# swacisko/ALGA

Hardware: AMD Instinct MI355X
Metric: overlap_edges_per_sec (higher is better)
Workload: dtype u32; 1 GPU; cfg4_50M_150bp: 50000000 x 150 bp reads, genome 250000000, seed 11, err 0.00 -> 90621096 nodes (both strands, duplicates removed), min_overlap 82, rsoemo 116; generated on the device (alga_amd.workload.device_build) in 0.9 s; nodes=90621096, edges=92350115

## Files before the change

alga_amd/csrc/engine.hip:

```cpp
#include <hip/hip_runtime.h>

#include <algorithm>
#include <chrono>
#include <cstdio>
#include <cstdlib>
#include <cstring>
#include <new>
#include <string>
#include <thread>
#include <vector>

#include "engine_internal.h"
#include "prefsuf_shard.h"

using namespace alga;

namespace {

using Prepared = AlgaPrepared;

int prepare(alga_engine *e, const alga_nodes *nodes, const alga_prefsuf_params *p, hipStream_t s, Prepared &out) {
    if (!nodes || !p) return alga_fail(e, ALGA_ERR_INVALID_ARGUMENT, "nodes/params must not be NULL");
    if (nodes->n < 0) return alga_fail(e, ALGA_ERR_INVALID_ARGUMENT, "negative node count");
    if (nodes->n > 0 && (!nodes->words || !nodes->len)) return alga_fail(e, ALGA_ERR_INVALID_ARGUMENT, "words/len must not be NULL");
// ... 88 lines not shown
    const void *before = e->cl_pile_tab.p;
    const size_t cap_before = e->cl_pile_tab.cap;
    if ((rc = alga_ensure(e, e->cl_pile_tab, pile_table_bytes(n_buckets)))) return rc;
    if (e->cl_pile_tab.p != before || e->cl_pile_tab.cap != cap_before) {
        HIP_TRY(e, hipMemsetAsync(e->cl_pile_tab.p, 0, e->cl_pile_tab.cap, s));
        HIP_TRY(e, hipStreamSynchronize(s));
        e->pile_epoch = 0;
    }
    return ALGA_OK;
}

int discover_impl(alga_engine *e, const Prepared &pp, int32_t src_begin, int32_t src_end, hipStream_t s, uint64_t *n_rec, bool local = false,
                  bool *overflow = nullptr) {
    int rc;
    const NodesDev &nd = pp.nd;
    const PrefSufCfg &cfg = pp.cfg;
    unsigned long long *cnt = (unsigned long long *) e->counters.p;
    *n_rec = 0;
    HIP_TRY(e, hipEventRecord(e->ev[EV_START], s));
    if (pp.live >= (1ull << 31)) return alga_fail(e, ALGA_ERR_CAPACITY, "too many nodes for one seed table; shard the input");
    const bool clustered = local && pp.cluster_eq != 0;
    e->pairs_timed = false;
    e->store_timed = false;
    e->pile_timed = false;
    e->pile_deg_pending = false;
    const bool all_sources = src_begin == 0 && src_end == pp.nd.n;
    const bool pile_index_left = e->opt_pile_range != 0 && e->pile_n == pp.nd.n && e->pile_words == (const void *) pp.nd.words;
    bool pile = clustered && e->opt_pile != 0 && e->opt_cluster_pairs != 0 && e->opt_cluster_order != 0 && pp.local_sw == 1 &&
                      (pp.keys_shared == 0 || (pp.keys_shared == 2 && pile_index_left)) &&
                      (all_sources || (e->opt_pile_range != 0 && src_begin >= 0 && src_end <= pp.nd.n && src_begin < src_end)) && pile_plan(cfg, pp.cluster, pp.cluster_eq, pp.uniform_len, pp.nd.from != nullptr || pp.nd.to != nullptr);
    e->loc_second_used = false;
    bool keys_only = false;
    const bool need_vals = !e->opt_own_sort || e->opt_test_unsorted_index;
    uint32_t n_buckets = 0, filter_bits = 0;
    bool have_table = false;
    auto build_table = [&]() -> int {
        n_buckets = seed_buckets_for(pp.live, e->seed_fill_x10);
        const size_t table_bytes = (size_t) n_buckets * SEED_BUCKET * sizeof(unsigned long long);
        int r;
        if ((r = alga_ensure(e, e->table, table_bytes))) return r;
        HIP_TRY(e, hipMemsetAsync(e->table.p, 0xFF, table_bytes, s));
        filter_bits = seed_filter_bits_for(pp.live);
        if (filter_bits) {
            if ((r = alga_ensure(e, e->filter, filter_bits / 8))) return r;
            HIP_TRY(e, hipMemsetAsync(e->filter.p, 0, filter_bits / 8, s));
        }
        launch_seed_build(nd, cfg, (unsigned long long *) e->table.p, n_buckets, (uint32_t *) e->filter.p, filter_bits, s);
        if ((r = alga_check_launch(e, "k_seed_build"))) return r;
        e->stats.table_slots = (uint64_t) n_buckets * SEED_BUCKET;
        have_table = true;
        return ALGA_OK;
    };
    ClusterCfg cc{};
    if (clustered) {
        cc = pp.cluster;
        if ((rc = cluster_alloc(e, pp))) return rc;
        if (pp.keys_shared == 2) {
            const bool store_left = e->store_n == nd.n && e->store_words == (const void *) nd.words && e->store_eq == pp.cluster_eq && e->store_buckets == cc.n_buckets;
            const bool piles_serve = pile && e->pile_kept_pure && e->store_buckets == cc.n_buckets && e->store_eq == pp.cluster_eq;
            if (!(store_left || piles_serve) || src_begin < e->store_run_begin || src_end > e->store_run_end)
                return alga_fail(e, ALGA_ERR_INVALID_ARGUMENT, "keys_shared = 2: no entry array of this node set that covers the sources is left from the previous build");
            keys_only = pile && e->pile_keys_only;
        } else {
            int32_t run_begin = 0, run_end = nd.n;
            if (pp.keys_shared == 1) {
                if (e->keyed_n != nd.n || e->keyed_words != (const void *) nd.words || src_begin < e->keyed_begin || src_end > e->keyed_end)
                    return alga_fail(e, ALGA_ERR_INVALID_ARGUMENT, "keys_shared: alga_prefsuf_keys_device has not been called on this node set for a range that covers the sources");
                run_begin = e->keyed_begin; run_end = e->keyed_end;
            } else {
                keys_only = pile && e->opt_pile_runs != 0 && !e->expect_pairwise && !e->opt_pile_check;
                launch_cluster_keys(nd, cfg, cc, 0, nd.n, (uint32_t *) e->cl_keys[0].p, need_vals ? (uint32_t *) e->cl_vals[0].p : nullptr, (uint32_t *) e->cl_meta.p, e->cl_runs.p,
                                    (uint8_t *) e->cl_nruns.p, s, !keys_only);
                if ((rc = alga_check_launch(e, "k_node_runs"))) return rc;
            }
            HIP_TRY(e, hipEventRecord(e->ev[EV_KEYS], s));
            e->keyed_n = -1;
            e->store_n = -1;
            HIP_TRY(e, launch_cluster_sort(nd, cc, (uint32_t *) e->cl_keys[0].p, (uint32_t *) e->cl_vals[0].p, (uint32_t *) e->cl_keys[1].p,
                                           (uint32_t *) e->cl_vals[1].p, e->sort_temp.p, cluster_sort_temp_bytes((uint64_t) nd.n), pp.keys_shared == 1 || !need_vals,
                                           e->ev[EV_SORT], e->opt_test_unsorted_index != 0, s, e->opt_own_sort != 0));
            const bool dir_late = pile && e->opt_pile_dir >= 1;
            e->dir_late = dir_late;
            if (!dir_late) {
                HIP_TRY(e, launch_cluster_dir(nd, cc, (const uint32_t *) e->cl_keys[1].p, e->cl_dir.p, cnt + CNT_TOTAL + 1, nullptr, s));
                HIP_TRY(e, hipEventRecord(e->ev[EV_DIR], s));
            }
            e->pile_n = -1;
            if (pile) {
                rc = e->opt_test_pile_oom ? alga_fail(e, ALGA_ERR_OUT_OF_MEMORY, "pile_alloc (option test_pile_oom)") : pile_alloc(e, (uint64_t) nd.n, cc.n_buckets, s);
                if (rc == ALGA_ERR_OUT_OF_MEMORY) {
                    (void) hipGetLastError();
                    alga_release(e->cl_pile_tab); alga_release(e->cl_pile_rec); alga_release(e->cl_pile_rec2); alga_release(e->cl_pile_succ); alga_release(e->cl_pile_own);
                    alga_release(e->cl_pile_list);
                    e->pile_epoch = 0; e->pile_n = -1;
                    e->err.clear();
                    pile = false;
                    rc = ALGA_OK;
                    if (keys_only) {
                        launch_cluster_keys(nd, cfg, cc, 0, nd.n, (uint32_t *) e->cl_keys[0].p, (uint32_t *) e->cl_vals[0].p, (uint32_t *) e->cl_meta.p, e->cl_runs.p,
                                            (uint8_t *) e->cl_nruns.p, s, true);
                        if ((rc = alga_check_launch(e, "k_node_runs"))) return rc;
                        keys_only = false;
                    }
                } else if (rc) return rc;
            }
            if (pile) {
                launch_pile_sample(nd, cc, pp.uniform_len, (const uint32_t *) e->cl_keys[1].p, (const uint32_t *) e->cl_vals[1].p, e->cl_dir.p,
                                   (unsigned long long *) e->cl_pile_cnt.p, e->opt_pile >= 2 ? e->opt_pile - 1 : 0, s, e->opt_pile_dir >= 1);
                if ((rc = alga_check_launch(e, "k_pile_build<sample>"))) return rc;
            }
            e->pile_tab_index = pile && e->opt_pile_dir >= 2 && e->opt_pile_skip_gather && !cfg.stats;
            if (dir_late) {
                HIP_TRY(e, hipEventRecord(e->ev[EV_SAMPLE], s));
                HIP_TRY(e, launch_cluster_dir(nd, cc, (const uint32_t *) e->cl_keys[1].p, e->cl_dir.p, cnt + CNT_TOTAL + 1,
                                              e->pile_tab_index ? (const unsigned long long *) e->cl_pile_cnt.p : nullptr, s));
                HIP_TRY(e, hipEventRecord(e->ev[EV_DIR], s));
            }
            HIP_TRY(e, launch_cluster_gather(nd, cc, pp.cluster_eq, (const uint32_t *) e->cl_keys[1].p, (const uint32_t *) e->cl_vals[1].p, (const uint32_t *) e->cl_meta.p,
                                             pp.uniform_len, e->cl_store.p, (pile && e->opt_pile_skip_gather) ? (const unsigned long long *) e->cl_pile_cnt.p : nullptr, s));
            HIP_TRY(e, hipEventRecord(e->ev[EV_GATHER], s));
            if (pile) {
                if (e->pile_epoch >= 511u) {
                    HIP_TRY(e, hipMemsetAsync(e->cl_pile_tab.p, 0, e->cl_pile_tab.cap, s));
                    e->pile_epoch = 0;
                }
                e->pile_epoch++;
                const bool from_consensus = e->opt_pile_runs != 0;
                launch_pile_build(nd, cfg, cc, pp.uniform_len, (const uint32_t *) e->cl_keys[1].p, (const uint32_t *) e->cl_vals[1].p, e->cl_dir.p, e->cl_pile_rec.p, e->cl_pile_rec2.p, e->cl_pile_tab.p,
                                  e->pile_epoch, e->cl_pile_succ.p, e->cl_runs.p, pp.uniform_len - cfg.Lmin + 1, (const unsigned long long *) e->cl_pile_cnt.p,
                                  from_consensus ? (uint32_t *) e->cl_pile_own.p : nullptr, (from_consensus && e->opt_pile_runs_list) ? e->cl_pile_list.p : nullptr, s,
                                  e->opt_pile_dir >= 1, cnt + CNT_TOTAL + 1, e->pile_tab_index, e->opt_pile_runs_ahead != 0);
                if ((rc = alga_check_launch(e, "k_pile_build"))) return rc;
                if (keys_only) {
                    launch_pile_own_ids((const uint32_t *) e->cl_pile_own.p, (const uint32_t *) e->cl_vals[1].p, (uint64_t) nd.n, (int32_t *) e->cl_defer.p, (uint32_t) nd.n,
                                        (unsigned long long *) e->cl_pile_cnt.p, s);
                    launch_cluster_runs_list(nd, cfg, cc, (const int32_t *) e->cl_defer.p, (const unsigned long long *) e->cl_pile_cnt.p + 3, (uint32_t) nd.n, (uint32_t) e->n_cu * 16u,
                                             e->cl_runs.p, (uint8_t *) e->cl_nruns.p, s);
                    launch_cluster_keys(nd, cfg, cc, 0, nd.n, (uint32_t *) e->cl_keys[0].p, (uint32_t *) e->cl_vals[0].p, (uint32_t *) e->cl_meta.p, e->cl_runs.p,
                                        (uint8_t *) e->cl_nruns.p, s, true, (const unsigned long long *) e->cl_pile_cnt.p);
                    if ((rc = alga_check_launch(e, "k_node_runs (own lists)"))) return rc;
                }
                if (e->opt_pile_check && from_consensus)
                    launch_pile_check(e->cl_pile_succ.p, (uint64_t) nd.n, cc.n_buckets, e->cl_pile_tab.p, e->cl_pile_rec2.p, e->pile_epoch, e->cl_runs.p, nd.n, pp.uniform_len - cfg.Lmin + 1,
                                      (unsigned long long *) e->cl_pile_cnt.p, s);
                e->pile_n = nd.n; e->pile_words = (const void *) nd.words;
                e->pile_keys_only = keys_only; e->pile_kept_pure = false;
                e->pile_timed = nd.n > 0;
            }
            e->store_timed = nd.n > 0;
            e->store_n = pile ? -1 : nd.n;
            e->store_words = (const void *) nd.words; e->store_eq = pp.cluster_eq; e->store_buckets = cc.n_buckets;
            e->store_run_begin = run_begin; e->store_run_end = run_end;
        }
        e->stats.table_slots = cc.n_buckets;
    } else if ((rc = build_table())) return rc;
    HIP_TRY(e, hipEventRecord(e->ev[EV_SEED], s));

    const uint64_t n_src = (uint64_t) std::max<int64_t>(0, (int64_t) src_end - src_begin);
    const uint64_t slack = std::max(probe_record_slack(e->n_cu, n_src, local), clustered ? cluster_record_slack(e->n_cu, n_src) : 0);
    uint64_t &hint = local ? e->rec_cap_hint_local : e->rec_cap_hint;
    uint64_t cap = std::max<uint64_t>(hint, (local ? 2 : 16) * n_src + 4096) + slack;
    if (local) {
        if ((rc = alga_ensure(e, e->outdeg, (size_t) (n_src + 1) * sizeof(uint32_t)))) return rc;
        if ((rc = alga_ensure(e, e->loc_first, (size_t) (n_src + 1) * sizeof(unsigned long long)))) return rc;
    }
    const uint32_t big_list_cap = 1u << 20;
    if (local && (rc = alga_ensure(e, e->loc_big_list, big_list_cap * sizeof(int32_t)))) return rc;
    bool pure_streamed = false;
    for (int attempt = 0; attempt < 4; attempt++) {
        if (cap >= (1ull << 32) - 16) return alga_fail(e, ALGA_ERR_CAPACITY, "more than 2^32 overlap records; shard the input");
        if (local) HIP_TRY(e, hipMemsetAsync(e->outdeg.p, 0, (size_t) (n_src + 1) * sizeof(uint32_t), s));
        if ((rc = alga_ensure(e, e->rec_dst, cap * sizeof(uint32_t)))) return rc;
        if ((rc = alga_ensure(e, e->rec_val, cap * sizeof(unsigned long long)))) return rc;
        HIP_TRY(e, hipMemsetAsync(cnt, 0, CNT_TOTAL * sizeof(unsigned long long), s));
        ProbeBig big{(int32_t *) e->loc_big_list.p, big_list_cap, 0u, nullptr, 0u};
        e->defer_list_valid = clustered && e->opt_cluster_pairs && pp.local_sw == 1 && pp.cluster_eq <= 4;
        if (clustered) {
            if (e->opt_cluster_pairs && pp.local_sw == 1 && pp.cluster_eq <= 4) {
                if ((rc = alga_ensure(e, e->cl_defer, (size_t) (n_src + 64) * sizeof(int32_t)))) return rc;
                const uint32_t slot_stride = e->opt_stream_slots >= 4 ? (uint32_t) (n_src + 1) : 0u;
                if ((rc = alga_ensure(e, e->loc_second, (size_t) (slot_stride ? LOCAL_SLOTS_MAX - 1 : 1) * (n_src + 1) * sizeof(unsigned long long)))) return rc;
                e->loc_second_used = true;
                e->loc_slot_stride = slot_stride;
                const bool by_key = e->opt_cluster_order != 0 && src_begin == 0 && src_end == nd.n;
                const bool piled = pile && e->pile_n == nd.n && e->pile_words == (const void *) nd.words;
                if (piled) {
                    if (!all_sources) {
                        if ((rc = alga_ensure(e, e->cl_pile_side_r, (size_t) (n_src + 64) * 16))) return rc;
                        if ((rc = alga_ensure(e, e->cl_pile_cursor, 64))) return rc;
                    }
                    launch_pile_probe(nd, cfg, cc, pp.uniform_len, e->cl_pile_tab.p, e->pile_epoch, e->cl_pile_rec.p, e->cl_pile_rec2.p, e->cl_pile_succ.p,
                                      e->cl_runs.p, cnt, (uint32_t *) e->outdeg.p, (unsigned long long *) e->loc_first.p, (unsigned long long *) e->loc_second.p,
                                      (int32_t *) e->cl_defer.p, (uint32_t) n_src, (const unsigned long long *) e->cl_pile_cnt.p, e->n_cu, s, src_begin, src_end,
                                      e->cl_pile_side_r.p, (unsigned long long *) e->cl_pile_cursor.p, e->opt_pile_probe_lean != 0, e->opt_pile_probe_tail != 0);
                    if ((rc = alga_check_launch(e, "k_pile_probe"))) return rc;
                    if (keys_only)
                        launch_cluster_runs_list(nd, cfg, cc, (const int32_t *) e->cl_defer.p, cnt + CNT_DEFERRED, (uint32_t) std::min<uint64_t>(n_src + 64, 0xFFFFFFFFull),
                                                 (uint32_t) e->n_cu * 16u, e->cl_runs.p, (uint8_t *) e->cl_nruns.p, s);
                }
                launch_probe_stream(nd, cfg, cc, pp.cluster_eq, e->cl_store.p, e->cl_dir.p, e->cl_runs.p, (const uint8_t *) e->cl_nruns.p,
                                    src_begin, src_end, by_key, cnt, e->n_cu, (uint32_t *) e->outdeg.p, (unsigned long long *) e->loc_first.p,
                                    (unsigned long long *) e->loc_second.p, (int32_t *) e->cl_defer.p, (uint32_t) n_src,
                                    piled ? (const unsigned long long *) e->cl_pile_cnt.p : nullptr, s, slot_stride);
                if ((rc = alga_check_launch(e, "k_probe_stream"))) return rc;
                if (piled) {
                    if ((rc = alga_ensure(e, e->cl_defer2, (size_t) (n_src + 64) * sizeof(int32_t)))) return rc;
                    pure_streamed = launch_probe_stream_list(nd, cfg, cc, pp.cluster_eq, e->cl_store.p, e->cl_dir.p, e->cl_runs.p, (const uint8_t *) e->cl_nruns.p, (int32_t *) e->cl_defer.p,
                                             (uint32_t) n_src, cnt, e->n_cu, (uint32_t *) e->outdeg.p, (unsigned long long *) e->loc_first.p,
                                             (unsigned long long *) e->loc_second.p, (int32_t *) e->cl_defer2.p, (const unsigned long long *) e->cl_pile_cnt.p, s, slot_stride, src_begin,
                                             (const uint32_t *) e->cl_keys[1].p, (const uint32_t *) e->cl_vals[1].p, pp.uniform_len, e->opt_pile_stream_by_id != 0,
                                             e->pile_tab_index ? e->cl_pile_tab.p : nullptr, e->pile_epoch);
                    if ((rc = alga_check_launch(e, "k_probe_stream (list)"))) return rc;
                }
                HIP_TRY(e, hipEventRecord(e->ev[EV_PAIRS], s));
// ... 256 lines not shown
    hipError_t err = hipGetDeviceCount(&ndev);
    if (err != hipSuccess || ndev <= 0) return ALGA_ERR_NO_DEVICE;
    if (hip_device < 0 || hip_device >= ndev) return ALGA_ERR_INVALID_ARGUMENT;
    DeviceGuard guard;
    if (hipSetDevice(hip_device) != hipSuccess) return ALGA_ERR_NO_DEVICE;
    alga_engine *e = new (std::nothrow) alga_engine();
    if (!e) return ALGA_ERR_OUT_OF_MEMORY;
    e->device = hip_device;
    memset(&e->stats, 0, sizeof(e->stats));
    hipDeviceProp_t prop;
    if (hipGetDeviceProperties(&prop, hip_device) == hipSuccess) {
        snprintf(e->dev_name, sizeof(e->dev_name), "%s (%s, %d CUs)", prop.name, prop.gcnArchName, prop.multiProcessorCount);
        if (prop.multiProcessorCount > 0) e->n_cu = prop.multiProcessorCount;
    }
    int rc = ALGA_OK;
    if (hipStreamCreateWithFlags(&e->own_stream, hipStreamNonBlocking) != hipSuccess) { e->own_stream = nullptr; rc = ALGA_ERR_HIP; }
    if (rc == ALGA_OK && hipStreamCreateWithFlags(&e->side_stream, hipStreamNonBlocking) != hipSuccess) { e->side_stream = nullptr; rc = ALGA_ERR_HIP; }
    if (rc == ALGA_OK && hipEventCreateWithFlags(&e->ev_side, hipEventDisableTiming) != hipSuccess) { e->ev_side = nullptr; rc = ALGA_ERR_HIP; }
    for (int i = 0; i < EV_COUNT && rc == ALGA_OK; i++)
        if (hipEventCreate(&e->ev[i]) != hipSuccess) { e->ev[i] = nullptr; rc = ALGA_ERR_HIP; }
    if (rc == ALGA_OK && hipHostMalloc((void **) &e->h_counters, (CNT_TOTAL + 2 + alga_engine::H_EXTRA) * sizeof(unsigned long long)) != hipSuccess) { e->h_counters = nullptr; rc = ALGA_ERR_OUT_OF_MEMORY; }
    if (rc == ALGA_OK && hipHostGetDevicePointer((void **) &e->h_counters_dev, e->h_counters, 0) != hipSuccess) rc = ALGA_ERR_HIP;
    if (rc != ALGA_OK) { engine_free_handles(e); delete e; return rc; }
    *out = e;
    return ALGA_OK;
}

void alga_engine_destroy(alga_engine *e) {
    if (!e) return;
    DeviceGuard guard;
    (void) hipSetDevice(e->device);
    if (e->own_stream) (void) hipStreamSynchronize(e->own_stream);
    if (e->side_stream) (void) hipStreamSynchronize(e->side_stream);
    for (DevBuf *b : e->owned) alga_release(*b);
    alga_release(e->up_raw);
    for (DevBuf *b : {&e->in_bytes[0], &e->in_bytes[1], &e->in_nl[0], &e->in_nl[1], &e->in_tiles, &e->in_tile_off}) alga_release(*b);
    for (DevBuf *b : {&e->sp_rowptr, &e->sp_sorted, &e->sp_list, &e->sp_cnt, &e->sp_orow, &e->sp_out, &e->sp_in}) alga_release(*b);
    alga_staging_release(e);
    for (void *&p : e->gfa_pin) { if (p) (void) hipHostFree(p); p = nullptr; }
    for (auto &kv : e->host_lists) free(kv.first);
    e->host_lists.clear();
    engine_free_handles(e);
    delete e;
}

const char *alga_last_error(const alga_engine *e) { return e ? e->err.c_str() : "no engine"; }

int alga_engine_device_name(const alga_engine *e, char *buf, size_t buflen) {
    if (!e || !buf || buflen == 0) return ALGA_ERR_INVALID_ARGUMENT;
    snprintf(buf, buflen, "%s", e->dev_name);
    return ALGA_OK;
}

int alga_engine_set_option(alga_engine *e, const char *name, int64_t value) {
    if (!e || !name) return ALGA_ERR_INVALID_ARGUMENT;
    e->err.clear();
    if (!strcmp(name, "probe")) {
        if (value < ALGA_PROBE_AUTO || value > ALGA_PROBE_CLUSTER) return alga_fail(e, ALGA_ERR_INVALID_ARGUMENT, "option probe: 0 auto, 1 table, 2 cluster");
        e->opt_probe = (int) value;
    } else if (!strcmp(name, "cluster_bucket_bias")) {
        if (value < -8 || value > 8) return alga_fail(e, ALGA_ERR_INVALID_ARGUMENT, "option cluster_bucket_bias: -8 .. 8");
        e->opt_cluster_bucket_bias = (int) value;
    } else if (!strcmp(name, "cluster_pairs")) {
        e->opt_cluster_pairs = value != 0;
    } else if (!strcmp(name, "pile")) {
        e->opt_pile = (value == 2 || value == 3) ? (int) value : (value != 0);
    } else if (!strcmp(name, "pile_runs")) {
        e->opt_pile_runs = value != 0;
    } else if (!strcmp(name, "pile_runs_list")) {
        e->opt_pile_runs_list = value != 0;
    } else if (!strcmp(name, "pile_dir")) {
        if (value < 0 || value > 2) return alga_fail(e, ALGA_ERR_INVALID_ARGUMENT, "option pile_dir: 0 directory records, 1 k_pile_build from the keys, 2 ... and no directory for a pure pile build");
        e->opt_pile_dir = (int) value;
    } else if (!strcmp(name, "pile_deg_fold")) {
        e->opt_pile_deg_fold = value != 0;
    } else if (!strcmp(name, "emit_fused")) {
        e->opt_emit_fused = value != 0;
    } else if (!strcmp(name, "pile_probe_lean")) {
        e->opt_pile_probe_lean = value != 0;
    } else if (!strcmp(name, "pile_probe_tail")) {
        e->opt_pile_probe_tail = value != 0;
    } else if (!strcmp(name, "pile_runs_ahead")) {
        e->opt_pile_runs_ahead = value != 0;
    } else if (!strcmp(name, "pile_stream_by_id")) {
        e->opt_pile_stream_by_id = value != 0;
    } else if (!strcmp(name, "pile_check")) {
        e->opt_pile_check = value != 0;
    } else if (!strcmp(name, "pile_skip_gather")) {
        e->opt_pile_skip_gather = value != 0;
    } else if (!strcmp(name, "cluster_order")) {
        e->opt_cluster_order = value != 0;
    } else if (!strcmp(name, "local_big_max")) {
        e->big_limit = value < 0 ? -1 : (int) std::min<int64_t>(value, 1 << 20);
    } else if (!strcmp(name, "shard_bucket_max")) {
        e->opt_shard_dmax = (int) std::max<int64_t>(1, std::min<int64_t>(value, 4096));
    } else if (!strcmp(name, "rsort_variant")) {
        if (value < 0 || value > 1) return alga_fail(e, ALGA_ERR_INVALID_ARGUMENT, "option rsort_variant: 0 tiles of 8192 pairs, 1 tiles of 16384 pairs");
        rsort_set_variant((int) value);
    } else if (!strcmp(name, "stream_slots")) {
        e->opt_stream_slots = value >= 4 ? 4 : 2;
    } else if (!strcmp(name, "pile_range")) {
        e->opt_pile_range = value != 0;
    } else if (!strcmp(name, "pkb_legacy")) {
        e->opt_pkb_legacy = (int) value;
    } else if (!strcmp(name, "own_sort")) {
        e->opt_own_sort = value != 0;
    } else if (!strcmp(name, "test_presort_oom")) {
        e->opt_test_presort_oom = value != 0;
    } else if (!strcmp(name, "test_pile_oom")) {
        e->opt_test_pile_oom = value != 0;
    } else if (!strcmp(name, "test_unsorted_index")) {
        e->opt_test_unsorted_index = value != 0;
    } else if (!strcmp(name, "gfa_chunk_mb")) {
        if (value < 1 || value > 4096) return alga_fail(e, ALGA_ERR_INVALID_ARGUMENT, "option gfa_chunk_mb: 1 .. 4096");
        e->opt_gfa_chunk_mb = (int) value;
    } else if (!strcmp(name, "mst_mid_nodes")) {
        if (value < 8 || value > (1 << 20)) return alga_fail(e, ALGA_ERR_INVALID_ARGUMENT, "option mst_mid_nodes: 8 .. 2^20");
        e->opt_mst_mid_nodes = (int) value;
    } else if (!strcmp(name, "consensus_max_blocks")) {
        if (value < 0 || value > (1 << 20)) return alga_fail(e, ALGA_ERR_INVALID_ARGUMENT, "option consensus_max_blocks: 0 .. 2^20");
        e->opt_consensus_max_blocks = (int) value;
    } else if (!strcmp(name, "unitig_ruling")) {
        if (value < -1 || value > 1) return alga_fail(e, ALGA_ERR_INVALID_ARGUMENT, "option unitig_ruling: -1, 0 or 1");
        e->opt_unitig_ruling = (int) value;
    } else if (!strcmp(name, "correct_slice_keys")) {
        if (value < 1 || value > (1ll << 31)) return alga_fail(e, ALGA_ERR_INVALID_ARGUMENT, "option correct_slice_keys: 1 .. 2^31");
        e->opt_correct_slice_keys = value;
    } else if (!strcmp(name, "correct_dir_bits")) {
        if (value < 0 || value > 28) return alga_fail(e, ALGA_ERR_INVALID_ARGUMENT, "option correct_dir_bits: 0 (auto) or 1 .. 28");
        e->opt_correct_dir_bits = (int) value;
    } else if (!strcmp(name, "place_dir_bits")) {
        if (value < 0 || value > 26) return alga_fail(e, ALGA_ERR_INVALID_ARGUMENT, "option place_dir_bits: 0 (auto) or 1 .. 26");
        e->opt_place_dir_bits = (int) value;
    } else if (!strcmp(name, "auto_reduction_per_target")) {
        e->opt_force_per_target = value != 0;
    } else return alga_fail(e, ALGA_ERR_INVALID_ARGUMENT, "unknown option");
    return ALGA_OK;
}

int alga_engine_reserve(alga_engine *e, int32_t n_nodes, int32_t max_len, int32_t min_overlap, uint64_t n_edges_hint) {
    if (!e) return ALGA_ERR_INVALID_ARGUMENT;
    e->err.clear();
    if (n_nodes < 0 || max_len < 1 || min_overlap < 1) return alga_fail(e, ALGA_ERR_INVALID_ARGUMENT, "alga_engine_reserve: n_nodes >= 0, max_len >= 1, min_overlap >= 1");
    DeviceGuard guard;
    HIP_TRY(e, hipSetDevice(e->device));
    int rc;
    const uint64_t n = (uint64_t) n_nodes;
    const uint64_t E = n_edges_hint ? n_edges_hint : n + n / 16 + 4096;
    if ((rc = alga_ensure(e, e->counters, (CNT_TOTAL + 2) * sizeof(unsigned long long)))) return rc;
    Prepared pp;
    pp.nd.n = n_nodes; pp.max_len = max_len; pp.live = n;
    pp.cfg.Lmin = min_overlap; pp.cfg.Lcap = std::min(max_len, 500) + 1; pp.cfg.rsoemo = min_overlap; pp.cfg.soes = 3;
    int eq = 0;
    const bool local = max_len <= 500 && max_len - min_overlap <= LOCAL_MAX_SPAN;
    const bool clustered = local && e->opt_probe != ALGA_PROBE_TABLE &&
                           cluster_plan(pp.cfg, max_len, n, e->opt_cluster_bucket_bias, &pp.cluster, &eq);
    if (clustered) {
        pp.cluster_eq = eq;
        if ((rc = cluster_alloc(e, pp))) return rc;
        if (max_len - min_overlap <= 63 && eq <= 4) {
            if ((rc = alga_ensure(e, e->cl_defer, (size_t) (n + 64) * sizeof(int32_t)))) return rc;
            if ((rc = alga_ensure(e, e->loc_second, (size_t) (e->opt_stream_slots >= 4 ? LOCAL_SLOTS_MAX - 1 : 1) * (n + 1) * sizeof(unsigned long long)))) return rc;
        }
        if (e->opt_pile != 0 && e->opt_cluster_pairs != 0 && e->opt_cluster_order != 0 && max_len - min_overlap <= 63 && pile_plan(pp.cfg, pp.cluster, eq, max_len, false)) {
            if ((rc = pile_alloc(e, n, pp.cluster.n_buckets, e->own_stream))) return rc;
        }
// ... 669 lines not shown
```

alga_amd/csrc/engine_internal.h:

```cpp
#pragma once
#include <hip/hip_runtime.h>

#include <cstdio>
#include <algorithm>
#include <string>
#include <vector>
#include <unordered_map>

#include "../../include/alga_amd.h"
#include "prefsuf_common.h"
#include "prefsuf_kernels.h"
#include "pkb_kernels.h"

struct DevBuf {
    void  *p = nullptr;
    size_t cap = 0;
};

enum { EV_START = 0, EV_SEED, EV_PROBE, EV_GROUP, EV_REDUCE, EV_EMIT, EV_PAIRS, EV_KEYS, EV_SORT, EV_GATHER, EV_DIR, EV_SAMPLE, EV_COUNT };
constexpr int ALGA_STAGE_THREADS = 8;

struct alga_engine {
    std::vector<DevBuf *> owned;
    int         device = -1;
    hipStream_t own_stream = nullptr;
    hipStream_t side_stream = nullptr;
    hipEvent_t  ev_side = nullptr;
    std::string err;
    char        dev_name[256] = {0};
    int         n_cu = 256;
    int         seed_fill_x10 = 20;
    int         opt_probe = 0;
    int         opt_cluster_bucket_bias = 0;
    int         opt_force_per_target = 0;
    int         opt_shard_dmax = 4096;
    int         opt_test_unsorted_index = 0;
    hipEvent_t  ev[EV_COUNT] = {};
    DevBuf table, filter, counters, rowptr, rec_dst, rec_val, keys, seg_key, seg_val, heads, sort_temp, out_cnt, outdeg, out_rowptr, edges, scan_scratch;
    DevBuf cl_defer;
    uint32_t h_first_hkey = 255;
    int32_t keyed_n = -1, keyed_begin = 0, keyed_end = 0;
    bool defer_list_valid = false;
    const void *keyed_words = nullptr;
    int32_t store_n = -1, store_run_begin = 0, store_run_end = 0, store_eq = 0;
    uint32_t store_buckets = 0;
    const void *store_words = nullptr;
    int stat_max_len = 0, stat_min_len = 0; uint64_t stat_live = 0; unsigned long long stat_mask_asym = 0;
    const void *stat_len = nullptr, *stat_from = nullptr, *stat_to = nullptr;
    bool   warmed = false;
    bool   pairs_timed = false;
    bool   store_timed = false;
    bool   pile_keys_only = false, pile_kept_pure = false;
    int    opt_pile_range = 1;
    int    opt_pile_skip_gather = 1;
    int    opt_pile = 1;
    int    opt_pile_runs = 1;
    int    opt_pile_runs_list = 1;
    DevBuf cl_pile_list;
    int    opt_pile_deg_fold = 1;
    int    opt_emit_fused = 1;
    int    opt_pile_dir = 2;
    bool   dir_late = false;
    bool   pile_tab_index = false;
    int    opt_pile_stream_by_id = 0;
    int    opt_pile_probe_lean = 1;
    int    opt_pile_probe_tail = 1;
    int    opt_pile_runs_ahead = 0;
    bool   pile_deg_pending = false;
    int    opt_pile_check = 0;
    bool   expect_pairwise = false;
    DevBuf cl_pile_side_r, cl_pile_cursor;
    DevBuf cl_pile_own;
    int    opt_pkb_legacy = 0;
    int    opt_own_sort = 1;
    int    opt_test_presort_oom = 0;
    int    opt_test_pile_oom = 0;
    bool   pile_timed = false;
    DevBuf cl_pile_succ;
    DevBuf cl_pile_rec2;
    DevBuf cl_pile_rec, cl_pile_cnt, cl_pile_tab;
    uint32_t pile_epoch = 0;
    int32_t pile_n = -1; const void *pile_words = nullptr;
    int    opt_cluster_order = 1;
    int    opt_cluster_pairs = 1;
    DevBuf cl_keys[2], cl_vals[2], cl_meta, cl_runs, cl_nruns, cl_store, cl_dir;
    DevBuf loc_second;
    bool   loc_second_used = false;
    uint32_t loc_slot_stride = 0;
    int    opt_stream_slots = 4;
    DevBuf loc_first, loc_big_list, loc_big_items;
    int    big_limit = -1;
    DevBuf edge_keys, edge_keys2, edge_vals, edge_vals2, edges_sorted, xs_dst, xs_val;
    DevBuf up_words, up_len, up_from, up_to;
    DevBuf up_len_narrow;
    DevBuf cp_deg, cp_dst, cp_off;
    DevBuf cl_defer2;
    DevBuf pk_keys, pk_keys2, pk_vals, pk_vals2, pk_marks, pk_big, pk_add, pk_ekeys, pk_ekeys2, pk_flag, pk_pos, pk_edges[2], pk_rowptr, pk_deg,
           pk_mask, pk_cnt, pk_io, pk_io2, pk_tips, pk_heads, pk_g[2], pk_addk, pk_addk2, pk_merged, pk_hsz, pk_hsz2, pk_heads2, pk_nadd, pk_koff,
           pk_gsz, pk_fixlist, pk_bounds, pk_tiprec, pk_tipidx, pk_keys_all, pk_vals_all;
    DevBuf pk_keys2b, pk_vals2b, pk_headsb, pk_hszb, sort_temp2, pk_fixlist2, pk_cnt2;
    DevBuf pp_rows, pp_len, pp_perm[2], pp_keys[2], pp_mark, pp_keep, pp_pos, pp_out_rows, pp_out_len, pp_out_pair, pp_tally;
    bool        stage_ready = false;
    void       *stage_pin[ALGA_STAGE_THREADS][2] = {};
    hipEvent_t  stage_ev[ALGA_STAGE_THREADS][2] = {};
    hipStream_t stage_stream[ALGA_STAGE_THREADS] = {};
    DevBuf      up_raw;
    std::unordered_map<void *, size_t> host_lists;
    void       *host_spare = nullptr;
    size_t      host_spare_cap = 0;
    DevBuf      in_bytes[2], in_nl[2], in_tiles, in_tile_off;
    DevBuf      sp_rowptr, sp_sorted, sp_list, sp_cnt, sp_orow, sp_out, sp_in;
    DevBuf      tp_cnt, tp_keys[2], tp_vals[2], tp_flag, tp_pos, tp_best, tp_est, tp_rev, tp_rfid, tp_rowptr[2], tp_alive, tp_kill, tp_rec[2], tp_branch,
                tp_overflow, tp_ws, tp_out;
    DevBuf      mp_cnt, mp_rowptr, mp_rows, mp_len, mp_owner, mp_pend[2], mp_win, mp_overflow, mp_overflow2, mp_ws, mp_ws_big, mp_orow, mp_out;
    struct MstFilled { const void *p = nullptr; size_t bytes = 0; uint32_t hbits = 0, cap_nodes = 0, cap_edges = 0; int32_t n_ws = 0; } mp_filled[2];
    int         opt_mst_mid_nodes = 4096;
    DevBuf      gfa_sizes, gfa_off, gfa_rowptr, gfa_tiles, gfa_bounds, gfa_buf;
    void       *gfa_pin[2] = {nullptr, nullptr};
    size_t      gfa_pin_cap = 0;
    int         opt_gfa_chunk_mb = 256;
    DevBuf      ut_cnt, ut_keys[2], ut_vals[2], ut_flag, ut_pos, ut_best, ut_estar, ut_rowptr, ut_nxt, ut_noff, ut_prv, ut_rank[2], ut_min[2], ut_tail,
                ut_win, ut_pair, ut_pcnt, ut_ulen, ut_ulen2, ut_uwords, ut_path_off, ut_word_off, ut_tiles, ut_path_node, ut_path_pos, ut_uid, ut_words,
                ut_edges, ut_link, ut_rnode, ut_rrec[2];
    int         opt_unitig_ruling = -1;
    uint64_t    ut_n_pairs = 0, ut_n_edges = 0;
    bool        ut_valid = false;
    int32_t     ut_n_nodes = 0;
    uint64_t    ut_total_bases = 0;
    bool        ut_is_contig = false;
    DevBuf      ex_cnt, ex_rowptr, ex_w, ex_kcnt, ex_dlink, ex_outcnt, ex_sole, ex_xhead, ex_xbase, ex_xrank, ex_uid, ex_scnt, ex_seam_off,
                ex_seam_entry, ex_pcnt, ex_uwords, ex_ulen, ex_ulen2, ex_path_off, ex_word_off, ex_path_node, ex_path_pos, ex_words, ex_edges;
    bool        ut_is_extended = false;
    DevBuf      ct_cnt, ct_B[2], ct_rowptr, ct_pflag, ct_runkey, ct_chain, ct_headchain, ct_drop, ct_flag, ct_pos, ct_keys[2], ct_vals[2], ct_hw, ct_hk, ct_H,
                ct_hrow, ct_hsorted, ct_hlist, ct_hcnt, ct_win, ct_pair, ct_oid, ct_cid, ct_deg, ct_epos, ct_ekeys[2], ct_evals[2], ct_names;
    DevBuf      cs_cnt, cs_words, cs_mask, cs_votes, cs_trim, cs_len, cs_changed;
    bool        cs_valid = false;
    bool        cs_has_votes = false;
    DevBuf      fc_cnt, fc_keys[2], fc_vals, fc_first, fc_min, fc_list[2], fc_flag, fc_ids, fc_verdict, fc_rank, fc_id, fc_new, fc_trim, fc_begin, fc_len,
                fc_order, fc_wbegin, fc_wlen, fc_rows, fc_rlen, fc_tid;
    bool        fc_valid = false;
    uint64_t    fc_n_accepted = 0;
    int         opt_consensus_max_blocks = 0;
    DevBuf      cr_cnt, cr_table, cr_hist, cr_keys[2], cr_flag, cr_pos, cr_solid, cr_dir;
    int64_t     opt_correct_slice_keys = 1ll << 28;
    int         opt_correct_dir_bits = 0;
    DevBuf      pl_cnt, pl_fbegin, pl_flen, pl_scan, pl_cols, pl_keys[2], pl_vals[2], pl_dir, pl_ub, pl_diff;
    DevBuf      pl_target, pl_pos, pl_mm, pl_hits, pl_state, pl_coloff, pl_cover, pl_tstat, pl_hist;
    bool        pl_valid = false;
    uint64_t    pl_targets = 0, pl_reads = 0;
    uint64_t    pl_ncolumns = 0, pl_nhist = 0;
// ... 3 lines not shown
    DevBuf      po_cnt, po_keys[2], po_vals[2], po_marks, po_pop, po_scan;
    DevBuf      po_coloff, po_words, po_ccols, po_cbases, po_tstat, po_counts;
    bool        po_valid = false;
    uint64_t    po_targets = 0, po_columns = 0;
    uint64_t    po_final_epoch = 0;
    uint64_t    pl_serial = 0, po_pl_serial = 0;
    DevBuf      sc_cnt, sc_keys[2], sc_vals[2], sc_span, sc_heads, sc_pos, sc_bstart, sc_best, sc_choice, sc_partner, sc_lists[2], sc_head, sc_first, sc_scan;
    DevBuf      sc_ba, sc_bb, sc_blinks, sc_bspan, sc_bgap, sc_bstate, sc_estate, sc_scaffold, sc_rank, sc_orient, sc_start, sc_gapafter, sc_jlinks, sc_soff,
                sc_smembers, sc_slen;
    bool        sc_valid = false;
    uint64_t    sc_targets = 0, sc_scaffolds = 0, sc_longest = 0;
    uint64_t    sc_pl_serial = 0;
    DevBuf      br_cnt, br_diff, br_starts, br_rpos, br_marks, br_rfirst, br_rlast, br_closed, br_cpos;
    DevBuf      br_span, br_ccols, br_cfirst, br_clast, br_tcuts, br_poff, br_begin, br_len, br_ptarget, br_pstart, br_words;
    bool        br_valid = false;
    uint64_t    br_targets = 0, br_pieces = 0, br_cuts = 0, br_columns = 0, br_longest = 0;
    DevBuf      gr_cnt, gr_flag, gr_pos, gr_cand, gr_elen, gr_eoff, gr_ecols, gr_keys[2], gr_vals[2], gr_dir, gr_ub, gr_x, gr_g;
    struct GrowSet { DevBuf end, over, mm, hits, state, count, estop, evoters, left, right, len, coloff, begin, words; } gr_set[2];
    int         gr_cur = 0;
    bool        gr_valid = false;
    uint64_t    gr_reads = 0, gr_targets = 0, gr_columns = 0, gr_longest = 0;
    DevBuf      mg_cnt, mg_elen, mg_epad, mg_eoff, mg_ecols, mg_pcols, mg_keys[2], mg_vals[2], mg_dir, mg_join, mg_lists[2], mg_head, mg_first, mg_scan;
    struct MergeSet { DevBuf partner, olen, mm, hits, estate, merged, rank, orient, start, ovafter, moff, mmembers, len, coloff, begin, words; } mg_set[2];
    int         mg_cur = 0;
    bool        mg_valid = false;
    uint64_t    mg_targets = 0, mg_merged = 0, mg_columns = 0, mg_longest = 0;
    DevBuf      sh_keys[2], sh_vals[2], sh_store, sh_dir, sh_desc_out, sh_dkey[2], sh_dval[2], sh_small_top, sh_pending, sh_bitmap, sh_small_out,
                sh_ssrc[2], sh_skey[2], sh_edges_out, sh_deg, sh_rowptr, sh_cursor, sh_edges, sh_flagged, sh_cnt, sh_gflag, sh_gpos, sh_gstart;
    struct {
        int      phase = 0;
        int      rank = 0, n_ranks = 1, eq = 0, uniform_len = 0;
        int32_t  n = 0;
        const void *words = nullptr;
        alga::PrefSufCfg cfg{};
        alga::ClusterCfg cc{};
        uint32_t bucket_base = 0, bpr = 0;
        uint64_t n_targets = 0, n_desc = 0, n_rec = 0;
        uint32_t *d_keys_sorted = nullptr;
        unsigned long long *d_vals_sorted = nullptr;
    } sh;
    alga_shard_stats shard_stats{};
    struct {
        int      phase = 0;
        int      rounds = 0, round = 0, rank = 0, n_ranks = 1, cur = 0, key_bits = 0;
        int32_t  prio[4] = {0, 1, 2, 3};
        uint64_t E = 0, nk = 0;
        uint32_t n_tips = 0;
        int      pre_set = 0, cur_set = 0;
        bool     no_look_ahead = false;
        int      pre_round = -1;
        bool     kmers_all = false;
        size_t   kmers_stride = 0;
        int      kmers_sort_bits = 0;
        alga_nodes dn{};
        alga::PkbCfg cfg{};
    } pkb;
    unsigned long long *h_counters = nullptr;
    static constexpr int H_EXTRA = 132 + 16, H_PRE = alga::CNT_TOTAL + 2 + 132;
    uint32_t *h_counters_dev = nullptr;
    uint64_t    rec_cap_hint = 0, rec_cap_hint_local = 0;
    alga_prefsuf_stats stats;
    double      stats_host[2] = {0.0, 0.0};
    alga_pkb_stats pkb_stats;
};

struct AlgaPrepared {
    alga::NodesDev   nd;
    alga::PrefSufCfg cfg;
    int        max_len = 0;
    int        uniform_len = 0;
    uint64_t   live = 0;
    bool       local_ok = false;
    int        local_sw = 1;
    int        cluster_eq = 0;
    alga::ClusterCfg cluster{};
    int        reduction = ALGA_REDUCTION_AUTO;
    int        keys_shared = 0;
};

extern "C" int alga_upload_nodes_phase(alga_engine *e, const alga_nodes *nodes, bool twin_rows, int mode, uint64_t row_begin, uint64_t row_end, uint64_t raw_rows_cap, alga_nodes *dev,
                            uint32_t **d_raw);
int alga_prepare(alga_engine *e, const alga_nodes *nodes, const alga_prefsuf_params *p, hipStream_t s, AlgaPrepared &out);
int alga_cluster_alloc(alga_engine *e, const AlgaPrepared &pp);

inline int alga_fail(alga_engine *e, int code, const char *what, hipError_t herr = hipSuccess) {
    char buf[512];
    if (herr != hipSuccess) snprintf(buf, sizeof(buf), "%s: %s", what, hipGetErrorString(herr));
    else snprintf(buf, sizeof(buf), "%s", what);
    e->err = buf;
    return code;
}

#define HIP_TRY(e, call)                                                                     \
    do {                                                                                     \
        hipError_t _err = (call);                                                            \
        if (_err != hipSuccess) return alga_fail((e), _err == hipErrorOutOfMemory ? ALGA_ERR_OUT_OF_MEMORY : ALGA_ERR_HIP, #call, _err); \
    } while (0)

inline int alga_ensure(alga_engine *e, DevBuf &b, size_t bytes) {
    if (bytes == 0) bytes = 16;
    if (b.cap >= bytes) return ALGA_OK;
    if (b.p) { HIP_TRY(e, hipFree(b.p)); b.p = nullptr; b.cap = 0; }
    else if (std::find(e->owned.begin(), e->owned.end(), &b) == e->owned.end()) e->owned.push_back(&b);
    HIP_TRY(e, hipMalloc(&b.p, bytes));
    b.cap = bytes;
    return ALGA_OK;
}

inline void alga_forget_node_set(alga_engine *e) {
    e->keyed_n = -1; e->store_n = -1; e->pile_n = -1;
    e->stat_len = nullptr; e->stat_from = nullptr; e->stat_to = nullptr;
}

inline void alga_release(DevBuf &b) {
    if (b.p) (void) hipFree(b.p);
    b.p = nullptr; b.cap = 0;
}

#include <chrono>
#include <functional>
typedef std::function<void(void * , size_t , size_t )> AlgaStageFill;
int  alga_staged_h2d(alga_engine *e, void *d_dst, const void *h_src, size_t bytes);
int  alga_staged_h2d_fill(alga_engine *e, void *d_dst, size_t bytes, const AlgaStageFill &fill);
int  alga_staged_d2h(alga_engine *e, void *h_dst, const void *d_src, size_t bytes);
void alga_staging_release(alga_engine *e);
void *alga_host_list_take(alga_engine *e, size_t bytes);
void alga_host_list_give(alga_engine *e, void *p);

constexpr int ALGA_UT_MAX_ROUNDS = 112;
int alga_ut_check(alga_engine *e, const alga_nodes *nodes, const alga::alga_edge_dev *d_in, uint64_t m, unsigned long long *cnt, hipStream_t s);
int alga_ut_estar(alga_engine *e, const alga_nodes *nodes, const alga::alga_edge_dev *d_in, uint64_t m, unsigned long long *cnt, hipStream_t s, uint64_t *ms_out);
int alga_ut_rank(alga_engine *e, const int32_t *len, int32_t n, int32_t *nxt, const int32_t *noff, int32_t *prv, unsigned long long *cnt, uint32_t *p_flag,
                 int &cur, int &rounds, hipStream_t s);

struct AlgaTextJob {
    uint64_t items;
    std::function<void(uint32_t *sizes, unsigned long long *counters, hipStream_t s)> sizes;
    std::function<void(const unsigned long long *off, uint64_t i0, uint64_t i1, char *buf, hipStream_t s)> format;
    const char *kind = "FASTA";
    const char *head = "";
    std::function<int(unsigned long long *counters, hipStream_t s)> prepare;
};
int alga_text_job_run(alga_engine *e, const AlgaTextJob &job, const char *path, alga_gfa_info *info,
                      std::chrono::steady_clock::time_point t0 = std::chrono::steady_clock::now());

template <class F> int alga_text_records(alga_engine *e, const F &f, void (*sizes)(const F &, uint32_t *, unsigned long long *, hipStream_t),
                                         void (*write)(const F &, const unsigned long long *, uint64_t, uint64_t, char *, hipStream_t), const char *path,
                                         alga_gfa_info *info, std::chrono::steady_clock::time_point t0 = std::chrono::steady_clock::now()) {
    AlgaTextJob job;
    job.items = f.n;
    job.sizes = [f, sizes](uint32_t *out, unsigned long long *counters, hipStream_t s) { sizes(f, out, counters, s); };
    job.format = [f, write](const unsigned long long *off, uint64_t i0, uint64_t i1, char *buf, hipStream_t s) { write(f, off, i0, i1, buf, s); };
    return alga_text_job_run(e, job, path, info, t0);
}

int alga_correct_check_params(alga_engine *e, const alga_correct_params *p);
int alga_correct_impl(alga_engine *e, uint32_t *d_rows, int32_t stride, const int32_t *d_len, int64_t n_nodes, const alga_correct_params *p, hipStream_t s,
                      alga_correct_info *info);

bool alga_final_is_current(const alga_engine *e, const alga_unitigs *u, const alga_consensus *cons, const alga_final_contigs *fin, const char **why);

inline int alga_check_launch(alga_engine *e, const char *what) {
    hipError_t err = hipGetLastError();
    if (err != hipSuccess) return alga_fail(e, ALGA_ERR_HIP, what, err);
    return ALGA_OK;
}
// ... 1 lines not shown
```

alga_amd/csrc/engine_shard.hip:

```cpp
#include <hip/hip_runtime.h>

#include <algorithm>
#include <cstring>
#include <vector>

#include "engine_internal.h"
#include "prefsuf_shard.h"

using namespace alga;

namespace {

struct EvPair { hipEvent_t a = nullptr, b = nullptr; };

struct PhaseTimer {
    hipStream_t s; hipEvent_t a = nullptr, b = nullptr;
    explicit PhaseTimer(hipStream_t st) : s(st) { if (hipEventCreate(&a) != hipSuccess) a = nullptr; if (hipEventCreate(&b) != hipSuccess) b = nullptr; if (a) (void) hipEventRecord(a, s); }
    double stop() { float ms = 0.f; if (a && b && hipEventRecord(b, s) == hipSuccess && hipEventSynchronize(b) == hipSuccess) (void) hipEventElapsedTime(&ms, a, b); return ms; }
    ~PhaseTimer() { if (a) (void) hipEventDestroy(a); if (b) (void) hipEventDestroy(b); }
};

int shard_sync_counters(alga_engine *e, hipStream_t s, const unsigned long long *d, int n, std::vector<unsigned long long> &h) {
    h.assign(256, 0ull);
    HIP_TRY(e, hipStreamSynchronize(s));
    HIP_TRY(e, hipMemcpy(h.data(), d, (size_t) n * sizeof(unsigned long long), hipMemcpyDeviceToHost));
    return ALGA_OK;
}

}

extern "C" {

int alga_shard_index_device(alga_engine *e, const alga_nodes *nodes, const alga_prefsuf_params *p, int32_t rank, int32_t n_ranks, void *hip_stream,
                            const uint32_t **d_desc, uint64_t *desc_counts, uint64_t *desc_offsets) {
    if (!e) return ALGA_ERR_INVALID_ARGUMENT;
    e->err.clear();
    if (!d_desc || !desc_counts || !desc_offsets) return alga_fail(e, ALGA_ERR_INVALID_ARGUMENT, "output pointers must not be NULL");
    *d_desc = nullptr;
    if (n_ranks < 1 || n_ranks > 64 || rank < 0 || rank >= n_ranks) return alga_fail(e, ALGA_ERR_INVALID_ARGUMENT, "bad rank / n_ranks (1 .. 64 ranks)");
    for (int q = 0; q < n_ranks; q++) { desc_counts[q] = 0; desc_offsets[q] = 0; }
    e->sh.phase = 0;
    HIP_TRY(e, hipSetDevice(e->device));
    hipStream_t s = hip_stream ? (hipStream_t) hip_stream : e->own_stream;
    const int32_t kb = e->keyed_begin, ke = e->keyed_end;
    if (!nodes || e->keyed_n != nodes->n || e->keyed_words != (const void *) nodes->words)
        return alga_fail(e, ALGA_ERR_INVALID_ARGUMENT, "alga_shard_index_device: alga_prefsuf_keys_device has not been called on this node set");
    alga_prefsuf_params p2 = *p;
    p2.keys_shared = 2;
    e->store_n = -1;
    AlgaPrepared pp;
    {
        const int32_t kn = e->keyed_n;
        int rc = alga_prepare(e, nodes, &p2, s, pp);
        if (rc) return rc;
        e->keyed_n = kn;
    }
    if (!pp.local_ok || pp.cluster_eq == 0 || pp.cluster_eq > 4 || pp.local_sw != 1 || pp.reduction == ALGA_REDUCTION_PER_TARGET)
        return alga_fail(e, ALGA_ERR_UNSUPPORTED, "the bucket-sharded form takes reads of up to 208 nt with max_len - min_overlap <= 63 (one-word offset masks) and the source-side preconditions");
    memset(&e->shard_stats, 0, sizeof(e->shard_stats));
    const ClusterCfg cc = pp.cluster;
    const uint32_t n = (uint32_t) nodes->n;
    const uint32_t bpr = shard_buckets_per_rank(cc.n_buckets, n_ranks);
    const uint32_t b_lo = std::min<uint64_t>((uint64_t) rank * bpr, cc.n_buckets), b_hi = std::min<uint64_t>((uint64_t) (rank + 1) * bpr, cc.n_buckets);
    int rc;
    if ((rc = alga_ensure(e, e->sh_cnt, 256 * sizeof(unsigned long long)))) return rc;
    unsigned long long *cnt = (unsigned long long *) e->sh_cnt.p;
    HIP_TRY(e, hipMemsetAsync(cnt, 0, 256 * sizeof(unsigned long long), s));
    PhaseTimer t_index(s);
    for (int k = 0; k < 2; k++) {
        if ((rc = alga_ensure(e, e->sh_keys[k], ((size_t) n + 1) * sizeof(uint32_t)))) return rc;
        if ((rc = alga_ensure(e, e->sh_vals[k], ((size_t) n + 1) * sizeof(uint32_t)))) return rc;
    }
    launch_shard_select((const uint32_t *) e->cl_keys[0].p, n, cc.idx_shift, b_lo, b_hi, (uint32_t *) e->sh_keys[0].p, (uint32_t *) e->sh_vals[0].p, cnt, s);
    if ((rc = alga_check_launch(e, "k_shard_select"))) return rc;
    const uint32_t flagged_cap = 1u << 20;
    if ((rc = alga_ensure(e, e->sh_flagged, (size_t) flagged_cap * sizeof(int32_t)))) return rc;
    launch_shard_export(true, e->cl_runs.p, kb, ke, cc.idx_shift, bpr, (uint32_t) n_ranks, cnt + 64, (int32_t *) e->sh_flagged.p, cnt + 1, flagged_cap, nullptr, nullptr, nullptr, s);
    if ((rc = alga_check_launch(e, "k_shard_export (count)"))) return rc;
    std::vector<unsigned long long> hc;
    if ((rc = shard_sync_counters(e, s, cnt, 128, hc))) return rc;
    const uint64_t m = hc[0], n_flagged = hc[1];
    if (n_flagged > flagged_cap) return alga_fail(e, ALGA_ERR_UNSUPPORTED, "more than 2^20 sources of this rank need brute-force window minimizers");
    std::vector<unsigned long long> seg((size_t) n_ranks + 1, 0ull);
    for (int q = 0; q < n_ranks; q++) seg[(size_t) q + 1] = seg[(size_t) q] + hc[64 + (size_t) q] + 64ull * n_flagged;
    const uint64_t desc_cap = seg[(size_t) n_ranks];
    if (desc_cap >= (1ull << 32) - 16) return alga_fail(e, ALGA_ERR_CAPACITY, "more than 2^32 run descriptors on one rank");
    if ((rc = alga_ensure(e, e->sh_desc_out, (desc_cap + 1) * 12))) return rc;
    HIP_TRY(e, hipMemcpyAsync(cnt + 192, seg.data(), (size_t) n_ranks * sizeof(unsigned long long), hipMemcpyHostToDevice, s));
    const uint32_t n_b_local = b_hi - b_lo;
    if ((rc = alga_ensure(e, e->sh_store, (m + 2) * 16 * (size_t) pp.cluster_eq))) return rc;
    if ((rc = alga_ensure(e, e->sh_dir, ((size_t) n_b_local + 2) * 16))) return rc;
    if ((rc = alga_ensure(e, e->sort_temp, std::max(cluster_sort_temp_bytes(m), sort_desc_temp_bytes(1))))) return rc;
    HIP_TRY(e, launch_cluster_store_slice(pp.nd, cc, pp.cluster_eq, m, b_lo, n_b_local, (uint32_t *) e->sh_keys[0].p, (uint32_t *) e->sh_vals[0].p, (uint32_t *) e->sh_keys[1].p,
                                          (uint32_t *) e->sh_vals[1].p, (const uint32_t *) e->cl_meta.p, pp.uniform_len, e->sort_temp.p, cluster_sort_temp_bytes(m),
                                          e->sh_store.p, e->sh_dir.p, cnt + 2, s, e->opt_own_sort != 0));
    e->shard_stats.ms_index = t_index.stop();
    PhaseTimer t_export(s);
    launch_shard_export(false, e->cl_runs.p, kb, ke, cc.idx_shift, bpr, (uint32_t) n_ranks, nullptr, nullptr, nullptr, 0u, cnt + 192, cnt + 128, (uint32_t *) e->sh_desc_out.p, s);
    if ((rc = alga_check_launch(e, "k_shard_export"))) return rc;
    launch_shard_export_flagged(pp.nd, pp.cfg, cc, (const int32_t *) e->sh_flagged.p, (uint32_t) n_flagged, bpr, (uint32_t) n_ranks, cnt + 192, cnt + 128,
                                (uint32_t *) e->sh_desc_out.p, s);
    if ((rc = alga_check_launch(e, "k_shard_export_flagged"))) return rc;
    e->shard_stats.ms_export = t_export.stop();
    if ((rc = shard_sync_counters(e, s, cnt, 192, hc))) return rc;
    if (hc[2] != 0) return alga_fail(e, ALGA_ERR_HIP, "bucket-sharded index: the sorted key array is not in order");
    uint64_t total = 0;
    for (int q = 0; q < n_ranks; q++) {
        desc_counts[q] = hc[128 + (size_t) q]; desc_offsets[q] = seg[(size_t) q];
        if (desc_counts[q] > seg[(size_t) q + 1] - seg[(size_t) q]) return alga_fail(e, ALGA_ERR_HIP, "bucket-sharded index: descriptor segment overflow");
        total += desc_counts[q];
    }
    e->shard_stats.targets_owned = m; e->shard_stats.descriptors_out = total; e->shard_stats.flagged_sources = n_flagged;
    e->sh.phase = 1; e->sh.rank = rank; e->sh.n_ranks = n_ranks; e->sh.eq = pp.cluster_eq; e->sh.uniform_len = pp.uniform_len; e->sh.n = nodes->n;
    e->sh.words = (const void *) nodes->words; e->sh.cfg = pp.cfg; e->sh.cc = cc; e->sh.bucket_base = b_lo; e->sh.bpr = bpr; e->sh.n_targets = m;
    *d_desc = (const uint32_t *) e->sh_desc_out.p;
    return ALGA_OK;
}

int alga_shard_join_device(alga_engine *e, const alga_nodes *nodes, const uint32_t *d_desc_in, uint64_t n_desc, void *hip_stream, const uint32_t **d_pending_src,
                           uint64_t *n_pending_src) {
    if (!e) return ALGA_ERR_INVALID_ARGUMENT;
    e->err.clear();
    if (!d_pending_src || !n_pending_src) return alga_fail(e, ALGA_ERR_INVALID_ARGUMENT, "output pointers must not be NULL");
    *d_pending_src = nullptr; *n_pending_src = 0;
    if (e->sh.phase != 1 || !nodes || nodes->n != e->sh.n || (const void *) nodes->words != e->sh.words)
        return alga_fail(e, ALGA_ERR_INVALID_ARGUMENT, "alga_shard_join_device follows alga_shard_index_device on the same node set");
    if (n_desc && !d_desc_in) return alga_fail(e, ALGA_ERR_INVALID_ARGUMENT, "descriptor array must not be NULL");
    if (n_desc >= (1ull << 32) - 16) return alga_fail(e, ALGA_ERR_CAPACITY, "more than 2^32 run descriptors on one rank");
    HIP_TRY(e, hipSetDevice(e->device));
    hipStream_t s = hip_stream ? (hipStream_t) hip_stream : e->own_stream;
    int rc;
    NodesDev nd;
    nd.words = nodes->words; nd.len = nodes->len; nd.from = nodes->align_from; nd.to = nodes->align_to; nd.n = nodes->n; nd.stride = nodes->stride_words;
    unsigned long long *cnt = (unsigned long long *) e->counters.p;
    unsigned long long *scnt = (unsigned long long *) e->sh_cnt.p;
    PhaseTimer t_sort(s);
    for (int k = 0; k < 2; k++) {
        if ((rc = alga_ensure(e, e->sh_dkey[k], (n_desc + 64) * sizeof(uint32_t)))) return rc;
        if ((rc = alga_ensure(e, e->sh_dval[k], (n_desc + 64) * sizeof(unsigned long long)))) return rc;
    }
    if ((rc = alga_ensure(e, e->sort_temp, sort_desc_temp_bytes(n_desc)))) return rc;
    if ((rc = alga_ensure(e, e->sh_small_top, (n_desc + 1) * 3 * sizeof(unsigned long long)))) return rc;
    const int shift = e->sh.cc.idx_shift;
    int range_bits = 1;
    while (range_bits < 32 - shift && (1ull << range_bits) < (uint64_t) e->sh.bpr) range_bits++;
    launch_shard_desc_split(d_desc_in, n_desc, e->sh.bucket_base << shift, (uint32_t *) e->sh_dkey[0].p, (unsigned long long *) e->sh_dval[0].p, s);
    if ((rc = alga_check_launch(e, "k_shard_desc_split"))) return rc;
    HIP_TRY(e, sort_desc(e->sort_temp.p, sort_desc_temp_bytes(n_desc), (const uint32_t *) e->sh_dkey[0].p, (uint32_t *) e->sh_dkey[1].p, (const unsigned long long *) e->sh_dval[0].p,
                         (unsigned long long *) e->sh_dval[1].p, n_desc, shift, std::min(32, shift + range_bits), s, e->opt_own_sort != 0));
    if ((rc = alga_ensure(e, e->sh_gflag, (n_desc + 2) * sizeof(uint32_t)))) return rc;
    if ((rc = alga_ensure(e, e->sh_gpos, (n_desc + 2) * sizeof(uint32_t)))) return rc;
    if ((rc = alga_ensure(e, e->sh_gstart, (n_desc + 2) * sizeof(uint32_t)))) return rc;
    if ((rc = alga_ensure(e, e->scan_scratch, scan_scratch_bytes(n_desc + 1)))) return rc;
    launch_shard_groups((const uint32_t *) e->sh_dkey[1].p, n_desc, e->sh.cc.idx_shift, (uint32_t *) e->sh_gflag.p, (uint32_t *) e->sh_gpos.p, (uint32_t *) e->sh_gstart.p,
                        (uint64_t *) e->scan_scratch.p, s);
    if ((rc = alga_check_launch(e, "k_shard_groups"))) return rc;
    uint32_t n_groups = 0;
    if (n_desc) {
        HIP_TRY(e, hipMemcpyAsync(e->h_counters, (const uint32_t *) e->sh_gpos.p + n_desc, sizeof(uint32_t), hipMemcpyDeviceToHost, s));
        HIP_TRY(e, hipStreamSynchronize(s));
        n_groups = *(const uint32_t *) e->h_counters;
    }
    e->shard_stats.ms_sort = t_sort.stop();
    e->sh.d_keys_sorted = (uint32_t *) e->sh_dkey[1].p; e->sh.d_vals_sorted = (unsigned long long *) e->sh_dval[1].p;
    PhaseTimer t_join(s);
    const uint64_t slack = shard_join_record_slack(e->n_cu);
    uint64_t cap = std::max<uint64_t>(e->rec_cap_hint, 2 * e->sh.n_targets + n_desc / 4 + 4096) + slack;
    uint64_t n_rec = 0;
    bool done = false;
    unsigned long long join_passes[2] = {0, 0};
    for (int attempt = 0; attempt < 4 && !done; attempt++) {
        if (cap >= (1ull << 32) - 16) return alga_fail(e, ALGA_ERR_CAPACITY, "more than 2^32 overlap records; shard the input");
        if ((rc = alga_ensure(e, e->rec_dst, cap * sizeof(uint32_t)))) return rc;
        if ((rc = alga_ensure(e, e->rec_val, cap * sizeof(unsigned long long)))) return rc;
        HIP_TRY(e, hipMemsetAsync(cnt, 0, CNT_TOTAL * sizeof(unsigned long long), s));
        HIP_TRY(e, hipMemsetAsync(scnt, 0, 8 * sizeof(unsigned long long), s));
        launch_shard_join(nd, e->sh.cfg, e->sh.cc, e->sh.eq, e->sh.uniform_len, e->sh_store.p, e->sh_dir.p, e->sh.bucket_base, e->sh.d_keys_sorted, e->sh.d_vals_sorted, n_desc,
                          (const uint32_t *) e->sh_gstart.p, n_groups, (uint32_t *) e->rec_dst.p, (unsigned long long *) e->rec_val.p, cap, cnt, (unsigned long long *) e->sh_small_top.p, scnt + 3, e->opt_shard_dmax, e->n_cu, s);
// ... 181 lines not shown
```

alga_amd/csrc/prefsuf_cluster.hip:

```cpp
#include <hip/hip_runtime.h>
#include <algorithm>
#include "prefsuf_common.h"
#include "prefsuf_kernels.h"
#include "prefsuf_device.h"
#include "prefsuf_cluster_device.h"

namespace alga {


template <int TKW, bool WIDE, bool RUNS>
__global__ void __launch_bounds__(TK_ROWS) k_node_runs(NodesDev nd, PrefSufCfg cfg, ClusterCfg cc, int node_begin, int node_end,
                                                        uint32_t *__restrict__ keys, uint32_t *__restrict__ vals, uint32_t *__restrict__ meta,
                                                        uint2 *__restrict__ runs, uint8_t *__restrict__ nruns, const int32_t *__restrict__ id_list, const unsigned long long *__restrict__ id_count,
                                                        const unsigned long long *__restrict__ only_if_declined ) {
    if (only_if_declined && !pile_cnt_declines(only_if_declined)) return;
    __shared__ uint32_t s[TK_ROWS][TKW];
    __shared__ uint32_t stk[RUNS ? 2 * (NR_STACK + 1) : 1][TK_ROWS];
    __shared__ uint16_t rbuf[RUNS ? CL_RMAX + 1 : 1][TK_ROWS];
    const int list_n = id_list ? (int) min((unsigned long long) (node_end - node_begin), *id_count) : 0;
    __shared__ int sid[TK_ROWS];
    for (int blk = (int) blockIdx.x; id_list ? blk * TK_ROWS < list_n : node_begin + blk * TK_ROWS < node_end; blk += (int) gridDim.x) {
    const int base = node_begin + blk * TK_ROWS;
    const int nrows = id_list ? min(TK_ROWS, list_n - blk * TK_ROWS) : min(TK_ROWS, node_end - base);
    if (blk != (int) blockIdx.x) __syncthreads();
// ... 38 lines not shown
        for (int r = 0; r < CL_RMAX; r++) {
            if (r < nr_stored && is_src) {
                const uint32_t d = rbuf[r][t];
                const int q = (int) (d & 255u);
                uint32_t h, pk;
                kmer_key(row, q < (WIDE ? 192 : 128) ? q : 0, true, cc, h, pk);
                runs[(size_t) i * CL_RMAX + r] = make_uint2(cluster_key(h, fs), d | ((uint32_t) p1 << 16) | (r == 0 ? nr_code << 24 : 0u));
                p1 = (int) (d >> 8);
            }
        }
        if (in && !is_src) runs[(size_t) i * CL_RMAX] = make_uint2(0u, 0u);
        if (in) nruns[i] = (uint8_t) nr_code;
        if (id_list) continue;
    } else {
        const int nk = act ? min(nwin, WIDE ? 64 : nwin) - 1 + w : 0;
        uint64_t b0;
        {
            const uint32_t x0 = row[0], x1 = row[1], x2 = row[2], x3 = row[3], x4 = row[4];
            const uint32_t d0 = compress_even(class0_mask16(x0, x1)) | (compress_even(class0_mask16(x1, x2)) << 16);
            const uint32_t d1 = compress_even(class0_mask16(x2, x3)) | (compress_even(class0_mask16(x3, x4)) << 16);
            b0 = (uint64_t) d0 | ((uint64_t) d1 << 32);
            b0 &= nk >= 64 ? ~0ull : (nk <= 0 ? 0ull : ((1ull << nk) - 1ull));
            b0 &= w >= 64 ? ~0ull : ((1ull << w) - 1ull);
        }
        while (b0 != 0ull) {
            const int e = __builtin_ctzll(b0);
            b0 &= b0 - 1ull;
            const int bit = 2 * e, q = bit >> 5, r = bit & 31;
            const uint32_t x0 = row[q], x1 = row[q + 1], x2 = row[q + 2];
            const uint32_t pk = order_key0(kmer_hash(funnel(x0, x1, r) & cc.lo_mask, funnel(x1, x2, r) & cc.hi_mask), e);
            cur0 = pk < cur0 ? pk : cur0;
        }
    }
    uint32_t key = 0xFFFFFFFFu, m = act ? (((uint32_t) len << 8) | (is_src ? CL_META_FROM : 0u)) : 0u;
    if (is_tgt) {
        uint32_t pmin = cur0;
        if (pmin == 0xFFFFFFFFu) {
            for (int k = 0; k < w; k++) { uint32_t h, pk; kmer_key(row, k, true, cc, h, pk); pmin = pk < pmin ? pk : pmin; }
        }
        uint32_t h, pk;
        kmer_key(row, (int) (pmin & 255u), true, cc, h, pk);
        key = tgt_sort_key(cluster_key(h, fs), pmin & 255u, fs);
        m = (pmin & 255u) | ((uint32_t) len << 8) | (is_src ? CL_META_FROM : 0u);
    }
    if (in) { keys[i] = key; if (vals) vals[i] = (uint32_t) i; meta[i] = m; }
    }
}

template <int EQ, bool UNIFORM>
__global__ void __launch_bounds__(256) k_tgt_gather(NodesDev nd, uint64_t count ,
                                                     const uint32_t *__restrict__ keys, const uint32_t *__restrict__ vals,
                                                     const uint32_t *__restrict__ meta, uint32_t uniform_meta, int fs, uint4 *__restrict__ store,
                                                     const unsigned long long *__restrict__ pile_cnt ) {
    if (pile_cnt && pile_cnt[1] * PILE_IRREGULAR_ONE_IN <= pile_cnt[0]) return;
    for (uint64_t t = (uint64_t) blockIdx.x * blockDim.x + threadIdx.x; t < count * EQ; t += (uint64_t) gridDim.x * blockDim.x) {
    const uint64_t j = t / EQ;
    const int c = (int) (t % EQ);
    const uint32_t key = keys[j];
    const uint32_t id = vals[j];
    const uint32_t *row = nd.words + (size_t) id * nd.stride;
    uint4 v;
    if ((nd.stride & 3) == 0 && 4 * c + 3 < nd.stride && ((uintptr_t) nd.words & 15u) == 0) v = reinterpret_cast<const uint4 *>(row)[c];
    else {
        v.x = 4 * c + 0 < nd.stride ? row[4 * c + 0] : 0u; v.y = 4 * c + 1 < nd.stride ? row[4 * c + 1] : 0u;
        v.z = 4 * c + 2 < nd.stride ? row[4 * c + 2] : 0u; v.w = 4 * c + 3 < nd.stride ? row[4 * c + 3] : 0u;
    }
    if (c == EQ - 1) {
        v.y = id; v.z = key;
        if (!UNIFORM) v.w = meta[id];
        else if (key != 0xFFFFFFFFu) v.w = uniform_meta | ((key >> fs) & ((1u << CL_MBITS) - 1u));
        else v.w = (uint32_t) nd.len[id] == (uniform_meta >> 8 & 0xFFFu) ? uniform_meta : 0u;
    }
    store[j * EQ + c] = v;
    }
}

constexpr int TD_TILE = 256, TD_HALO = 96;
__global__ void __launch_bounds__(TD_TILE) k_tgt_dir(const uint32_t *__restrict__ keys, uint64_t n, int shift, uint32_t n_buckets ,
                                                     uint32_t bucket_base , uint4 *__restrict__ dir,
                                                     unsigned long long *__restrict__ bad ,
                                                     const unsigned long long *__restrict__ pile_cnt ) {
    if (pile_cnt && pile_cnt_pure(pile_cnt)) return;
    __shared__ uint32_t sb[TD_TILE + TD_HALO + 1];
    const uint64_t base = (uint64_t) blockIdx.x * TD_TILE;
    const uint32_t nb3 = n_buckets << 3;
    auto tagged = [&](uint64_t k) -> uint32_t { if (k >= n) return nb3; const uint32_t x = keys[k]; return x == 0xFFFFFFFFu ? nb3 : (x >> (shift - 3)) - (bucket_base << 3); };
    for (int k = (int) threadIdx.x; k <= TD_TILE + TD_HALO; k += TD_TILE)
        sb[k] = (base == 0 && k == 0) ? 0xFFFFFFFFu : tagged(base + (uint64_t) k - 1u);
    __syncthreads();
    const int t = (int) threadIdx.x, lane = lane_id();
    const uint64_t j = base + (uint64_t) t;
    auto put = [&](int64_t b, const uint4 &rec) { dir[b] = rec; };
    auto tally = [](unsigned long long acc, uint32_t cls) { return acc + (0x0101010101010100ull << (8u * cls)); };
    if (j >= 1 && j < n && sb[t + 1] < sb[t]) atomicOr(bad, 1ull);
    const uint32_t b = sb[t + 1] >> 3;
    const bool start = j <= n && b != (sb[t] >> 3);
    if (start && b == n_buckets) put(b, make_uint4((uint32_t) j, 0u, 0u, 0u));
    const bool real = start && b != n_buckets;
    constexpr int TD_SHORT = 4;
    const bool is_short = real && (sb[t + 1 + TD_SHORT] >> 3) != b;
    if (is_short) {
        unsigned long long acc = 0ull;
        int u = 0;
#pragma unroll
        for (; u < TD_SHORT; u++) {
            const uint32_t x = sb[t + 1 + u];
            if ((x >> 3) != b) break;
            acc = tally(acc, x & 7u);
        }
        put(b, make_uint4((uint32_t) j, (uint32_t) u, (uint32_t) acc, (uint32_t) (acc >> 32)));
    }
    unsigned long long longs = __ballot(real && !is_short);
    const int g = lane >> 4, gl = lane & 15;
    while (longs != 0ull) {
        int lsel = 64;
#pragma unroll
        for (int q = 0; q < 4; q++) {
            const int l = longs ? __builtin_ctzll(longs) : 64;
            longs = longs ? (longs & (longs - 1ull)) : 0ull;
            lsel = g == q ? l : lsel;
        }
        const bool has = lsel < 64;
        const int t0 = (t & ~63) + (has ? lsel : 0);
        const uint32_t bb = bperm(b, has ? lsel : 0);
        unsigned long long acc = 0ull;
        bool open = has, past = false;
        for (int u = 0;; u += 16) {
            const int idx = t0 + 1 + u + gl;
            const bool staged = idx <= TD_TILE + TD_HALO;
            const uint32_t x = staged ? sb[idx] : 0xFFFFFFFFu;
            const bool inb = open && staged && (x >> 3) == bb;
            const unsigned long long c = inb ? ((0x0101010101010100ull << (8u * (x & 7u))) | 1ull) : 0ull;
            uint32_t lo = (uint32_t) c, hi = (uint32_t) (c >> 32);
            lo += (uint32_t) __builtin_amdgcn_update_dpp(0, (int) lo, 0x111, 0xF, 0xF, true); hi += (uint32_t) __builtin_amdgcn_update_dpp(0, (int) hi, 0x111, 0xF, 0xF, true);
            lo += (uint32_t) __builtin_amdgcn_update_dpp(0, (int) lo, 0x112, 0xF, 0xF, true); hi += (uint32_t) __builtin_amdgcn_update_dpp(0, (int) hi, 0x112, 0xF, 0xF, true);
            lo += (uint32_t) __builtin_amdgcn_update_dpp(0, (int) lo, 0x114, 0xF, 0xF, true); hi += (uint32_t) __builtin_amdgcn_update_dpp(0, (int) hi, 0x114, 0xF, 0xF, true);
            lo += (uint32_t) __builtin_amdgcn_update_dpp(0, (int) lo, 0x118, 0xF, 0xF, true); hi += (uint32_t) __builtin_amdgcn_update_dpp(0, (int) hi, 0x118, 0xF, 0xF, true);
            lo = bperm(lo, lane | 15); hi = bperm(hi, lane | 15);
            acc += ((unsigned long long) hi << 32) | lo;
            const uint32_t took = lo & 255u, cnt = (uint32_t) acc & 255u;
            if (open && took < 16u) { open = false; past = t0 + 1 + u + (int) took > TD_TILE + TD_HALO; }
            else if (open && cnt >= 240u) { open = false; past = true; }
            if (__ballot(open) == 0ull) break;
        }
        if (has && gl == 0) {
            const uint64_t j0 = base + (uint64_t) t0;
            uint64_t k = j0 + (uint64_t) ((uint32_t) acc & 255u);
            acc &= ~255ull;
            if (past) {
                for (; k < j0 + 256u; k++) {
                    const uint32_t x = tagged(k);
                    if ((x >> 3) != bb) break;
                    acc = tally(acc, x & 7u);
                }
                if (k >= j0 + 256u && (tagged(k) >> 3) == bb) {
                    uint64_t a = k, z = n;
                    while (z - a > 1) { const uint64_t mid = a + (z - a) / 2; if ((tagged(mid) >> 3) == bb) a = mid; else z = mid; }
                    k = z;
                }
            }
            const uint32_t c = (uint32_t) (k - j0);
            put(bb, make_uint4((uint32_t) j0, c, c <= 255u ? (uint32_t) acc : 0u, c <= 255u ? (uint32_t) (acc >> 32) : 0u));
        }
    }
}

#ifndef CL_OCC
#define CL_OCC 6
#endif

struct ByIdEntries {
    const uint32_t *skeys, *sids;
    uint32_t uniform_meta;
    const unsigned long long *pile_cnt;
    BucketIndex bx;
};
__device__ __forceinline__ void by_id_pair(const ByIdEntries &by, size_t ei, uint32_t n_nodes, uint32_t &key, uint32_t &id) {
    key = by.skeys[ei];
    id = min(by.sids[ei], n_nodes - 1u);
}
template <int EQ>
__device__ __forceinline__ void entry_by_id(const NodesDev &nd, uint32_t uniform_meta, int fs, uint32_t key, uint32_t id, uint32_t (&ew)[4 * EQ]) {
    static_assert(EQ == 3, "entries by id: rows of nine words");
    const uint32_t *row = nd.words + (size_t) id * nd.stride;
    if ((nd.stride & 3) == 0 && nd.stride >= 12 && ((uintptr_t) nd.words & 15u) == 0) {
        const uint4 v0 = reinterpret_cast<const uint4 *>(row)[0], v1 = reinterpret_cast<const uint4 *>(row)[1];
        ew[0] = v0.x; ew[1] = v0.y; ew[2] = v0.z; ew[3] = v0.w; ew[4] = v1.x; ew[5] = v1.y; ew[6] = v1.z; ew[7] = v1.w;
        ew[8] = row[8];
    } else {
#pragma unroll
        for (int k = 0; k < 9; k++) ew[k] = k < nd.stride ? row[k] : 0u;
    }
    ew[9] = id; ew[10] = key;
    ew[11] = key != 0xFFFFFFFFu ? (uniform_meta | ((key >> fs) & ((1u << CL_MBITS) - 1u))) : 0u;
}
template <bool STATS, int EQ, int KF, int SW = 1, bool BYID = false>
__global__ void __launch_bounds__(PROBE_WAVES * 64, SW == 1 && EQ <= 4 ? CL_OCC : 4)
k_probe_clustered(NodesDev nd, PrefSufCfg cfg, ClusterCfg cc, const uint4 *__restrict__ store, const uint4 *__restrict__ dir,
                  const uint2 *__restrict__ runs, const uint8_t *__restrict__ nruns, int32_t src_begin, int32_t src_end, ProbeOut o,
                  const int32_t *__restrict__ src_list ,
                  const unsigned long long *__restrict__ list_count ,
                  ByIdEntries by) {
    constexpr int WC = 4 * EQ - 3;
    if (by.pile_cnt) {
        const bool kept = by.pile_cnt[1] * PILE_IRREGULAR_ONE_IN <= by.pile_cnt[0];
        if (kept != BYID) return;
    }
    if (list_count) {
        const unsigned long long c = *list_count;
        if (c < (unsigned long long) src_end) src_end = (int32_t) c;
    }
    __shared__ uint32_t sB[PROBE_WAVES][2][STAGE_WORDS];
    __shared__ uint4 sRun[PROBE_WAVES][2][CL_RMAX];
    __shared__ uint32_t sRecC[PROBE_WAVES][WBUF_LOCAL];
    __shared__ unsigned long long sRecV[PROBE_WAVES][WBUF_LOCAL];
    __shared__ uint32_t sCnt[PROBE_WAVES][3];
    __shared__ uint32_t sItemC[PROBE_WAVES][ITEMMAX];
    __shared__ uint32_t sItemM[PROBE_WAVES][ITEMMAX];
    __shared__ uint4 sItemO[PROBE_WAVES][ITEMMAX * SW];
    __shared__ uint8_t sItemT[PROBE_WAVES][64 * SW];
    __shared__ uint4 sMask[KF > 0 ? 129 : 1];
    const int wave = __builtin_amdgcn_readfirstlane((int) (threadIdx.x >> 6));
    const int lane = lane_id();
    WaveLds w{sB[wave][0], nullptr, nullptr, &sCnt[wave][0], sRecC[wave], sRecV[wave], &sCnt[wave][1]};
    ItemLds it{sItemC[wave], sItemM[wave], sItemO[wave], sItemT[wave], &sCnt[wave][2]};
    if (lane == 0) { *w.recN = 0; *it.N = 0; }
    if constexpr (KF > 0) {
        for (int t = (int) threadIdx.x; t <= 128; t += PROBE_WAVES * 64)
            sMask[t] = make_uint4(low_bits32(t), low_bits32(t - 32), low_bits32(t - 64), low_bits32(t - 96));
        __syncthreads();
    }
    uint64_t chunk_base = 0;
    int chunk_fill = REC_CHUNK_LOCAL;
    uint64_t st_raw = 0, st_slots = 0, st_win = 0, st_rec = 0, st_cmp = 0, st_generic = 0;
    const int total_waves = (int) gridDim.x * PROBE_WAVES;
    const int kfull = KF ? KF : (2 * cfg.Lmin) >> 5;

    const int pre_words = nd.stride < STAGE_WORDS ? nd.stride : STAGE_WORDS;
    int Bl = src_begin + (int) blockIdx.x * PROBE_WAVES + wave;
    int n_id = 0, n_len = 0, n_nr = 0; uint32_t n_word = 0; uint2 n_run = make_uint2(0u, 0u);
    auto fetch = [&]() {
        if (Bl < src_end) {
            const int b = src_list ? __builtin_amdgcn_readfirstlane(src_list[Bl]) : Bl;
            n_id = b;
            n_len = nd.len[b];
            n_nr = nruns[b];
// ... 701 lines not shown
        bool first = true;
        for (int q = pos0; q < src_end; q = step <= src_end - q ? q + step : src_end) {
            const int j = q + g < src_end ? q + g : last_src;
            const int b = BYKEY ? (int) reinterpret_cast<const uint32_t *>(store)[(size_t) j * (4 * EQ) + 4 * EQ - 3]
                                : (LIST ? (int) min((uint32_t) src_list[j], (uint32_t) nd.n - 1u) : j);
            const bool dfr = gl == 0 && q + g < src_end && !(first && g < cur) && (run_w[(size_t) b * (2 * CL_RMAX) + 1] >> 24) != 0u;
            defer_rows(dfr, b);
            first = false;
        }
    }
    flush_defer();
    st_rec = wave_sum_u64(st_rec);
    if (lane == 0 && st_rec) atomicAdd(&o.counters[CNT_VALID_RECORDS], (unsigned long long) st_rec);
    if (STATS) {
        st_raw = wave_sum_u64(st_raw); st_slots = wave_sum_u64(st_slots); st_win = wave_sum_u64(st_win); st_cmp = wave_sum_u64(st_cmp);
        if (lane == 0) {
            atomicAdd(&o.counters[CNT_RAW], (unsigned long long) st_raw);
            atomicAdd(&o.counters[CNT_SLOTS], (unsigned long long) st_slots);
            atomicAdd(&o.counters[CNT_WINDOWS], (unsigned long long) st_win);
            atomicAdd(&o.counters[CNT_TR_COMPARES], (unsigned long long) st_cmp);
            atomicAdd(&o.counters[CNT_ROUNDS], (unsigned long long) st_rounds);
        }
    }
}

bool cluster_plan(const PrefSufCfg &cfg, int max_len, uint64_t live, int bucket_log2_bias, ClusterCfg *c, int *eq) {
    const int W = blocks_of(max_len);
    int e = (W + 3 + 3) / 4;
    if (e < 2) e = 2;
    const int nwin = max_len - cfg.Lmin + 1;
    if (e > CL_MAX_EQ || nwin < 1 || nwin > 128) return false;
    int kk = std::min(32, std::max(cfg.Lmin - 63, std::min(cfg.Lmin, CL_KMIN)));
    const int nw_half = std::min(nwin, 64);
    if (nw_half > std::min(cfg.Lmin - kk + 1, 64)) kk = cfg.Lmin - nw_half + 1;
    if (kk < CL_KMIN_HARD || kk > 32 || kk > cfg.Lmin) return false;
    c->kk = kk;
    c->w = std::min(cfg.Lmin - kk + 1, 64);
    c->lo_mask = kk >= 16 ? 0xFFFFFFFFu : ((1u << (2 * kk)) - 1u);
    c->hi_mask = kk <= 16 ? 0u : (kk >= 32 ? 0xFFFFFFFFu : ((1u << (2 * kk - 32)) - 1u));
    int bits = 4;
    while (bits < 28 && (1ull << bits) < live) bits++;
    bits = std::max(4, std::min(32 - CL_MBITS, bits + bucket_log2_bias));
    c->n_buckets = 1u << bits;
    c->idx_shift = 32 - bits;
    *eq = e;
    return true;
}

size_t cluster_sort_temp_bytes(uint64_t n) { return sort_u32_pairs_temp_bytes(n); }

void launch_cluster_keys(const NodesDev &nd, const PrefSufCfg &cfg, const ClusterCfg &cc, int32_t node_begin, int32_t node_end, uint32_t *keys, uint32_t *vals,
                         uint32_t *meta, void *runs, uint8_t *nruns, hipStream_t s, bool with_runs, const unsigned long long *only_if_declined) {
    if (node_end <= node_begin) return;
    const uint64_t m = (uint64_t) (node_end - node_begin);
    const unsigned long long *gate = only_if_declined;
    const dim3 grid((unsigned) (gate ? std::min<uint64_t>((m + TK_ROWS - 1) / TK_ROWS, 8192) : (m + TK_ROWS - 1) / TK_ROWS)), block(TK_ROWS);
    const int32_t *nol = nullptr; const unsigned long long *noc = nullptr;
#define NR_LAUNCH(TKW, WIDE) do { if (with_runs) hipLaunchKernelGGL((k_node_runs<TKW, WIDE, true>), grid, block, 0, s, nd, cfg, cc, (int) node_begin, (int) node_end, keys, vals, meta, (uint2 *) runs, nruns, nol, noc, gate); \
                                  else hipLaunchKernelGGL((k_node_runs<TKW, WIDE, false>), grid, block, 0, s, nd, cfg, cc, (int) node_begin, (int) node_end, keys, vals, meta, (uint2 *) runs, nruns, nol, noc, gate); } while (0)
    if (blocks_of(cfg.Lcap - 1) > 13 || (cfg.Lcap - 1) - cfg.Lmin + 1 > 64) NR_LAUNCH(21, true);
    else if (blocks_of(cfg.Lcap - 1) <= 9) NR_LAUNCH(11, false);
    else NR_LAUNCH(17, false);
#undef NR_LAUNCH
}

void launch_cluster_runs_list(const NodesDev &nd, const PrefSufCfg &cfg, const ClusterCfg &cc, const int32_t *ids, const unsigned long long *count, uint32_t cap, uint32_t grid_blocks,
                              void *runs, uint8_t *nruns, hipStream_t s) {
    if (cap == 0 || nd.n <= 0) return;
    const dim3 grid(std::max<uint32_t>(1u, std::min<uint32_t>(grid_blocks, (cap + TK_ROWS - 1) / TK_ROWS))), block(TK_ROWS);
    uint32_t *nok = nullptr;
#define NR_LAUNCH(TKW, WIDE) hipLaunchKernelGGL((k_node_runs<TKW, WIDE, true>), grid, block, 0, s, nd, cfg, cc, 0, (int) cap, nok, nok, nok, (uint2 *) runs, nruns, ids, count, (const unsigned long long *) nullptr)
    if (blocks_of(cfg.Lcap - 1) > 13 || (cfg.Lcap - 1) - cfg.Lmin + 1 > 64) NR_LAUNCH(21, true);
    else if (blocks_of(cfg.Lcap - 1) <= 9) NR_LAUNCH(11, false);
    else NR_LAUNCH(17, false);
#undef NR_LAUNCH
}

__global__ void __launch_bounds__(256) k_iota(uint32_t *__restrict__ v, uint32_t n) {
    for (uint32_t i = blockIdx.x * 256u + threadIdx.x; i < n; i += gridDim.x * 256u) v[i] = i;
}

hipError_t launch_cluster_store(const NodesDev &nd, const ClusterCfg &cc, uint32_t *keys, uint32_t *vals, uint32_t *keys2, uint32_t *vals2,
                                void *sort_temp, size_t sort_temp_bytes, void *dir, bool fill_vals,
                                hipEvent_t ev_sorted, unsigned long long *bad_flag, bool test_skip_sort, hipStream_t s, bool own_sort) {
    const hipError_t err = launch_cluster_sort(nd, cc, keys, vals, keys2, vals2, sort_temp, sort_temp_bytes, fill_vals, ev_sorted, test_skip_sort, s, own_sort);
    return err != hipSuccess ? err : launch_cluster_dir(nd, cc, keys2, dir, bad_flag, nullptr, s);
}

hipError_t launch_cluster_sort(const NodesDev &nd, const ClusterCfg &cc, uint32_t *keys, uint32_t *vals, uint32_t *keys2, uint32_t *vals2, void *sort_temp, size_t sort_temp_bytes,
                               bool fill_vals, hipEvent_t ev_sorted, bool test_skip_sort, hipStream_t s, bool own_sort) {
    if (nd.n <= 0) return hipSuccess;
    const uint64_t n = (uint64_t) nd.n;
    if (fill_vals && (!own_sort || test_skip_sort)) hipLaunchKernelGGL(k_iota, dim3((unsigned) std::min<uint64_t>((n + 255) / 256, 8192)), dim3(256), 0, s, vals, (uint32_t) n);
    hipError_t err = hipSuccess;
    if (test_skip_sort) {
        err = hipMemcpyAsync(keys2, keys, n * sizeof(uint32_t), hipMemcpyDeviceToDevice, s);
        if (err == hipSuccess) err = hipMemcpyAsync(vals2, vals, n * sizeof(uint32_t), hipMemcpyDeviceToDevice, s);
    } else err = sort_u32_pairs(sort_temp, sort_temp_bytes, keys, keys2, own_sort ? (const uint32_t *) nullptr : vals, vals2, n, cc.idx_shift - 3, s, own_sort);
    if (err != hipSuccess) return err;
    if (ev_sorted) (void) hipEventRecord(ev_sorted, s);
    return hipSuccess;
}

constexpr int DF_UNROLL = 4;
__global__ void __launch_bounds__(256) k_dir_fill(uint4 *__restrict__ dir, uint64_t n_rec, const unsigned long long *__restrict__ pile_cnt) {
    if (pile_cnt && pile_cnt_pure(pile_cnt)) return;
    const uint4 z = make_uint4(0u, 0u, 0u, 0u);
    for (uint64_t p = (uint64_t) blockIdx.x * (256u * DF_UNROLL); p < n_rec; p += (uint64_t) gridDim.x * (256u * DF_UNROLL)) {
#pragma unroll
        for (int u = 0; u < DF_UNROLL; u++) {
            const uint64_t i = p + (uint64_t) u * 256u + threadIdx.x;
            if (i < n_rec) dir[i] = z;
        }
    }
}

hipError_t launch_cluster_dir(const NodesDev &nd, const ClusterCfg &cc, const uint32_t *keys2, void *dir, unsigned long long *bad_flag, const unsigned long long *only_if_no_pure_piles,
                              hipStream_t s) {
    if (nd.n <= 0) return hipSuccess;
    const uint64_t n = (uint64_t) nd.n, n_rec = (uint64_t) cc.n_buckets + 2;
    if (only_if_no_pure_piles)
        hipLaunchKernelGGL(k_dir_fill, dim3((unsigned) std::min<uint64_t>((n_rec + 256 * DF_UNROLL - 1) / (256 * DF_UNROLL), 1u << 17)), dim3(256), 0, s, (uint4 *) dir, n_rec,
                           only_if_no_pure_piles);
    else {
        const hipError_t err = hipMemsetAsync(dir, 0, n_rec * 16, s);
        if (err != hipSuccess) return err;
    }
    hipLaunchKernelGGL(k_tgt_dir, dim3((unsigned) ((n + 1 + TD_TILE - 1) / TD_TILE)), dim3(TD_TILE), 0, s, keys2, n, cc.idx_shift, cc.n_buckets, 0u, (uint4 *) dir, bad_flag, only_if_no_pure_piles);
    return hipGetLastError();
}

hipError_t launch_cluster_gather(const NodesDev &nd, const ClusterCfg &cc, int eq, const uint32_t *keys2, const uint32_t *vals2, const uint32_t *meta, int uniform_len,
                                 void *store, const unsigned long long *pile_cnt, hipStream_t s) {
    if (nd.n <= 0) return hipSuccess;
    const uint64_t n = (uint64_t) nd.n;
    const uint64_t pieces = n * (uint64_t) eq;
    const unsigned g = (unsigned) std::min<uint64_t>((pieces + 255) / 256, 1u << 16);
    const int fs = cc.idx_shift - CL_MBITS;
    const uint32_t um = uniform_len > 0 ? (((uint32_t) uniform_len << 8) | CL_META_FROM) : 0u;
#define TG_LAUNCH(E, U) hipLaunchKernelGGL((k_tgt_gather<E, U>), dim3(g), dim3(256), 0, s, nd, n, keys2, vals2, meta, um, fs, (uint4 *) store, pile_cnt)
#define TG_EQ(E) do { if (uniform_len > 0) TG_LAUNCH(E, true); else TG_LAUNCH(E, false); } while (0)
    if (eq == 2)      TG_EQ(2);
    else if (eq == 3) TG_EQ(3);
    else if (eq == 4) TG_EQ(4);
    else              TG_EQ(5);
#undef TG_EQ
#undef TG_LAUNCH
    return hipGetLastError();
}

hipError_t launch_cluster_store_slice(const NodesDev &nd, const ClusterCfg &cc, int eq, uint64_t m, uint32_t bucket_base, uint32_t n_buckets_local, uint32_t *keys,
                                      uint32_t *vals, uint32_t *keys2, uint32_t *vals2, const uint32_t *meta, int uniform_len, void *sort_temp, size_t sort_temp_bytes,
                                      void *store, void *dir, unsigned long long *bad_flag, hipStream_t s, bool own_sort) {
    hipError_t err = hipMemsetAsync(dir, 0, ((size_t) n_buckets_local + 2) * 16, s);
    if (err != hipSuccess || m == 0) return err;
    err = sort_u32_pairs(sort_temp, sort_temp_bytes, keys, keys2, vals, vals2, m, cc.idx_shift - 3, s, own_sort);
    if (err != hipSuccess) return err;
    const uint64_t n = m, pieces = m * (uint64_t) eq;
    const unsigned g = (unsigned) ((pieces + 255) / 256);
    const int fs = cc.idx_shift - CL_MBITS;
    const uint32_t um = uniform_len > 0 ? (((uint32_t) uniform_len << 8) | CL_META_FROM) : 0u;
#define TG_LAUNCH(E, U) hipLaunchKernelGGL((k_tgt_gather<E, U>), dim3(g), dim3(256), 0, s, nd, n, (const uint32_t *) keys2, (const uint32_t *) vals2, meta, um, fs, (uint4 *) store, (const unsigned long long *) nullptr)
#define TG_EQ(E) do { if (uniform_len > 0) TG_LAUNCH(E, true); else TG_LAUNCH(E, false); } while (0)
    if (eq == 2)      TG_EQ(2);
    else if (eq == 3) TG_EQ(3);
    else if (eq == 4) TG_EQ(4);
    else              TG_EQ(5);
#undef TG_EQ
#undef TG_LAUNCH
    hipLaunchKernelGGL(k_tgt_dir, dim3((unsigned) ((n + 1 + TD_TILE - 1) / TD_TILE)), dim3(TD_TILE), 0, s, (const uint32_t *) keys2, n, cc.idx_shift, n_buckets_local, bucket_base,
                       (uint4 *) dir, bad_flag, (const unsigned long long *) nullptr);
    return hipGetLastError();
}

uint64_t cluster_probe_blocks(int n_cu, uint64_t n_src) {
    return std::max<uint64_t>(1, std::min<uint64_t>((n_src + PROBE_WAVES - 1) / PROBE_WAVES, (uint64_t) std::max(1, n_cu) * CL_OCC));
}

uint64_t cluster_record_slack(int n_cu, uint64_t n_src) { return cluster_probe_blocks(n_cu, n_src) * PROBE_WAVES * (uint64_t) REC_CHUNK_LOCAL; }

void launch_probe_stream(const NodesDev &nd, const PrefSufCfg &cfg, const ClusterCfg &cc, int eq, const void *store, const void *dir,
                         const void *runs, const uint8_t *nruns, int32_t src_begin, int32_t src_end, bool by_key, unsigned long long *counters, int n_cu,
                         uint32_t *deg, unsigned long long *first, unsigned long long *second, int32_t *defer_list, uint32_t defer_cap,
                         const unsigned long long *pile_cnt, hipStream_t s, uint32_t slot_stride) {
    const int64_t ns = (int64_t) src_end - src_begin;
    if (ns <= 0) return;
    const uint64_t quads = ((uint64_t) ns + 3) / 4;
    const int kf = (2 * cfg.Lmin) >> 5;
    const int kfs = (eq == 3 && (kf == 5 || kf == 3)) || (eq == 2 && kf == 3) ? kf : 0;
    dim3 grid((unsigned) std::max<uint64_t>(1, std::min<uint64_t>((quads + PROBE_WAVES - 1) / PROBE_WAVES, (uint64_t) std::max(1, n_cu) * clq_occ(eq <= 3 ? eq : 4, kfs, by_key)))),
         block(PROBE_WAVES * 64);
    ProbeOut o{nullptr, nullptr, 0, counters, deg, first, by_key ? 0 : src_begin, second};
    o.slot_stride = slot_stride;
    const uint4 *st = (const uint4 *) store;
#define CLQ_LAUNCH(ST, E, K, BK) hipLaunchKernelGGL((k_probe_stream<ST, E, K, BK>), grid, block, 0, s, nd, cfg, cc, st, (const uint4 *) dir, (const uint2 *) runs, nruns, src_begin, src_end, o, defer_list, defer_cap, pile_cnt, \
                                                    (const int32_t *) nullptr, (const unsigned long long *) nullptr, ByIdEntries{nullptr, nullptr, 0u, nullptr, BucketIndex{nullptr, 0u}})
#define CLQ_ORDER(ST, E, K) do { if (by_key) CLQ_LAUNCH(ST, E, K, true); else CLQ_LAUNCH(ST, E, K, false); } while (0)
#define CLQ_STATS(E, K) do { if (cfg.stats) CLQ_ORDER(true, E, K); else CLQ_ORDER(false, E, K); } while (0)
    if (eq == 3 && kf == 5)      CLQ_STATS(3, 5);
    else if (eq == 3 && kf == 3) CLQ_STATS(3, 3);
    else if (eq == 2 && kf == 3) CLQ_STATS(2, 3);
    else if (eq == 2)            CLQ_STATS(2, 0);
    else if (eq == 3)            CLQ_STATS(3, 0);
    else                         CLQ_STATS(4, 0);
#undef CLQ_STATS
#undef CLQ_ORDER
#undef CLQ_LAUNCH
}

__global__ void __launch_bounds__(256) k_defer_swap(const unsigned long long *__restrict__ pile_cnt, unsigned long long *__restrict__ counters, const int32_t *__restrict__ list2,
                                                     int32_t *__restrict__ list, uint32_t cap, bool pure_too ) {
    if (!(pile_cnt_mixed(pile_cnt) || (pure_too && !pile_cnt_declines(pile_cnt)))) return;
    const uint64_t n2 = min(counters[CNT_DEFERRED2], (unsigned long long) cap);
    for (uint64_t i = (uint64_t) blockIdx.x * blockDim.x + threadIdx.x; i < n2; i += (uint64_t) gridDim.x * blockDim.x) list[i] = list2[i];
    if (blockIdx.x == 0 && threadIdx.x == 0) { counters[CNT_DEFERRED_PILE] = counters[CNT_DEFERRED]; counters[CNT_DEFERRED] = n2; }
}

bool launch_probe_stream_list(const NodesDev &nd, const PrefSufCfg &cfg, const ClusterCfg &cc, int eq, const void *store, const void *dir, const void *runs, const uint8_t *nruns,
                              int32_t *src_list, uint32_t list_cap, unsigned long long *counters, int n_cu, uint32_t *deg, unsigned long long *first,
                              unsigned long long *second, int32_t *defer2, const unsigned long long *pile_cnt, hipStream_t s, uint32_t slot_stride, int32_t src_base,
                              const uint32_t *skeys, const uint32_t *sids, int uniform_len, bool by_id, const void *tab, uint32_t epoch) {
    if (eq != 3 || list_cap == 0) return false;
    const int kf = (2 * cfg.Lmin) >> 5;
    const int kfs = (kf == 5 || kf == 3) ? kf : 0;
    const dim3 grid((unsigned) std::max(1, n_cu) * clq_occ(3, kfs, false)), block(PROBE_WAVES * 64);
    ProbeOut o{nullptr, nullptr, 0, counters, deg, first, src_base, second};
    o.slot_stride = slot_stride;
    const bool pure_too = by_id && skeys && sids && uniform_len > 0 && nd.n > 0;
    const ByIdEntries by{skeys, sids, uniform_len > 0 ? (((uint32_t) uniform_len << 8) | CL_META_FROM) : 0u, pile_cnt, BucketIndex{(const uint4 *) tab, epoch}};
#define CLQ_LIST(K, BI) hipLaunchKernelGGL((k_probe_stream<false, 3, K, false, true, BI>), grid, block, 0, s, nd, cfg, cc, (const uint4 *) store, (const uint4 *) dir, (const uint2 *) runs, nruns, 0, \
                                           (int32_t) std::min<uint32_t>(list_cap, 0x7FFFFFFFu), o, defer2, list_cap, pile_cnt, (const int32_t *) src_list, (const unsigned long long *) (counters + CNT_DEFERRED), by)
#define CLQ_BOTH(K) do { CLQ_LIST(K, false); if (pure_too) CLQ_LIST(K, true); } while (0)
    if (kf == 5) CLQ_BOTH(5); else if (kf == 3) CLQ_BOTH(3); else CLQ_BOTH(0);
#undef CLQ_BOTH
#undef CLQ_LIST
    hipLaunchKernelGGL(k_defer_swap, dim3(1024), dim3(256), 0, s, pile_cnt, counters, (const int32_t *) defer2, src_list, list_cap, pure_too);
    return pure_too;
}

void launch_probe_clustered(const NodesDev &nd, const PrefSufCfg &cfg, const ClusterCfg &cc, int eq, const void *store, const void *dir,
                            const void *runs, const uint8_t *nruns, int32_t src_begin, int32_t src_end, const int32_t *src_list, int32_t src_base,
                            uint32_t *rec_dst, unsigned long long *rec_val, uint64_t rec_cap,
                            unsigned long long *counters, int n_cu, uint32_t *deg, unsigned long long *first, const ProbeBig *big,
                            const unsigned long long *list_count, int sw , hipStream_t s,
                            const uint32_t *skeys, const uint32_t *sids, int uniform_len, const unsigned long long *pile_cnt, const void *tab, uint32_t epoch) {
    const int64_t ns = (int64_t) src_end - src_begin;
    if (ns <= 0) return;
    dim3 grid((unsigned) cluster_probe_blocks(n_cu, (uint64_t) ns)), block(PROBE_WAVES * 64);
    ProbeOut o{rec_dst, rec_val, rec_cap, counters, deg, first, src_base};
    if (big) { o.big_list = big->list; o.big_list_cap = big->list_cap; }
    const uint4 *st = (const uint4 *) store;
    const bool maybe_by_id = pile_cnt && skeys && sids && uniform_len > 0 && eq == 3 && sw == 1 && !cfg.stats;
    const ByIdEntries by{skeys, sids, uniform_len > 0 ? (((uint32_t) uniform_len << 8) | CL_META_FROM) : 0u, maybe_by_id ? pile_cnt : nullptr, BucketIndex{(const uint4 *) tab, epoch}};
    const int kf = (2 * cfg.Lmin) >> 5;
// ... 27 lines not shown
```

alga_amd/csrc/prefsuf_kernels.h:

```cpp
#pragma once
#include <hip/hip_runtime.h>
#include <stddef.h>
#include <stdint.h>
#include "prefsuf_common.h"

namespace alga {

struct alga_edge_dev { int32_t src, dst, offset; };

void launch_restride(const uint32_t *in, int stride_in, uint32_t *out, int stride_out, uint64_t n, hipStream_t s);
void launch_widen_len(const void *in, int elem_bytes , int32_t *out, uint64_t n, hipStream_t s);
void launch_compact_edges(const alga_edge_dev *edges, int32_t n, uint64_t n_edges, uint8_t *deg, uint32_t *dst, uint8_t *off, unsigned long long *bad, hipStream_t s);
void launch_expand_twins(const uint32_t *in, int stride_in, const int32_t *len , uint32_t *out, int stride_out, uint64_t n_pairs, hipStream_t s);
void launch_node_stats(const NodesDev &nd, unsigned long long *counters, int *max_len , hipStream_t s);

uint32_t seed_buckets_for(uint64_t live_nodes, int fill_x10);
uint32_t seed_filter_bits_for(uint64_t live_nodes);
void launch_seed_build(const NodesDev &nd, const PrefSufCfg &cfg, unsigned long long *table, uint32_t n_buckets, uint32_t *filter,
                       uint32_t filter_bits, hipStream_t s);

struct ProbeBig { int32_t *list; uint32_t list_cap; uint32_t count; void *items; uint32_t item_cap; };
int    local_item_capacity();
int    local_big_limit();
size_t probe_big_bytes(int n_cu, uint32_t count, int local, uint32_t item_cap);

void launch_probe(const NodesDev &nd, const PrefSufCfg &cfg, const unsigned long long *table, uint32_t n_buckets,
                  const uint32_t *filter, uint32_t filter_bits, int32_t src_begin, int32_t src_end, uint32_t *rec_dst, unsigned long long *rec_val, uint64_t rec_cap,
                  unsigned long long *counters, int n_cu, int local , uint32_t *deg , unsigned long long *first ,
                  const ProbeBig *big , hipStream_t s);
uint64_t probe_record_slack(int n_cu, uint64_t n_src, bool local);
void launch_local_emit(int32_t src_base, int32_t n_src, const uint32_t *deg, const unsigned long long *first, const unsigned long long *second,
                       const uint32_t *rec_dst, const unsigned long long *rec_val, uint64_t n_rec, uint32_t *rowptr, uint32_t *cursor,
                       alga_edge_dev *edges, const int32_t *record_sources, const unsigned long long *record_sources_count, uint32_t record_sources_cap, hipStream_t s, uint32_t slot_stride = 0,
                       uint64_t *fused_scratch = nullptr, const unsigned long long *pile_cnt = nullptr);

bool       cluster_plan(const PrefSufCfg &cfg, int max_len, uint64_t live, int bucket_log2_bias, ClusterCfg *c, int *eq);
size_t     cluster_sort_temp_bytes(uint64_t n);
void       launch_cluster_keys(const NodesDev &nd, const PrefSufCfg &cfg, const ClusterCfg &cc, int32_t node_begin, int32_t node_end, uint32_t *keys,
                               uint32_t *vals, uint32_t *meta, void *runs, uint8_t *nruns, hipStream_t s, bool with_runs = true ,
                               const unsigned long long *only_if_declined = nullptr );
void       launch_cluster_runs_list(const NodesDev &nd, const PrefSufCfg &cfg, const ClusterCfg &cc, const int32_t *ids, const unsigned long long *count, uint32_t cap,
                                    uint32_t grid_blocks, void *runs, uint8_t *nruns, hipStream_t s);
hipError_t launch_cluster_store(const NodesDev &nd, const ClusterCfg &cc, uint32_t *keys, uint32_t *vals, uint32_t *keys2 , uint32_t *vals2, void *sort_temp,
                                size_t sort_temp_bytes, void *dir, bool fill_vals, hipEvent_t ev_sorted ,
                                unsigned long long *bad_flag ,
                                bool test_skip_sort , hipStream_t s, bool own_sort = true);
hipError_t launch_cluster_sort(const NodesDev &nd, const ClusterCfg &cc, uint32_t *keys, uint32_t *vals, uint32_t *keys2, uint32_t *vals2, void *sort_temp, size_t sort_temp_bytes,
                               bool fill_vals, hipEvent_t ev_sorted, bool test_skip_sort, hipStream_t s, bool own_sort = true);
hipError_t launch_cluster_dir(const NodesDev &nd, const ClusterCfg &cc, const uint32_t *keys2, void *dir, unsigned long long *bad_flag, const unsigned long long *only_if_no_pure_piles,
                              hipStream_t s);
hipError_t launch_cluster_gather(const NodesDev &nd, const ClusterCfg &cc, int eq, const uint32_t *keys2, const uint32_t *vals2, const uint32_t *meta,
                                 int uniform_len , void *store,
                                 const unsigned long long *pile_cnt , hipStream_t s);
uint64_t   cluster_record_slack(int n_cu, uint64_t n_src);
void       launch_probe_clustered(const NodesDev &nd, const PrefSufCfg &cfg, const ClusterCfg &cc, int eq, const void *store, const void *dir,
                                  const void *runs, const uint8_t *nruns, int32_t src_begin, int32_t src_end, const int32_t *src_list, int32_t src_base, uint32_t *rec_dst, unsigned long long *rec_val, uint64_t rec_cap,
                                  unsigned long long *counters, int n_cu, uint32_t *deg, unsigned long long *first, const ProbeBig *big,
                                  const unsigned long long *list_count ,
                                  int sw , hipStream_t s,
                                  const uint32_t *skeys = nullptr, const uint32_t *sids = nullptr, int uniform_len = 0,
                                  const unsigned long long *pile_cnt = nullptr ,
                                  const void *tab = nullptr , uint32_t epoch = 0);
void       launch_probe_stream(const NodesDev &nd, const PrefSufCfg &cfg, const ClusterCfg &cc, int eq, const void *store, const void *dir,
                               const void *runs, const uint8_t *nruns, int32_t src_begin, int32_t src_end, bool by_key ,
                               unsigned long long *counters, int n_cu, uint32_t *deg, unsigned long long *first, unsigned long long *second, int32_t *defer_list,
                               uint32_t defer_cap, const unsigned long long *pile_cnt ,
                               hipStream_t s, uint32_t slot_stride = 0 );
void       launch_pile_deg(int32_t n, unsigned long long *first, uint32_t *deg, const unsigned long long *pile_cnt, hipStream_t s);
bool       pile_plan(const PrefSufCfg &cfg, const ClusterCfg &cc, int eq, int uniform_len, bool masks);
size_t     pile_record_bytes(uint64_t n);
size_t     pile_table_bytes(uint32_t n_buckets);
void       launch_pile_sample(const NodesDev &nd, const ClusterCfg &cc, int uniform_len, const uint32_t *skeys , const uint32_t *sids , const void *dir,
                              unsigned long long *pile_cnt , int no_sample, hipStream_t s,
                              bool from_keys = false );
constexpr int PILE_CNT_WORDS = 6;
size_t     pile_own_mask_bytes(uint64_t n);
size_t     pile_list_bytes(uint64_t n);
void       launch_pile_build(const NodesDev &nd, const PrefSufCfg &cfg, const ClusterCfg &cc, int uniform_len, const uint32_t *skeys, const uint32_t *sids, const void *dir, void *rec,
                             void *rec2 , void *tab, uint32_t epoch, void *side, const void *runs, int nwin, const unsigned long long *pile_cnt,
                             uint32_t *own_mask ,
                             void *plist , hipStream_t s,
                             bool from_keys = false , unsigned long long *bad_flag = nullptr,
                             bool full_record = false ,
                             bool runs_ahead = false );
void       launch_pile_own_ids(const uint32_t *own_mask, const uint32_t *sids, uint64_t n_entries, int32_t *list, uint32_t cap, unsigned long long *pile_cnt, hipStream_t s);
void       launch_pile_check(const void *side, uint64_t n_entries, uint32_t n_buckets, const void *tab, const void *rec2, uint32_t epoch, const void *runs, int n_nodes, int nwin,
                             unsigned long long *pile_cnt, hipStream_t s);
bool       launch_probe_stream_list(const NodesDev &nd, const PrefSufCfg &cfg, const ClusterCfg &cc, int eq, const void *store, const void *dir, const void *runs, const uint8_t *nruns,
                                    int32_t *src_list, uint32_t list_cap, unsigned long long *counters, int n_cu, uint32_t *deg, unsigned long long *first,
                                    unsigned long long *second, int32_t *defer2, const unsigned long long *pile_cnt, hipStream_t s, uint32_t slot_stride = 0,
                                    int32_t src_base = 0 ,
                                    const uint32_t *skeys = nullptr, const uint32_t *sids = nullptr, int uniform_len = 0, bool by_id = false,
                                    const void *tab = nullptr , uint32_t epoch = 0);
void       launch_pile_probe(const NodesDev &nd, const PrefSufCfg &cfg, const ClusterCfg &cc, int uniform_len, const void *tab, uint32_t epoch, const void *rec, const void *rec2, const void *side,
                             const void *runs, unsigned long long *counters, uint32_t *deg, unsigned long long *first, unsigned long long *second, int32_t *defer_list,
                             uint32_t defer_cap, const unsigned long long *pile_cnt, int n_cu, hipStream_t s, int32_t src_begin, int32_t src_end,
                             void *side_range , unsigned long long *cursor ,
                             bool lean = true , bool tail = false );

size_t     rsort_u32_pairs_temp_bytes(uint64_t n);
void       rsort_set_variant(int v);
hipError_t rsort_u32_pairs(void *temp, size_t temp_bytes, const uint32_t *keys_in, uint32_t *keys_out, const uint32_t *vals_in, uint32_t *vals_out, uint64_t n,
                           int begin_bit, hipStream_t s);
size_t     sort_u32_pairs_temp_bytes(uint64_t n);
hipError_t sort_u32_pairs(void *temp, size_t temp_bytes, const uint32_t *keys_in, uint32_t *keys_out, const uint32_t *vals_in, uint32_t *vals_out,
                          uint64_t n, int begin_bit , hipStream_t s, bool own_sort = true );
size_t     rsort_u64_pairs_temp_bytes(uint64_t n);
hipError_t rsort_u64_pairs(void *temp, size_t temp_bytes, const unsigned long long *keys_in, unsigned long long *keys_out, const unsigned long long *vals_in,
                           unsigned long long *vals_out, uint64_t n, int bits, hipStream_t s);
hipError_t rsort_u32_u64(void *temp, size_t temp_bytes, const uint32_t *keys_in, uint32_t *keys_out, const unsigned long long *vals_in, unsigned long long *vals_out,
                         uint64_t n, int begin_bit, int end_bit, hipStream_t s);
size_t     sort_u64_pairs_temp_bytes(uint64_t n, int bits);
hipError_t sort_u64_pairs(void *temp, size_t temp_bytes, const unsigned long long *keys_in, unsigned long long *keys_out,
                          const unsigned long long *vals_in, unsigned long long *vals_out, uint64_t n, int bits, hipStream_t s);

void launch_make_keys(const uint32_t *rec_dst, uint64_t n_rec, int32_t dst_begin, int32_t dst_end, uint32_t *keys,
                      unsigned long long *n_valid, hipStream_t s);
size_t     sort_records_temp_bytes(uint64_t n, int bits);
hipError_t sort_records(void *temp, size_t temp_bytes, const uint32_t *keys_in, uint32_t *keys_out, const unsigned long long *vals_in,
                        unsigned long long *vals_out, uint64_t n, int bits, hipStream_t s);
void launch_rowptr_from_sorted(const uint32_t *keys, const unsigned long long *n_valid_ptr, uint64_t n_rec_max, int32_t n_owned,
                               uint32_t *rowptr, hipStream_t s);

size_t   scan_scratch_bytes(uint64_t n);
uint64_t scan_total_index(uint64_t n);
void launch_exclusive_scan(const uint32_t *in, uint64_t n, uint32_t *out, uint64_t *scratch, hipStream_t s);
void launch_exclusive_scan_pile_deg(uint32_t *deg, uint64_t n, uint32_t *out, uint64_t *scratch, unsigned long long *first, const unsigned long long *pile_cnt, hipStream_t s);
constexpr int MAIL_SEGS = 6;
struct MailSeg { const uint32_t *src; uint32_t words, dst; };
struct MailArgs {
    MailSeg seg[MAIL_SEGS];
    int n = 0;
    void add(const void *src, uint32_t words, uint32_t dst_word) { seg[n].src = (const uint32_t *) src; seg[n].words = words; seg[n].dst = dst_word; n++; }
};
void launch_mail(const MailArgs &a, uint32_t *host_block_dev, hipStream_t s);

int  reduce_targets_per_block(uint64_t n_records, uint64_t n_targets);
void launch_gather_heads(const NodesDev &nd, const unsigned long long *seg_val, const unsigned long long *n_valid_ptr, uint64_t n_rec_max,
                         void *heads , hipStream_t s);
void launch_reduce_targets(const NodesDev &nd, const PrefSufCfg &cfg, int32_t dst_begin, int32_t n_owned, int32_t targets_per_block,
                           const uint32_t *rowptr, unsigned long long *seg_val, const void *heads, uint32_t *out_cnt, uint32_t *outdeg,
                           unsigned long long *counters, hipStream_t s);
void launch_scatter_by_source(const PrefSufCfg &cfg, int32_t dst_begin, int32_t n_owned, const uint32_t *rowptr,
                              const unsigned long long *seg_val, const uint32_t *out_cnt, const uint32_t *out_rowptr, uint32_t *out_cursor,
                              alga_edge_dev *edges, hipStream_t s);
void launch_sort_rows(int32_t n, const uint32_t *out_rowptr, alga_edge_dev *edges, hipStream_t s);

void launch_edges_to_keys(const alga_edge_dev *e, uint64_t n, unsigned long long *keys, uint32_t *vals, hipStream_t s);
void launch_keys_to_edges(const unsigned long long *keys, const uint32_t *vals, uint64_t n, alga_edge_dev *e, hipStream_t s);
size_t     sort_edges_temp_bytes(uint64_t n);
hipError_t sort_edges(void *temp, size_t temp_bytes, const unsigned long long *keys_in, unsigned long long *keys_out, const uint32_t *vals_in,
                      uint32_t *vals_out, uint64_t n, int src_bits, hipStream_t s);

}
```

alga_amd/csrc/prefsuf_pile.hip:

```cpp
#include <hip/hip_runtime.h>
#include <algorithm>
#include "prefsuf_common.h"
#include "prefsuf_kernels.h"
#include "prefsuf_device.h"
#include "prefsuf_cluster_device.h"

namespace alga {

constexpr int PB_TILE = 192, PB_HALO = 64, PB_THREADS = PB_TILE + PB_HALO;
constexpr int PILE_SW = 13;
constexpr int PILE_MAXSUB = 4;
constexpr int PILE_EQ = 3;

__device__ __forceinline__ bool pile_declines(const unsigned long long *pile_cnt) { return pile_cnt_declines(pile_cnt); }

__device__ __forceinline__ uint32_t pile_who(uint32_t group, uint32_t w, uint32_t n_buckets, uint64_t n_entries) {
    return group == 0u ? min(w, n_buckets) : (uint32_t) min((uint64_t) w, n_entries) | 0x80000000u;
}

__device__ __forceinline__ void load_row9(const NodesDev &nd, uint32_t id, uint32_t (&row)[9]) {
    const uint32_t *rp = nd.words + (size_t) id * nd.stride;
    if ((nd.stride & 3) == 0 && nd.stride >= 12 && ((uintptr_t) nd.words & 15u) == 0) {
        const uint4 v0 = reinterpret_cast<const uint4 *>(rp)[0], v1 = reinterpret_cast<const uint4 *>(rp)[1];
        row[0] = v0.x; row[1] = v0.y; row[2] = v0.z; row[3] = v0.w; row[4] = v1.x; row[5] = v1.y; row[6] = v1.z; row[7] = v1.w;
        row[8] = rp[8];
    } else {
#pragma unroll
        for (int k = 0; k < 9; k++) row[k] = k < nd.stride ? rp[k] : 0u;
    }
}

template <bool SAMPLE, bool KEYS>
__global__ void __launch_bounds__(PB_THREADS, 6) k_pile_build(NodesDev nd, const uint32_t *__restrict__ skeys, const uint32_t *__restrict__ sids, uint64_t n_entries, const uint4 *__restrict__ dir, ClusterCfg cc, int U,
                                                           uint4 *__restrict__ rec, uint4 *__restrict__ tab, uint32_t epoch,
                                                           uint4 *__restrict__ side, unsigned long long *__restrict__ pile_cnt, uint32_t *__restrict__ own_mask,
                                                           uint32_t *__restrict__ plist, uint32_t *__restrict__ pcount, unsigned long long *__restrict__ bad,
                                                           uint32_t full_record) {
    if (!SAMPLE && pile_declines(pile_cnt)) return;
    const int idx_shift = cc.idx_shift, kk = cc.kk;
    __shared__ uint32_t sRow[PB_THREADS][PILE_SW];
    __shared__ unsigned long long sKm[PB_THREADS];
    __shared__ unsigned long long sLead[PB_THREADS];
    __shared__ unsigned long long sRm[PB_THREADS];
    __shared__ uint32_t sMin[PB_THREADS], sMax[PB_THREADS];
    __shared__ uint32_t sBad[PB_THREADS];
    __shared__ uint8_t sTag[PB_THREADS];
    __shared__ uint32_t sCount[3];
    __shared__ uint32_t sPiles;
    __shared__ unsigned long long sMask[KEYS ? PB_THREADS / 64 : 1][8];
    __shared__ uint32_t sPrev;
    const int t = (int) threadIdx.x;
    const uint64_t base = (uint64_t) blockIdx.x * PB_TILE;
    const uint64_t j = base + (uint64_t) t;
    const bool have = j < n_entries;
    const uint64_t jc = have ? j : (n_entries ? n_entries - 1 : 0);
    const uint32_t key = skeys[jc], node_id = min(sids[jc], (uint32_t) nd.n - 1u);
    const uint32_t meta = key >> (cc.idx_shift - CL_MBITS);
    const bool tgt = have && key != 0xFFFFFFFFu;
    const uint32_t nb3 = cc.n_buckets << 3;
    auto tagged = [&](uint32_t x) -> uint32_t { return x == 0xFFFFFFFFu ? nb3 : x >> (idx_shift - 3); };
    uint4 drec = make_uint4(0u, 0u, 0u, 0u);
    uint32_t tg_own = 0u, tg_before = 0u, tg_look = 0u, bk_before = 0u;
    bool pre = false;
    if (KEYS) {
        tg_own = have ? tagged(key) : nb3;
        tg_before = j == 0 ? 0xFFFFFFFFu : (j - 1 < n_entries ? tagged(skeys[j - 1]) : nb3);
        if (t < 64 && base >= 64u) tg_look = tagged(skeys[min(base - 64u + (uint64_t) t, n_entries - 1)]);
        const uint64_t jl = min(base + (uint64_t) (PB_TILE - 1), n_entries - 1);
        bk_before = base == 0 ? 0x1FFFFFFFu : tagged(skeys[min(base - 1, n_entries - 1)]) >> 3;
        const uint32_t bk_last = tagged(skeys[jl]) >> 3;
        pre = tgt && (tg_own >> 3) != bk_before && (tg_own >> 3) <= bk_last;
    } else if (tgt) drec = dir[key >> idx_shift];
    uint32_t row[9] = {0u, 0u, 0u, 0u, 0u, 0u, 0u, 0u, 0u};
    if (KEYS && pre) load_row9(nd, node_id, row);
    uint64_t e0 = drec.x;
    uint32_t cnt = drec.y;
    bool owned = tgt && e0 >= base && e0 < base + PB_TILE && e0 <= j && j - e0 < (uint64_t) cnt;
    int s = owned ? (int) (e0 - base) : 0;
    int i = owned ? (int) (j - e0) : 0;
    bool part = owned && cnt <= 64u;
    bool regular = tgt && cnt <= 64u;
    if (!KEYS && part) load_row9(nd, node_id, row);
    if (KEYS) {
        const int wv = t >> 6;
        const bool first = tg_own >> 3 != tg_before >> 3;
        if (!SAMPLE && t < PB_TILE && j >= 1 && j < n_entries && tg_own < tg_before) atomicOr(bad, 1ull);
        const unsigned long long mf = __ballot(first);
        unsigned long long mc[7];
#pragma unroll
        for (int c = 1; c <= 7; c++) mc[c - 1] = __ballot((tg_own & 7u) < (uint32_t) c);
        if ((t & 63) == 0) {
            sMask[wv][0] = mf;
#pragma unroll
            for (int c = 1; c <= 7; c++) sMask[wv][c] = mc[c - 1];
        }
        if (t < 64) {
            const unsigned long long ml = __ballot(base >= 64u && (tg_look >> 3) == bk_before);
            if (t == 0) sPrev = (uint32_t) __popcll(ml);
        }
    }
    sLead[t] = 0ull; sRm[t] = 0ull; sMin[t] = 0xFFFFFFFFu; sMax[t] = 0u; sBad[t] = 0u;
    if (t < 3) sCount[t] = 0u;
    if (t == 0) sPiles = 0u;
    __syncthreads();
    const int m = (int) (meta & 63u);
    uint32_t A[PILE_SW];
    {
        const int w0 = (2 * m) >> 5, sh = (2 * m) & 31;
        const int lo = 2 * (64 - m), hi = lo + 2 * U;
        uint32_t Rp[18];
#pragma unroll
        for (int k = 0; k < 18; k++) Rp[k] = 0u;
#pragma unroll
        for (int k = 0; k < 9; k++) Rp[4 + k] = row[k];
        uint32_t m1 = 0u - (uint32_t) (w0 & 1), m2 = 0u - (uint32_t) ((w0 >> 1) & 1);
        asm volatile("" : "+v"(m1), "+v"(m2));
        uint32_t y1[PILE_SW + 3], y[PILE_SW + 1];
#pragma unroll
        for (int k = 0; k < PILE_SW + 3; k++) y1[k] = (Rp[k + 1] & m1) | (Rp[k] & ~m1);
#pragma unroll
        for (int k = 0; k <= PILE_SW; k++) y[k] = (y1[k + 2] & m2) | (y1[k] & ~m2);
#pragma unroll
        for (int k = 0; k < PILE_SW; k++) A[k] = funnel(y[k], y[k + 1], sh) & low_bits32(hi - 32 * k) & ~low_bits32(lo - 32 * k);
    }
    const unsigned long long kmask = kk >= 32 ? ~0ull : ((1ull << (2 * kk)) - 1ull);
    const unsigned long long kmer = (((unsigned long long) A[5] << 32) | A[4]) & kmask;
    sKm[t] = kmer;
#pragma unroll
    for (int k = 0; k < PILE_SW; k++) sRow[t][k] = A[k];
    __syncthreads();
    if (KEYS) {
        const int wv = t >> 6, ln = t & 63;
        int sk = -1, ek = PB_THREADS;
        {
            const unsigned long long own = sMask[wv][0];
            const unsigned long long at = own & (~0ull >> (63 - ln)), after = ln == 63 ? 0ull : own & (~0ull << (ln + 1));
            if (at) sk = wv * 64 + 63 - __clzll((long long) at);
            if (after) ek = wv * 64 + __builtin_ctzll(after);
#pragma unroll
            for (int v = 1; v < PB_THREADS / 64; v++) {
                if (sk < 0 && wv - v >= 0) { const unsigned long long mv = sMask[wv - v][0]; if (mv) sk = (wv - v) * 64 + 63 - __clzll((long long) mv); }
                if (ek == PB_THREADS && wv + v < PB_THREADS / 64) { const unsigned long long mv = sMask[wv + v][0]; if (mv) ek = (wv + v) * 64 + __builtin_ctzll(mv); }
            }
        }
        owned = tgt && sk >= 0 && sk < PB_TILE;
        s = owned ? sk : 0;
        i = owned ? t - sk : 0;
        cnt = owned ? (uint32_t) (ek - sk) : 0u;
        e0 = base + (uint64_t) s;
        part = owned && pre && cnt <= 64u;
        regular = tgt && (sk >= 0 ? cnt <= 64u : sPrev + (uint32_t) ek <= 64u);
        drec.x = (uint32_t) e0;
    }
    auto class_offsets = [&]() -> unsigned long long {
        const int last = s + (int) cnt - 1, w0 = s >> 6, w1 = last >> 6;
        const unsigned long long r0 = (~0ull << (s & 63)) & (w1 == w0 ? ~0ull >> (63 - (last & 63)) : ~0ull);
        const unsigned long long r1 = w1 == w0 ? 0ull : ~0ull >> (63 - (last & 63));
        unsigned long long acc = 0ull;
#pragma unroll
        for (int c = 1; c <= 7; c++)
            acc |= (unsigned long long) (__popcll(sMask[KEYS ? w0 : 0][c] & r0) + __popcll(sMask[KEYS ? w1 : 0][c] & r1)) << (8 * c);
        return acc;
    };
    int L = t;
    if (part) {
        for (int u = 0; u < i; u++) if (sKm[s + u] == kmer) { L = s + u; break; }
        if (L == t) {
            atomicOr(&sLead[s], 1ull << i);
            sTag[t] = (uint8_t) (cluster_key(kmer_hash((uint32_t) kmer & cc.lo_mask, (uint32_t) (kmer >> 32) & cc.hi_mask), idx_shift - CL_MBITS) & 31u);
        }
        atomicMin(&sMin[L], ((uint32_t) m << 16) | (uint32_t) t);
        atomicMax(&sMax[L], ((uint32_t) m << 16) | (uint32_t) t);
        const unsigned long long bit = 1ull << (63 - m);
        if (atomicOr(&sRm[L], bit) & bit) atomicOr(&sBad[s], 1u);
    }
    __syncthreads();
    uint32_t *sSlot = reinterpret_cast<uint32_t *>(sKm);
    int my_slot = -1, my_rank = 0;
    if (part) {
        const unsigned long long lm = sLead[s];
        const int kgrp = __popcll(lm & ((1ull << (L - s)) - 1ull));
        if (kgrp < PILE_MAXSUB) {
            int before = 0;
            unsigned long long rest = lm;
#pragma unroll
            for (int g = 0; g < PILE_MAXSUB - 1; g++) {
                if (g < kgrp) { before += __popcll(sRm[s + __builtin_ctzll(rest)]); rest &= rest - 1ull; }
            }
            my_rank = m == 0 ? 0 : __popcll(sRm[L] >> (64 - m));
            my_slot = s + before + my_rank;
            if (my_slot < s + (int) cnt) sSlot[my_slot] = node_id; else my_slot = -1;
        }
    }
    uint32_t S[PILE_SW];
#pragma unroll
    for (int k = 0; k < PILE_SW; k++) S[k] = 0u;
    if (part) {
        const int t0 = (int) (sMax[L] & 0xFFFFu), t1 = (int) (sMin[L] & 0xFFFFu);
        const int lo = 2 * (64 - m), hi = lo + 2 * U;
        uint32_t diff = 0u;
#pragma unroll
        for (int k = 0; k < PILE_SW; k++) {
            S[k] = sRow[t0][k] | sRow[t1][k];
            diff |= (A[k] ^ S[k]) & low_bits32(hi - 32 * k) & ~low_bits32(lo - 32 * k);
        }
        if (diff != 0u) atomicOr(&sBad[s], 1u);
    }
    __syncthreads();
    if (owned) {
        uint4 *line = tab + (size_t) (key >> idx_shift) * 8;
        if (!part) {
            if (i == 0) {
                if (!SAMPLE) {
                    uint32_t cz = drec.z, cw = drec.w;
                    if (KEYS && full_record) {
                        const uint32_t b3 = tg_own & ~7u;
                        auto lower = [&](uint64_t lo, uint64_t hi, uint32_t tv) -> uint64_t {
                            while (lo < hi) { const uint64_t mid = lo + ((hi - lo) >> 1); if (tagged(skeys[mid]) < tv) lo = mid + 1; else hi = mid; }
                            return lo;
                        };
                        uint64_t hi = min(j + 256u, n_entries);
                        while (hi < n_entries && tagged(skeys[hi]) < b3 + 8u) hi = min(j + 2u * (hi - j), n_entries);
                        const uint64_t end = lower(j + 1u, hi, b3 + 8u);
                        unsigned long long co = 0ull;
                        for (uint32_t c = 1; c <= 7u; c++) co |= (unsigned long long) min(lower(j, end, b3 + c) - j, (uint64_t) 255u) << (8u * c);
                        cz = (uint32_t) co; cw = (uint32_t) (co >> 32);
                        line[5] = make_uint4((uint32_t) min(end - j, (uint64_t) 0xFFFFFFFFu), 0u, 0u, 0u);
                    }
                    line[3] = make_uint4(0u, 0u, 0u, (1u << 22) | (epoch << 23));
                    line[4] = make_uint4(127u, drec.x, cz, cw);
                }
                atomicAdd(&sCount[0], 1u); atomicAdd(&sCount[1], 1u);
            }
        } else {
            const unsigned long long lm = sLead[s];
            const int nsub = __popcll(lm);
            const int iL = L - s;
            const int k = __popcll(lm & ((1ull << iL) - 1ull));
            if (!SAMPLE) {
                const unsigned long long right = m == 0 ? 0ull : (sRm[L] >> (64 - m));
                uint32_t succ_id = 0xFFFFFFFFu, delta = 0u;
                if (right != 0ull && my_slot > s && my_rank >= 1) { succ_id = sSlot[my_slot - 1]; delta = 1u + (uint32_t) __builtin_ctzll(right); }
                const bool first_group = (k == 0 || own_mask != nullptr) && k < PILE_MAXSUB && sBad[s] == 0u && nsub <= PILE_MAXSUB;
                const bool leftmost = first_group && t == (int) (sMax[L] & 0xFFFFu);
                side[j] = make_uint4(node_id, succ_id, delta | ((uint32_t) m << 8) | ((uint32_t) k << 16) | (leftmost ? 0x40000000u : 0u) | (first_group ? 0x80000000u : 0u),
                                     k == 0 ? key >> idx_shift : (uint32_t) (e0 + (uint64_t) k));
                if (leftmost && plist) plist[(size_t) blockIdx.x * PB_THREADS + atomicAdd(&sPiles, 1u)] = pile_who((uint32_t) k, k == 0 ? key >> idx_shift : (uint32_t) (e0 + (uint64_t) k), cc.n_buckets, n_entries);
                if (!first_group && own_mask) atomicOr(&own_mask[j >> 5], 1u << (j & 31u));
            }
            if (!SAMPLE && L == t && k >= 1 && k < PILE_MAXSUB) {
                const unsigned long long rm = sRm[t];
                const uint64_t slot = e0 + (uint64_t) k;
                rec[slot * 4 + 0] = make_uint4(S[0], S[1], S[2], S[3]);
                rec[slot * 4 + 1] = make_uint4(S[4], S[5], S[6], S[7]);
                rec[slot * 4 + 2] = make_uint4(S[8], S[9], S[10], S[11]);
                rec[slot * 4 + 3] = make_uint4(S[12], 0u, (uint32_t) rm, (uint32_t) (rm >> 32));
            }
            if (i == 0) {
                uint32_t tg[PILE_MAXSUB] = {0u, 0u, 0u, 0u};
                unsigned long long rest = lm;
#pragma unroll
                for (int g = 0; g < PILE_MAXSUB; g++) {
                    if (rest) { tg[g] = sTag[s + __builtin_ctzll(rest)]; rest &= rest - 1ull; }
                }
                const bool irregular = sBad[s] != 0u || nsub > PILE_MAXSUB;
                const uint32_t ns1 = (uint32_t) (nsub < PILE_MAXSUB ? nsub : PILE_MAXSUB) - 1u;
                if (!SAMPLE) {
                    const unsigned long long rm = sRm[t];
                    line[0] = make_uint4(S[0], S[1], S[2], S[3]);
                    line[1] = make_uint4(S[4], S[5], S[6], S[7]);
                    line[2] = make_uint4(S[8], S[9], S[10], S[11]);
                    line[3] = make_uint4(S[12], (uint32_t) rm, (uint32_t) (rm >> 32), tg[0] | (tg[1] << 5) | (tg[2] << 10) | (tg[3] << 15) | (ns1 << 20) | (irregular ? 1u << 22 : 0u) | (epoch << 23));
                }
                atomicAdd(&sCount[0], 1u);
                if (irregular) atomicAdd(&sCount[1], 1u);
            }
            if (!SAMPLE && L == s && t == (int) (sMax[s] & 0xFFFFu)) {
                if (KEYS) { const unsigned long long co = class_offsets(); drec.z = (uint32_t) co; drec.w = (uint32_t) (co >> 32); }
                line[4] = make_uint4(cnt, drec.x, drec.z, drec.w);
                line[5] = make_uint4(sSlot[s], sMin[s] >> 16, 0u, 0u);
            }
        }
    }
    if (!SAMPLE && have && t < PB_TILE && !regular) {
        side[j] = make_uint4(node_id, 0xFFFFFFFFu, 0u, 0u);
        if (own_mask) atomicOr(&own_mask[j >> 5], 1u << (j & 31u));
    }
    if (SAMPLE && owned) atomicAdd(&sCount[2], 1u);
    __syncthreads();
    if (!SAMPLE && plist && t == 0) pcount[blockIdx.x] = sPiles;
    if (SAMPLE && t < 3 && sCount[t]) atomicAdd(&pile_cnt[t], (unsigned long long) sCount[t]);
}

constexpr int PILE_RUNS = 8;
__device__ __forceinline__ void pile_list_store(uint4 *line, uint32_t entries, bool ok, int n, const uint32_t (&key)[PILE_RUNS], const uint32_t (&kc)[PILE_RUNS], uint32_t c1_last) {
    uint32_t *lw = reinterpret_cast<uint32_t *>(line);
    if (ok) {
        line[5] = make_uint4(key[0], key[1], key[2], key[3]);
        line[6] = make_uint4(key[4], key[5], key[6], key[7]);
        line[7] = make_uint4(kc[0] | (kc[1] << 16), kc[2] | (kc[3] << 16), kc[4] | (kc[5] << 16), kc[6] | (kc[7] << 16));
        bool dup = false;
#pragma unroll
        for (int a = 0; a < PILE_RUNS; a++)
#pragma unroll
            for (int b = a + 1; b < PILE_RUNS; b++) dup = dup || (b < n && key[a] == key[b]);
        lw[16] = (entries & 255u) | ((uint32_t) n << 8) | ((c1_last & 255u) << 16) | (dup ? 0x80000000u : 0u);
    } else lw[16] = entries & 255u;
}

__global__ void __launch_bounds__(256) k_pile_runs(const uint4 *__restrict__ side, uint64_t n_entries, uint32_t n_buckets, uint4 *__restrict__ tab, const uint2 *__restrict__ runs,
                                                   int n_nodes, int nwin, const unsigned long long *__restrict__ pile_cnt) {
    if (pile_declines(pile_cnt)) return;
    const uint64_t j = (uint64_t) blockIdx.x * 256 + threadIdx.x;
    if (j >= n_entries) return;
    const uint4 sd = side[j];
    if (((sd.z >> 30) & 1u) == 0u) return;
    uint4 *line = tab + (size_t) min(sd.w, n_buckets) * 8;
    const uint4 l4 = line[4], l5 = line[5];
    const uint4 *r0 = reinterpret_cast<const uint4 *>(runs + (size_t) min(sd.x, (uint32_t) n_nodes - 1u) * CL_RMAX);
    const uint4 *r1 = reinterpret_cast<const uint4 *>(runs + (size_t) min(l5.x, (uint32_t) n_nodes - 1u) * CL_RMAX);
    const uint4 a0 = r0[0], a1 = r0[1], a2 = r0[2], a3 = r0[3], b0 = r1[0], b1 = r1[1], b2 = r1[2];
    const int s0 = -(int) ((sd.z >> 8) & 63u), s1 = -(int) (l5.y & 63u), seam = s0 + nwin;
    const uint32_t k0[CL_RMAX] = {a0.x, a0.z, a1.x, a1.z, a2.x, a2.z, a3.x, a3.z}, y0[CL_RMAX] = {a0.y, a0.w, a1.y, a1.w, a2.y, a2.w, a3.y, a3.w};
    const uint32_t k1[6] = {b0.x, b0.z, b1.x, b1.z, b2.x, b2.z}, y1[6] = {b0.y, b0.w, b1.y, b1.w, b2.y, b2.w};
    const int nr0 = (int) (y0[0] >> 24), nr1 = (int) (y1[0] >> 24);
    bool ok = nr0 >= 1 && nr0 <= CL_RMAX && nr1 >= 1 && nr1 <= 6 && s1 <= seam;
    uint32_t ok_[PILE_RUNS], kc_[PILE_RUNS];
#pragma unroll
    for (int k = 0; k < PILE_RUNS; k++) { ok_[k] = 0u; kc_[k] = 0u; }
    int n = 0;
    uint32_t last_key = 0u, last_pos = 0xFFFFFFFFu, c1_last = 0u;
#pragma unroll
    for (int r = CL_RMAX - 1; r >= 0; r--) {
        if (ok && r < nr0) {
            const uint32_t kpos = (uint32_t) (s0 + (int) (y0[r] & 255u) + 64), c0 = (uint32_t) (s0 + (int) ((y0[r] >> 8) & 255u) + 64), c1 = (uint32_t) (s0 + (int) ((y0[r] >> 16) & 255u) + 64);
#pragma unroll
            for (int k = 0; k < PILE_RUNS; k++) if (k == n) { ok_[k] = k0[r]; kc_[k] = kpos | (c0 << 8); }
            last_key = k0[r]; last_pos = kpos; c1_last = c1;
            n++;
        }
    }
#pragma unroll
    for (int r = 5; r >= 0; r--) {
        if (ok && r < nr1) {
            const int c1i = s1 + (int) ((y1[r] >> 16) & 255u);
            if (c1i > seam) {
                const int c0i = max(s1 + (int) ((y1[r] >> 8) & 255u), seam);
                const uint32_t kpos = (uint32_t) (s1 + (int) (y1[r] & 255u) + 64), c1 = (uint32_t) (c1i + 64);
                if (n >= 1 && k1[r] == last_key && kpos == last_pos) c1_last = c1;
                else {
#pragma unroll
                    for (int k = 0; k < PILE_RUNS; k++) if (k == n) { ok_[k] = k1[r]; kc_[k] = kpos | ((uint32_t) (c0i + 64) << 8); }
                    last_key = k1[r]; last_pos = kpos; c1_last = c1;
                    n++;
                }
            }
        }
    }
    ok = ok && n >= 1 && n <= PILE_RUNS;
    pile_list_store(line, l4.x, ok, n, ok_, kc_, c1_last);
}

constexpr int PR_TILE = 3072;
constexpr int PR_TKW = 21;
constexpr int PR_RCAP = 14;
constexpr int PR_SEGS = 32;

__device__ __forceinline__ void pile_consensus_load(uint32_t who, const uint4 *__restrict__ tab, const uint4 *__restrict__ rec, uint4 &l0, uint4 &l1, uint4 &l2, uint4 &l3, uint32_t &w16) {
    const bool further = (who >> 31) != 0u;
    const uint4 *src = further ? rec + (size_t) (who & 0x7FFFFFFFu) * 4 : tab + (size_t) who * 8;
    l0 = src[0]; l1 = src[1]; l2 = src[2]; l3 = src[3];
    w16 = reinterpret_cast<const uint32_t *>(src)[further ? 0 : 16];
}

// ... 618 lines not shown
                for (int i = 0; i < PP_TAIL_K; i++) {
                    const uint4 *c1 = side + min((uint64_t) dd1.y + e1 + (uint32_t) i, last), *c2 = side + min((uint64_t) dd2.y + e2 + (uint32_t) i, last);
                    cx1[i] = c1->x; cz1[i] = c1->z; cx2[i] = c2->x; cz2[i] = c2->z;
                }
                static_assert(PP_TAIL_K == 4, "the batch is pinned word by word");
                asm volatile("" : "+v"(cx1[0]), "+v"(cz1[0]), "+v"(cx1[1]), "+v"(cz1[1]), "+v"(cx1[2]), "+v"(cz1[2]), "+v"(cx1[3]), "+v"(cz1[3]),
                                  "+v"(cx2[0]), "+v"(cz2[0]), "+v"(cx2[1]), "+v"(cz2[1]), "+v"(cx2[2]), "+v"(cz2[2]), "+v"(cx2[3]), "+v"(cz2[3]));
#pragma unroll
                for (int i = 0; i < PP_TAIL_K; i++) {
                    if (e1 + (uint32_t) i < e1_end && (int) ((cz1[i] >> 8) & 63u) == mm1 && ((cz1[i] >> 16) & 3u) == g1) lk_id1 = cx1[i];
                    if (e2 + (uint32_t) i < e2_end && (int) ((cz2[i] >> 8) & 63u) == mm2 && ((cz2[i] >> 16) & 3u) == g2) lk_id2 = cx2[i];
                }
                e1 += PP_TAIL_K; e2 += PP_TAIL_K;
            } while (__ballot(e1 < e1_end || e2 < e2_end) != 0ull);
        }
    }
    unsigned long long slot_val = LOCAL_FIRST_NONE;
    if (active && !dfr && nkept > 0) {
        const int d1 = __builtin_ctzll(kept);
        int p1_home = 0;
#pragma unroll
        for (int k = 0; k < CL_RMAX; k++) p1_home = (((vmask >> k) & 1u) != 0u && ((ry[k] >> 8) & 255u) == 0u) ? (int) ((ry[k] >> 16) & 255u) : p1_home;
        const bool by_succ = d1 < p1_home && (int) (my.z & 255u) == d1 && my.y != 0xFFFFFFFFu;
        const uint32_t id1 = by_succ ? my.y : (TAIL ? lk_id1 : lookup(d1));
        uint32_t id2 = 0u;
        int d2 = 0;
        bool two = false;
        if (nkept == 2) {
            d2 = 63 - __clzll((long long) kept);
            id2 = TAIL ? lk_id2 : lookup(d2);
            const int ds0 = U - cfg.rsoemo + 1;
            const unsigned long long lowm = ds0 <= 0 ? 0ull : (ds0 >= 64 ? ~0ull : ((1ull << ds0) - 1ull));
            two = d2 < ds0 || __popcll(occ & ((1ull << d2) - 1ull) & ~lowm) < 3;
        }
        if (id1 == 0xFFFFFFFFu || (nkept == 2 && id2 == 0xFFFFFFFFu)) dfr = true;
        else {
            slot_val = ((unsigned long long) id1 << 32) | (uint32_t) d1 | (two ? 0x100u : 0u);
            if (two) o.second[Bs - o.src_base] = ((unsigned long long) id2 << 32) | (uint32_t) d2;
            st_rec += two ? 2 : 1;
        }
    }
    if (have) o.first[Bs - o.src_base] = slot_val;
    dfr = dfr && nr_code != 0;
    const uint64_t dm = __ballot(dfr);
    if (dm != 0ull) {
        if (dfr) sDefer[wave][n_defer + (int) __builtin_amdgcn_mbcnt_hi((uint32_t) (dm >> 32), __builtin_amdgcn_mbcnt_lo((uint32_t) dm, 0u))] = Bs;
        n_defer += __popcll(dm);
        wave_lds_fence();
        if (n_defer >= 64) flush_defer();
    }
    }
    flush_defer();
    st_rec = wave_sum_u64(st_rec);
    if (lane == 0 && st_rec) atomicAdd(&o.counters[CNT_VALID_RECORDS], (unsigned long long) st_rec);
}

__global__ void __launch_bounds__(256) k_pile_deg(int32_t n, unsigned long long *__restrict__ first, uint32_t *__restrict__ deg, const unsigned long long *__restrict__ pile_cnt) {
    if (pile_declines(pile_cnt)) return;
    const int64_t i = (int64_t) blockIdx.x * 256 + threadIdx.x;
    if (i >= n) return;
    const unsigned long long f = first[i];
    if (f == LOCAL_FIRST_NONE || deg[i] != 0u) return;
    deg[i] = 1u + (uint32_t) ((f >> 8) & 1ull);
    if (f & 0x100ull) first[i] = f & ~0x100ull;
}

bool pile_plan(const PrefSufCfg &cfg, const ClusterCfg &cc, int eq, int uniform_len, bool masks) {
    if (eq != PILE_EQ || uniform_len <= 0 || masks || cfg.stats) return false;
    if (uniform_len > 144 || blocks_of(uniform_len) > 9) return false;
    if (uniform_len - cfg.Lmin + 1 > 64 || cc.w > 64 || cc.w < 16 || cc.kk > 32 || cc.kk < 1) return false;
    return true;
}
size_t pile_record_bytes(uint64_t n) { return (size_t) (n + 2) * 64; }

size_t pile_table_bytes(uint32_t n_buckets) { return ((size_t) n_buckets + 2) * 128; }

__global__ void k_pile_sample_close(unsigned long long *__restrict__ pile_cnt) {
    const unsigned long long by_entries = pile_cnt[2] / 8ull;
    if (by_entries > pile_cnt[0]) pile_cnt[0] = by_entries;
}

__global__ void k_pile_sample_force(unsigned long long *__restrict__ pile_cnt, unsigned long long buckets, unsigned long long irregular) { pile_cnt[0] = buckets; pile_cnt[1] = irregular; }

void launch_pile_sample(const NodesDev &nd, const ClusterCfg &cc, int uniform_len, const uint32_t *skeys, const uint32_t *sids, const void *dir, unsigned long long *pile_cnt,
                        int no_sample, hipStream_t s, bool from_keys) {
    (void) hipMemsetAsync(pile_cnt, 0, PILE_CNT_WORDS * sizeof(unsigned long long), s);
    const uint64_t n_entries = nd.n > 0 ? (uint64_t) nd.n : 0;
    if (no_sample == 2) hipLaunchKernelGGL(k_pile_sample_force, dim3(1), dim3(1), 0, s, pile_cnt, 100ull, 1ull);
    if (n_entries == 0 || no_sample) return;
    const uint64_t tiles = (n_entries + PB_TILE - 1) / PB_TILE;
    const dim3 sample((unsigned) std::max<uint64_t>(1, std::min<uint64_t>(tiles, std::max<uint64_t>(64, tiles / 32)))), block(PB_THREADS);
    hipLaunchKernelGGL((from_keys ? k_pile_build<true, true> : k_pile_build<true, false>), sample, block, 0, s, nd, skeys, sids, n_entries, (const uint4 *) dir, cc, uniform_len, (uint4 *) nullptr,
                       (uint4 *) nullptr, 0u, (uint4 *) nullptr, pile_cnt, (uint32_t *) nullptr, (uint32_t *) nullptr, (uint32_t *) nullptr, (unsigned long long *) nullptr, 0u);
    hipLaunchKernelGGL(k_pile_sample_close, dim3(1), dim3(1), 0, s, pile_cnt);
}

void launch_pile_build(const NodesDev &nd, const PrefSufCfg &cfg, const ClusterCfg &cc, int uniform_len, const uint32_t *skeys, const uint32_t *sids, const void *dir, void *rec, void *rec2,
                       void *tab, uint32_t epoch, void *side, const void *runs, int nwin, const unsigned long long *pile_cnt, uint32_t *own_mask, void *plist, hipStream_t s,
                       bool from_keys, unsigned long long *bad_flag, bool full_record, bool runs_ahead) {
    const uint64_t n_entries = nd.n > 0 ? (uint64_t) nd.n : 0;
    if (n_entries == 0) return;
    const uint64_t tiles = (n_entries + PB_TILE - 1) / PB_TILE;
    if (!own_mask) plist = nullptr;
    uint32_t *pl = (uint32_t *) plist, *pc = pl ? pl + tiles * PB_THREADS : nullptr;
    if (own_mask) (void) hipMemsetAsync(own_mask, 0, pile_own_mask_bytes(n_entries), s);
    hipLaunchKernelGGL((from_keys ? k_pile_build<false, true> : k_pile_build<false, false>), dim3((unsigned) tiles), dim3(PB_THREADS), 0, s, nd, skeys, sids, n_entries, (const uint4 *) dir, cc, uniform_len,
                       (uint4 *) rec, (uint4 *) tab, epoch, (uint4 *) side, const_cast<unsigned long long *>(pile_cnt), own_mask, pl, pc, bad_flag, full_record ? 1u : 0u);
    if (pl)
        hipLaunchKernelGGL(k_pile_runs_consensus_list, dim3((unsigned) ((tiles + PR_SEGS - 1) / PR_SEGS)), dim3(TK_ROWS), 0, s, (const uint32_t *) pl, (const uint32_t *) pc, (uint32_t) tiles,
                           (const uint4 *) side, n_entries, (uint4 *) tab, (const uint4 *) rec, (uint4 *) rec2, cc, uniform_len, cfg.Lmin, pile_cnt, own_mask, runs_ahead ? 1 : 0);
    else if (own_mask)
        hipLaunchKernelGGL(k_pile_runs_consensus, dim3((unsigned) ((n_entries + PR_TILE - 1) / PR_TILE)), dim3(TK_ROWS), 0, s, (const uint4 *) side, n_entries, cc.n_buckets, (uint4 *) tab,
                           (const uint4 *) rec, (uint4 *) rec2, cc, uniform_len, cfg.Lmin, pile_cnt, own_mask);
    else
        hipLaunchKernelGGL(k_pile_runs, dim3((unsigned) ((n_entries + 255) / 256)), dim3(256), 0, s, (const uint4 *) side, n_entries, cc.n_buckets, (uint4 *) tab, (const uint2 *) runs, nd.n, nwin, pile_cnt);
}

size_t pile_own_mask_bytes(uint64_t n) { return (size_t) ((n + 31) / 32 + 1024) * 4; }

size_t pile_list_bytes(uint64_t n) { const uint64_t tiles = (n + PB_TILE - 1) / PB_TILE; return (size_t) (tiles * (PB_THREADS + 1) + 64) * 4; }

void launch_pile_own_ids(const uint32_t *own_mask, const uint32_t *sids, uint64_t n_entries, int32_t *list, uint32_t cap, unsigned long long *pile_cnt, hipStream_t s) {
    if (n_entries == 0) return;
    const uint64_t words = (n_entries + 31) / 32;
    hipLaunchKernelGGL(k_pile_own_ids, dim3((unsigned) ((words + 1023) / 1024)), dim3(256), 0, s, own_mask, sids, n_entries, list, cap, pile_cnt + 3, (const unsigned long long *) pile_cnt);
}

void launch_pile_check(const void *side, uint64_t n_entries, uint32_t n_buckets, const void *tab, const void *rec2, uint32_t epoch, const void *runs, int n_nodes, int nwin,
                       unsigned long long *pile_cnt, hipStream_t s) {
    if (n_entries == 0) return;
    hipLaunchKernelGGL(k_pile_list_check, dim3((unsigned) ((n_entries + 255) / 256)), dim3(256), 0, s, (const uint4 *) side, n_entries, n_buckets, (const uint4 *) tab, (const uint4 *) rec2, epoch,
                       (const uint2 *) runs,
                       n_nodes, nwin, pile_cnt + 4, (const unsigned long long *) pile_cnt);
}

constexpr int PSR_IPT = 4;
__global__ void __launch_bounds__(256) k_pile_side_range(const uint4 *__restrict__ side, uint64_t n_entries, uint32_t src_begin, uint32_t src_end, uint4 *__restrict__ out,
                                                         uint64_t out_cap, unsigned long long *__restrict__ cursor, const unsigned long long *__restrict__ pile_cnt) {
    if (pile_declines(pile_cnt)) return;
    __shared__ uint32_t cnt[PSR_IPT * 4];
    __shared__ unsigned long long base;
    const int wave = (int) (threadIdx.x >> 6);
    const uint64_t b0 = (uint64_t) blockIdx.x * (256 * PSR_IPT);
    uint4 v[PSR_IPT];
    uint32_t before[PSR_IPT];
    bool in[PSR_IPT];
#pragma unroll
    for (int k = 0; k < PSR_IPT; k++) {
        const uint64_t j = b0 + (uint64_t) k * 256 + threadIdx.x;
        v[k] = j < n_entries ? side[j] : make_uint4(0xFFFFFFFFu, 0u, 0u, 0u);
        in[k] = j < n_entries && v[k].x >= src_begin && v[k].x < src_end;
        const uint64_t m = __ballot(in[k]);
        before[k] = (uint32_t) __builtin_amdgcn_mbcnt_hi((uint32_t) (m >> 32), __builtin_amdgcn_mbcnt_lo((uint32_t) m, 0u));
        if ((threadIdx.x & 63u) == 0u) cnt[k * 4 + wave] = (uint32_t) __popcll(m);
    }
    __syncthreads();
    if (threadIdx.x == 0) {
        uint32_t tot = 0;
        for (int i = 0; i < PSR_IPT * 4; i++) tot += cnt[i];
        base = tot ? atomicAdd(cursor, (unsigned long long) tot) : 0ull;
    }
    __syncthreads();
    uint32_t run = 0;
#pragma unroll
    for (int k = 0; k < PSR_IPT; k++) {
        uint32_t mine = run;
        for (int w = 0; w < 4; w++) { if (w < wave) mine += cnt[k * 4 + w]; run += cnt[k * 4 + w]; }
        const unsigned long long at = base + mine + before[k];
        if (in[k] && at < out_cap) out[at] = v[k];
    }
}

void launch_pile_probe(const NodesDev &nd, const PrefSufCfg &cfg, const ClusterCfg &cc, int uniform_len, const void *tab, uint32_t epoch, const void *rec, const void *rec2,
                       const void *side, const void *runs, unsigned long long *counters, uint32_t *deg, unsigned long long *first, unsigned long long *second,
                       int32_t *defer_list, uint32_t defer_cap, const unsigned long long *pile_cnt, int n_cu, hipStream_t s, int32_t src_begin, int32_t src_end,
                       void *side_range, unsigned long long *cursor, bool lean, bool tail) {
    const uint64_t n_entries = nd.n > 0 ? (uint64_t) nd.n : 0;
    if (n_entries == 0 || src_end <= src_begin) return;
    ProbeOut o{};
    o.counters = counters; o.deg = deg; o.first = first; o.second = second; o.src_base = src_begin;
    uint64_t n_mine = n_entries;
    const void *side_src = side;
    if (src_begin != 0 || src_end != nd.n) {
        n_mine = (uint64_t) (src_end - src_begin);
        (void) hipMemsetAsync(cursor, 0, sizeof(unsigned long long), s);
        hipLaunchKernelGGL(k_pile_side_range, dim3((unsigned) ((n_entries + 256 * PSR_IPT - 1) / (256 * PSR_IPT))), dim3(256), 0, s, (const uint4 *) side, n_entries,
                           (uint32_t) src_begin, (uint32_t) src_end, (uint4 *) side_range, n_mine, cursor, pile_cnt);
        side_src = side_range;
    }
    const uint64_t tiles = (n_mine + PP_WAVES * 64 - 1) / (PP_WAVES * 64);
// ... 12 lines not shown
```

alga_amd/csrc/prefsuf_shard.h:

```cpp
#pragma once
#include <hip/hip_runtime.h>
#include <stdint.h>
#include "prefsuf_common.h"
#include "prefsuf_kernels.h"

namespace alga {

inline uint32_t shard_buckets_per_rank(uint32_t n_buckets, int n_ranks) { return (uint32_t) (((uint64_t) n_buckets + (uint64_t) n_ranks - 1) / (uint64_t) n_ranks); }

void launch_shard_select(const uint32_t *keys, uint32_t n, int shift, uint32_t b_lo, uint32_t b_hi, uint32_t *okeys, uint32_t *ovals, unsigned long long *cursor, hipStream_t s);
hipError_t launch_cluster_store_slice(const NodesDev &nd, const ClusterCfg &cc, int eq, uint64_t m, uint32_t bucket_base, uint32_t n_buckets_local, uint32_t *keys,
                                      uint32_t *vals, uint32_t *keys2, uint32_t *vals2, const uint32_t *meta, int uniform_len, void *sort_temp, size_t sort_temp_bytes,
                                      void *store, void *dir, unsigned long long *bad_flag, hipStream_t s, bool own_sort = true);
void launch_shard_export(bool count, const void *runs, int32_t node_begin, int32_t node_end, int shift, uint32_t bpr, uint32_t n_ranks, unsigned long long *counts,
                         int32_t *flagged_list, unsigned long long *flagged_count, uint32_t flagged_cap, const unsigned long long *seg_off, unsigned long long *cursor,
                         uint32_t *out, hipStream_t s);
void launch_shard_export_flagged(const NodesDev &nd, const PrefSufCfg &cfg, const ClusterCfg &cc, const int32_t *flagged_list, uint32_t n_flagged, uint32_t bpr, uint32_t n_ranks,
                                 const unsigned long long *seg_off, unsigned long long *cursor, uint32_t *out, hipStream_t s);
void launch_shard_desc_split(const uint32_t *in, uint64_t n, uint32_t key_base , uint32_t *dkey, unsigned long long *dval, hipStream_t s);
size_t     sort_desc_temp_bytes(uint64_t n);
hipError_t sort_desc(void *temp, size_t temp_bytes, const uint32_t *keys_in, uint32_t *keys_out, const unsigned long long *vals_in, unsigned long long *vals_out, uint64_t n,
                     int begin_bit, int end_bit, hipStream_t s, bool own_sort = true);
uint64_t shard_join_record_slack(int n_cu);
void launch_shard_groups(const uint32_t *dkey, uint64_t n_desc, int shift, uint32_t *flag, uint32_t *pos, uint32_t *gstart, uint64_t *scan_scratch, hipStream_t s);
void launch_shard_join(const NodesDev &nd, const PrefSufCfg &cfg, const ClusterCfg &cc, int eq, int uniform_len, const void *store, const void *dir, uint32_t bucket_base,
                       const uint32_t *dkey, const unsigned long long *dval, uint64_t n_desc, const uint32_t *gstart, uint32_t n_groups, uint32_t *rec_dst,
                       unsigned long long *rec_val, uint64_t rec_cap, unsigned long long *counters, unsigned long long *small_top, unsigned long long *declined,
                       int dmax , int n_cu, hipStream_t s);
void launch_shard_pending_src(const uint32_t *rec_dst, const unsigned long long *rec_val, uint64_t n_rec, uint32_t *list, uint32_t cap, unsigned long long *count, hipStream_t s);
void launch_shard_bitmap_set(const uint32_t *ids, uint64_t n, uint32_t n_nodes, uint32_t *bitmap, hipStream_t s);
void launch_shard_small_emit(const unsigned long long *dval, const unsigned long long *small_top, uint64_t n_desc, const uint32_t *bitmap, uint32_t *out, uint32_t cap,
                             unsigned long long *count, hipStream_t s);
void launch_shard_small_split(const uint32_t *in, uint64_t n, uint32_t *ssrc, unsigned long long *skey, hipStream_t s);
void launch_shard_resolve(uint32_t *rec_dst, const unsigned long long *rec_val, uint64_t n_rec, const uint32_t *ssrc, const unsigned long long *skey, uint64_t n_small,
                          unsigned long long *dropped, hipStream_t s);
void launch_shard_edges_out(bool count, const uint32_t *rec_dst, const unsigned long long *rec_val, uint64_t n_rec, uint32_t chunk, uint32_t n_ranks,
                            unsigned long long *counts, const unsigned long long *seg_off, unsigned long long *cursor, alga_edge_dev *out, hipStream_t s);
void launch_shard_place_count(const alga_edge_dev *in, uint64_t n, int32_t src_base, int32_t n_src, uint32_t *deg, unsigned long long *bad, hipStream_t s);
void launch_shard_place_fill(const alga_edge_dev *in, uint64_t n, int32_t src_base, int32_t n_src, const uint32_t *rowptr, uint32_t *cursor, alga_edge_dev *out, hipStream_t s);

}
```

Measured before the change: 5.490 billion edges/s.

## Keep sampled pile tiles as built work and bound the dir kernel grid

The pile sampling pass can now run the full build on its sampled tiles and record them, so the later pile build launch starts after those tiles and skips them. Pile sampling and its epoch setup are moved ahead of the late dir and gather launches so the kept results can be reused. Separately, the target-directory kernel becomes grid-stride and is capped at 32 workgroups per CU by default. The aim is to avoid redoing the sampled tiles and to cut launch overhead from very large grids. In exchange, the sample pass must write real records before the directory and gather steps run, so ordering and correctness now depend on the sampled tiles being the leading tile range.

```diff
diff --git a/alga_amd/csrc/engine.hip b/alga_amd/csrc/engine.hip
--- a/alga_amd/csrc/engine.hip
+++ b/alga_amd/csrc/engine.hip
@@ -194,7 +194,7 @@
             const bool dir_late = pile && e->opt_pile_dir >= 1;
             e->dir_late = dir_late;
             if (!dir_late) {
-                HIP_TRY(e, launch_cluster_dir(nd, cc, (const uint32_t *) e->cl_keys[1].p, e->cl_dir.p, cnt + CNT_TOTAL + 1, nullptr, s));
+                HIP_TRY(e, launch_cluster_dir(nd, cc, (const uint32_t *) e->cl_keys[1].p, e->cl_dir.p, cnt + CNT_TOTAL + 1, nullptr, s, alga_dir_blocks(e)));
                 HIP_TRY(e, hipEventRecord(e->ev[EV_DIR], s));
             }
             e->pile_n = -1;
@@ -216,21 +216,8 @@
                     }
                 } else if (rc) return rc;
             }
-            if (pile) {
-                launch_pile_sample(nd, cc, pp.uniform_len, (const uint32_t *) e->cl_keys[1].p, (const uint32_t *) e->cl_vals[1].p, e->cl_dir.p,
-                                   (unsigned long long *) e->cl_pile_cnt.p, e->opt_pile >= 2 ? e->opt_pile - 1 : 0, s, e->opt_pile_dir >= 1);
-                if ((rc = alga_check_launch(e, "k_pile_build<sample>"))) return rc;
-            }
             e->pile_tab_index = pile && e->opt_pile_dir >= 2 && e->opt_pile_skip_gather && !cfg.stats;
-            if (dir_late) {
-                HIP_TRY(e, hipEventRecord(e->ev[EV_SAMPLE], s));
-                HIP_TRY(e, launch_cluster_dir(nd, cc, (const uint32_t *) e->cl_keys[1].p, e->cl_dir.p, cnt + CNT_TOTAL + 1,
-                                              e->pile_tab_index ? (const unsigned long long *) e->cl_pile_cnt.p : nullptr, s));
-                HIP_TRY(e, hipEventRecord(e->ev[EV_DIR], s));
-            }
-            HIP_TRY(e, launch_cluster_gather(nd, cc, pp.cluster_eq, (const uint32_t *) e->cl_keys[1].p, (const uint32_t *) e->cl_vals[1].p, (const uint32_t *) e->cl_meta.p,
-                                             pp.uniform_len, e->cl_store.p, (pile && e->opt_pile_skip_gather) ? (const unsigned long long *) e->cl_pile_cnt.p : nullptr, s));
-            HIP_TRY(e, hipEventRecord(e->ev[EV_GATHER], s));
+            uint32_t pile_tiles_built = 0;
             if (pile) {
                 if (e->pile_epoch >= 511u) {
                     HIP_TRY(e, hipMemsetAsync(e->cl_pile_tab.p, 0, e->cl_pile_tab.cap, s));
@@ -238,10 +225,28 @@
                 }
                 e->pile_epoch++;
                 const bool from_consensus = e->opt_pile_runs != 0;
+                const PileKeep keep{e->cl_pile_rec.p, e->cl_pile_tab.p, e->pile_epoch, e->cl_pile_succ.p, from_consensus ? (uint32_t *) e->cl_pile_own.p : nullptr,
+                                    (from_consensus && e->opt_pile_runs_list) ? e->cl_pile_list.p : nullptr, cnt + CNT_TOTAL + 1, e->pile_tab_index};
+                pile_tiles_built = launch_pile_sample(nd, cc, pp.uniform_len, (const uint32_t *) e->cl_keys[1].p, (const uint32_t *) e->cl_vals[1].p, e->cl_dir.p,
+                                                      (unsigned long long *) e->cl_pile_cnt.p, e->opt_pile >= 2 ? e->opt_pile - 1 : 0, s, e->opt_pile_dir >= 1,
+                                                      e->opt_pile_sample_keep ? &keep : nullptr);
+                if ((rc = alga_check_launch(e, "k_pile_build<sample>"))) return rc;
+            }
+            if (dir_late) {
+                HIP_TRY(e, hipEventRecord(e->ev[EV_SAMPLE], s));
+                HIP_TRY(e, launch_cluster_dir(nd, cc, (const uint32_t *) e->cl_keys[1].p, e->cl_dir.p, cnt + CNT_TOTAL + 1,
+                                              e->pile_tab_index ? (const unsigned long long *) e->cl_pile_cnt.p : nullptr, s, alga_dir_blocks(e)));
+                HIP_TRY(e, hipEventRecord(e->ev[EV_DIR], s));
+            }
+            HIP_TRY(e, launch_cluster_gather(nd, cc, pp.cluster_eq, (const uint32_t *) e->cl_keys[1].p, (const uint32_t *) e->cl_vals[1].p, (const uint32_t *) e->cl_meta.p,
+                                             pp.uniform_len, e->cl_store.p, (pile && e->opt_pile_skip_gather) ? (const unsigned long long *) e->cl_pile_cnt.p : nullptr, s));
+            HIP_TRY(e, hipEventRecord(e->ev[EV_GATHER], s));
+            if (pile) {
+                const bool from_consensus = e->opt_pile_runs != 0;
                 launch_pile_build(nd, cfg, cc, pp.uniform_len, (const uint32_t *) e->cl_keys[1].p, (const uint32_t *) e->cl_vals[1].p, e->cl_dir.p, e->cl_pile_rec.p, e->cl_pile_rec2.p, e->cl_pile_tab.p,
                                   e->pile_epoch, e->cl_pile_succ.p, e->cl_runs.p, pp.uniform_len - cfg.Lmin + 1, (const unsigned long long *) e->cl_pile_cnt.p,
                                   from_consensus ? (uint32_t *) e->cl_pile_own.p : nullptr, (from_consensus && e->opt_pile_runs_list) ? e->cl_pile_list.p : nullptr, s,
-                                  e->opt_pile_dir >= 1, cnt + CNT_TOTAL + 1, e->pile_tab_index, e->opt_pile_runs_ahead != 0);
+                                  e->opt_pile_dir >= 1, cnt + CNT_TOTAL + 1, e->pile_tab_index, e->opt_pile_runs_ahead != 0, pile_tiles_built);
                 if ((rc = alga_check_launch(e, "k_pile_build"))) return rc;
                 if (keys_only) {
                     launch_pile_own_ids((const uint32_t *) e->cl_pile_own.p, (const uint32_t *) e->cl_vals[1].p, (uint64_t) nd.n, (int32_t *) e->cl_defer.p, (uint32_t) nd.n,
@@ -664,6 +669,11 @@
         e->opt_pile_probe_tail = value != 0;
     } else if (!strcmp(name, "pile_runs_ahead")) {
         e->opt_pile_runs_ahead = value != 0;
+    } else if (!strcmp(name, "dir_grid")) {
+        if (value < 0 || value > (1 << 20)) return alga_fail(e, ALGA_ERR_INVALID_ARGUMENT, "option dir_grid: 0 a workgroup per tile, 1 bounded by the chip, 2 .. 2^20 that many workgroups");
+        e->opt_dir_grid = (int) value;
+    } else if (!strcmp(name, "pile_sample_keep")) {
+        e->opt_pile_sample_keep = value != 0;
     } else if (!strcmp(name, "pile_stream_by_id")) {
         e->opt_pile_stream_by_id = value != 0;
     } else if (!strcmp(name, "pile_check")) {
diff --git a/alga_amd/csrc/engine_internal.h b/alga_amd/csrc/engine_internal.h
--- a/alga_amd/csrc/engine_internal.h
+++ b/alga_amd/csrc/engine_internal.h
@@ -66,6 +66,8 @@
     int    opt_pile_probe_lean = 1;
     int    opt_pile_probe_tail = 1;
     int    opt_pile_runs_ahead = 0;
+    int    opt_dir_grid = 1;
+    int    opt_pile_sample_keep = 1;
     bool   pile_deg_pending = false;
     int    opt_pile_check = 0;
     bool   expect_pairwise = false;
@@ -235,6 +237,9 @@
                             uint32_t **d_raw);
 int alga_prepare(alga_engine *e, const alga_nodes *nodes, const alga_prefsuf_params *p, hipStream_t s, AlgaPrepared &out);
 int alga_cluster_alloc(alga_engine *e, const AlgaPrepared &pp);
+inline uint32_t alga_dir_blocks(const alga_engine *e) {
+    return e->opt_dir_grid <= 0 ? 0u : e->opt_dir_grid == 1 ? (uint32_t) std::max(1, e->n_cu) * 32u : (uint32_t) e->opt_dir_grid;
+}
 
 inline int alga_fail(alga_engine *e, int code, const char *what, hipError_t herr = hipSuccess) {
     char buf[512];
diff --git a/alga_amd/csrc/engine_shard.hip b/alga_amd/csrc/engine_shard.hip
--- a/alga_amd/csrc/engine_shard.hip
+++ b/alga_amd/csrc/engine_shard.hip
@@ -93,7 +93,7 @@
     if ((rc = alga_ensure(e, e->sort_temp, std::max(cluster_sort_temp_bytes(m), sort_desc_temp_bytes(1))))) return rc;
     HIP_TRY(e, launch_cluster_store_slice(pp.nd, cc, pp.cluster_eq, m, b_lo, n_b_local, (uint32_t *) e->sh_keys[0].p, (uint32_t *) e->sh_vals[0].p, (uint32_t *) e->sh_keys[1].p,
                                           (uint32_t *) e->sh_vals[1].p, (const uint32_t *) e->cl_meta.p, pp.uniform_len, e->sort_temp.p, cluster_sort_temp_bytes(m),
-                                          e->sh_store.p, e->sh_dir.p, cnt + 2, s, e->opt_own_sort != 0));
+                                          e->sh_store.p, e->sh_dir.p, cnt + 2, s, e->opt_own_sort != 0, alga_dir_blocks(e)));
     e->shard_stats.ms_index = t_index.stop();
     PhaseTimer t_export(s);
     launch_shard_export(false, e->cl_runs.p, kb, ke, cc.idx_shift, bpr, (uint32_t) n_ranks, nullptr, nullptr, nullptr, 0u, cnt + 192, cnt + 128, (uint32_t *) e->sh_desc_out.p, s);
diff --git a/alga_amd/csrc/prefsuf_cluster.hip b/alga_amd/csrc/prefsuf_cluster.hip
--- a/alga_amd/csrc/prefsuf_cluster.hip
+++ b/alga_amd/csrc/prefsuf_cluster.hip
@@ -144,9 +144,12 @@
                                                      const unsigned long long *__restrict__ pile_cnt ) {
     if (pile_cnt && pile_cnt_pure(pile_cnt)) return;
     __shared__ uint32_t sb[TD_TILE + TD_HALO + 1];
-    const uint64_t base = (uint64_t) blockIdx.x * TD_TILE;
     const uint32_t nb3 = n_buckets << 3;
     auto tagged = [&](uint64_t k) -> uint32_t { if (k >= n) return nb3; const uint32_t x = keys[k]; return x == 0xFFFFFFFFu ? nb3 : (x >> (shift - 3)) - (bucket_base << 3); };
+    const uint64_t n_tiles = (n + 1 + TD_TILE - 1) / TD_TILE;
+    for (uint64_t tile = blockIdx.x; tile < n_tiles; tile += gridDim.x) {
+    if (tile != blockIdx.x) __syncthreads();
+    const uint64_t base = tile * TD_TILE;
     for (int k = (int) threadIdx.x; k <= TD_TILE + TD_HALO; k += TD_TILE)
         sb[k] = (base == 0 && k == 0) ? 0xFFFFFFFFu : tagged(base + (uint64_t) k - 1u);
     __syncthreads();
@@ -224,6 +227,7 @@
             const uint32_t c = (uint32_t) (k - j0);
             put(bb, make_uint4((uint32_t) j0, c, c <= 255u ? (uint32_t) acc : 0u, c <= 255u ? (uint32_t) (acc >> 32) : 0u));
         }
+    }
     }
 }
 
@@ -1091,9 +1095,9 @@
 
 hipError_t launch_cluster_store(const NodesDev &nd, const ClusterCfg &cc, uint32_t *keys, uint32_t *vals, uint32_t *keys2, uint32_t *vals2,
                                 void *sort_temp, size_t sort_temp_bytes, void *dir, bool fill_vals,
-                                hipEvent_t ev_sorted, unsigned long long *bad_flag, bool test_skip_sort, hipStream_t s, bool own_sort) {
+                                hipEvent_t ev_sorted, unsigned long long *bad_flag, bool test_skip_sort, hipStream_t s, bool own_sort, uint32_t dir_blocks) {
     const hipError_t err = launch_cluster_sort(nd, cc, keys, vals, keys2, vals2, sort_temp, sort_temp_bytes, fill_vals, ev_sorted, test_skip_sort, s, own_sort);
-    return err != hipSuccess ? err : launch_cluster_dir(nd, cc, keys2, dir, bad_flag, nullptr, s);
+    return err != hipSuccess ? err : launch_cluster_dir(nd, cc, keys2, dir, bad_flag, nullptr, s, dir_blocks);
 }
 
 hipError_t launch_cluster_sort(const NodesDev &nd, const ClusterCfg &cc, uint32_t *keys, uint32_t *vals, uint32_t *keys2, uint32_t *vals2, void *sort_temp, size_t sort_temp_bytes,
@@ -1124,18 +1128,26 @@
     }
 }
 
+static void launch_tgt_dir(const uint32_t *keys2, uint64_t n, int shift, uint32_t n_buckets, uint32_t bucket_base, void *dir, unsigned long long *bad_flag,
+                           const unsigned long long *pile_cnt, uint32_t dir_blocks, hipStream_t s) {
+    uint64_t g = (n + 1 + TD_TILE - 1) / TD_TILE;
+    if (dir_blocks) g = std::min<uint64_t>(g, dir_blocks);
+    hipLaunchKernelGGL(k_tgt_dir, dim3((unsigned) g), dim3(TD_TILE), 0, s, keys2, n, shift, n_buckets, bucket_base, (uint4 *) dir, bad_flag, pile_cnt);
+}
+
 hipError_t launch_cluster_dir(const NodesDev &nd, const ClusterCfg &cc, const uint32_t *keys2, void *dir, unsigned long long *bad_flag, const unsigned long long *only_if_no_pure_piles,
-                              hipStream_t s) {
+                              hipStream_t s, uint32_t dir_blocks) {
     if (nd.n <= 0) return hipSuccess;
     const uint64_t n = (uint64_t) nd.n, n_rec = (uint64_t) cc.n_buckets + 2;
-    if (only_if_no_pure_piles)
-        hipLaunchKernelGGL(k_dir_fill, dim3((unsigned) std::min<uint64_t>((n_rec + 256 * DF_UNROLL - 1) / (256 * DF_UNROLL), 1u << 17)), dim3(256), 0, s, (uint4 *) dir, n_rec,
-                           only_if_no_pure_piles);
-    else {
+    if (only_if_no_pure_piles) {
+        uint64_t g = std::min<uint64_t>((n_rec + 256 * DF_UNROLL - 1) / (256 * DF_UNROLL), 1u << 17);
+        if (dir_blocks) g = std::min<uint64_t>(g, dir_blocks);
+        hipLaunchKernelGGL(k_dir_fill, dim3((unsigned) g), dim3(256), 0, s, (uint4 *) dir, n_rec, only_if_no_pure_piles);
+    } else {
         const hipError_t err = hipMemsetAsync(dir, 0, n_rec * 16, s);
         if (err != hipSuccess) return err;
     }
-    hipLaunchKernelGGL(k_tgt_dir, dim3((unsigned) ((n + 1 + TD_TILE - 1) / TD_TILE)), dim3(TD_TILE), 0, s, keys2, n, cc.idx_shift, cc.n_buckets, 0u, (uint4 *) dir, bad_flag, only_if_no_pure_piles);
+    launch_tgt_dir(keys2, n, cc.idx_shift, cc.n_buckets, 0u, dir, bad_flag, only_if_no_pure_piles, dir_blocks, s);
     return hipGetLastError();
 }
 
@@ -1160,7 +1172,7 @@
 
 hipError_t launch_cluster_store_slice(const NodesDev &nd, const ClusterCfg &cc, int eq, uint64_t m, uint32_t bucket_base, uint32_t n_buckets_local, uint32_t *keys,
                                       uint32_t *vals, uint32_t *keys2, uint32_t *vals2, const uint32_t *meta, int uniform_len, void *sort_temp, size_t sort_temp_bytes,
-                                      void *store, void *dir, unsigned long long *bad_flag, hipStream_t s, bool own_sort) {
+                                      void *store, void *dir, unsigned long long *bad_flag, hipStream_t s, bool own_sort, uint32_t dir_blocks) {
     hipError_t err = hipMemsetAsync(dir, 0, ((size_t) n_buckets_local + 2) * 16, s);
     if (err != hipSuccess || m == 0) return err;
     err = sort_u32_pairs(sort_temp, sort_temp_bytes, keys, keys2, vals, vals2, m, cc.idx_shift - 3, s, own_sort);
@@ -1177,8 +1189,7 @@
     else              TG_EQ(5);
 #undef TG_EQ
 #undef TG_LAUNCH
-    hipLaunchKernelGGL(k_tgt_dir, dim3((unsigned) ((n + 1 + TD_TILE - 1) / TD_TILE)), dim3(TD_TILE), 0, s, (const uint32_t *) keys2, n, cc.idx_shift, n_buckets_local, bucket_base,
-                       (uint4 *) dir, bad_flag, (const unsigned long long *) nullptr);
+    launch_tgt_dir((const uint32_t *) keys2, n, cc.idx_shift, n_buckets_local, bucket_base, dir, bad_flag, nullptr, dir_blocks, s);
     return hipGetLastError();
 }
 
diff --git a/alga_amd/csrc/prefsuf_kernels.h b/alga_amd/csrc/prefsuf_kernels.h
--- a/alga_amd/csrc/prefsuf_kernels.h
+++ b/alga_amd/csrc/prefsuf_kernels.h
@@ -44,11 +44,11 @@
 hipError_t launch_cluster_store(const NodesDev &nd, const ClusterCfg &cc, uint32_t *keys, uint32_t *vals, uint32_t *keys2 , uint32_t *vals2, void *sort_temp,
                                 size_t sort_temp_bytes, void *dir, bool fill_vals, hipEvent_t ev_sorted ,
                                 unsigned long long *bad_flag ,
-                                bool test_skip_sort , hipStream_t s, bool own_sort = true);
+                                bool test_skip_sort , hipStream_t s, bool own_sort = true, uint32_t dir_blocks = 0);
 hipError_t launch_cluster_sort(const NodesDev &nd, const ClusterCfg &cc, uint32_t *keys, uint32_t *vals, uint32_t *keys2, uint32_t *vals2, void *sort_temp, size_t sort_temp_bytes,
                                bool fill_vals, hipEvent_t ev_sorted, bool test_skip_sort, hipStream_t s, bool own_sort = true);
 hipError_t launch_cluster_dir(const NodesDev &nd, const ClusterCfg &cc, const uint32_t *keys2, void *dir, unsigned long long *bad_flag, const unsigned long long *only_if_no_pure_piles,
-                              hipStream_t s);
+                              hipStream_t s, uint32_t dir_blocks = 0 );
 hipError_t launch_cluster_gather(const NodesDev &nd, const ClusterCfg &cc, int eq, const uint32_t *keys2, const uint32_t *vals2, const uint32_t *meta,
                                  int uniform_len , void *store,
                                  const unsigned long long *pile_cnt , hipStream_t s);
@@ -70,9 +70,11 @@
 bool       pile_plan(const PrefSufCfg &cfg, const ClusterCfg &cc, int eq, int uniform_len, bool masks);
 size_t     pile_record_bytes(uint64_t n);
 size_t     pile_table_bytes(uint32_t n_buckets);
-void       launch_pile_sample(const NodesDev &nd, const ClusterCfg &cc, int uniform_len, const uint32_t *skeys , const uint32_t *sids , const void *dir,
+struct PileKeep { void *rec, *tab; uint32_t epoch; void *side; uint32_t *own_mask; void *plist; unsigned long long *bad_flag; bool full_record; };
+uint32_t   launch_pile_sample(const NodesDev &nd, const ClusterCfg &cc, int uniform_len, const uint32_t *skeys , const uint32_t *sids , const void *dir,
                               unsigned long long *pile_cnt , int no_sample, hipStream_t s,
-                              bool from_keys = false );
+                              bool from_keys = false ,
+                              const PileKeep *keep = nullptr );
 constexpr int PILE_CNT_WORDS = 6;
 size_t     pile_own_mask_bytes(uint64_t n);
 size_t     pile_list_bytes(uint64_t n);
@@ -82,7 +84,8 @@
                              void *plist , hipStream_t s,
                              bool from_keys = false , unsigned long long *bad_flag = nullptr,
                              bool full_record = false ,
-                             bool runs_ahead = false );
+                             bool runs_ahead = false ,
+                             uint32_t tile0 = 0 );
 void       launch_pile_own_ids(const uint32_t *own_mask, const uint32_t *sids, uint64_t n_entries, int32_t *list, uint32_t cap, unsigned long long *pile_cnt, hipStream_t s);
 void       launch_pile_check(const void *side, uint64_t n_entries, uint32_t n_buckets, const void *tab, const void *rec2, uint32_t epoch, const void *runs, int n_nodes, int nwin,
                              unsigned long long *pile_cnt, hipStream_t s);
diff --git a/alga_amd/csrc/prefsuf_pile.hip b/alga_amd/csrc/prefsuf_pile.hip
--- a/alga_amd/csrc/prefsuf_pile.hip
+++ b/alga_amd/csrc/prefsuf_pile.hip
@@ -30,12 +30,14 @@
     }
 }
 
-template <bool SAMPLE, bool KEYS>
-__global__ void __launch_bounds__(PB_THREADS, 6) k_pile_build(NodesDev nd, const uint32_t *__restrict__ skeys, const uint32_t *__restrict__ sids, uint64_t n_entries, const uint4 *__restrict__ dir, ClusterCfg cc, int U,
-                                                           uint4 *__restrict__ rec, uint4 *__restrict__ tab, uint32_t epoch,
-                                                           uint4 *__restrict__ side, unsigned long long *__restrict__ pile_cnt, uint32_t *__restrict__ own_mask,
-                                                           uint32_t *__restrict__ plist, uint32_t *__restrict__ pcount, unsigned long long *__restrict__ bad,
-                                                           uint32_t full_record) {
+template <bool SAMPLE, bool KEYS, bool KEEP>
+__device__ __forceinline__ void pile_build_tile(const NodesDev &nd, const uint32_t *__restrict__ skeys, const uint32_t *__restrict__ sids, uint64_t n_entries, const uint4 *__restrict__ dir, const ClusterCfg &cc, int U,
+                                                uint4 *__restrict__ rec, uint4 *__restrict__ tab, uint32_t epoch,
+                                                uint4 *__restrict__ side, unsigned long long *__restrict__ pile_cnt, uint32_t *__restrict__ own_mask,
+                                                uint32_t *__restrict__ plist, uint32_t *__restrict__ pcount, unsigned long long *__restrict__ bad,
+                                                uint32_t full_record, uint32_t tile) {
+    static_assert(SAMPLE || !KEEP, "the keeping form is a sample");
+    constexpr bool WRITES = !SAMPLE || KEEP;
     if (!SAMPLE && pile_declines(pile_cnt)) return;
     const int idx_shift = cc.idx_shift, kk = cc.kk;
     __shared__ uint32_t sRow[PB_THREADS][PILE_SW];
@@ -50,7 +52,7 @@
     __shared__ unsigned long long sMask[KEYS ? PB_THREADS / 64 : 1][8];
     __shared__ uint32_t sPrev;
     const int t = (int) threadIdx.x;
-    const uint64_t base = (uint64_t) blockIdx.x * PB_TILE;
+    const uint64_t base = (uint64_t) tile * PB_TILE;
     const uint64_t j = base + (uint64_t) t;
     const bool have = j < n_entries;
     const uint64_t jc = have ? j : (n_entries ? n_entries - 1 : 0);
@@ -84,7 +86,7 @@
     if (KEYS) {
         const int wv = t >> 6;
         const bool first = tg_own >> 3 != tg_before >> 3;
-        if (!SAMPLE && t < PB_TILE && j >= 1 && j < n_entries && tg_own < tg_before) atomicOr(bad, 1ull);
+        if (WRITES && t < PB_TILE && j >= 1 && j < n_entries && tg_own < tg_before) atomicOr(bad, 1ull);
         const unsigned long long mf = __ballot(first);
         unsigned long long mc[7];
 #pragma unroll
@@ -211,7 +213,7 @@
         uint4 *line = tab + (size_t) (key >> idx_shift) * 8;
         if (!part) {
             if (i == 0) {
-                if (!SAMPLE) {
+                if (WRITES) {
                     uint32_t cz = drec.z, cw = drec.w;
                     if (KEYS && full_record) {
                         const uint32_t b3 = tg_own & ~7u;
@@ -237,7 +239,7 @@
             const int nsub = __popcll(lm);
             const int iL = L - s;
             const int k = __popcll(lm & ((1ull << iL) - 1ull));
-            if (!SAMPLE) {
+            if (WRITES) {
                 const unsigned long long right = m == 0 ? 0ull : (sRm[L] >> (64 - m));
                 uint32_t succ_id = 0xFFFFFFFFu, delta = 0u;
                 if (right != 0ull && my_slot > s && my_rank >= 1) { succ_id = sSlot[my_slot - 1]; delta = 1u + (uint32_t) __builtin_ctzll(right); }
@@ -245,10 +247,10 @@
                 const bool leftmost = first_group && t == (int) (sMax[L] & 0xFFFFu);
                 side[j] = make_uint4(node_id, succ_id, delta | ((uint32_t) m << 8) | ((uint32_t) k << 16) | (leftmost ? 0x40000000u : 0u) | (first_group ? 0x80000000u : 0u),
                                      k == 0 ? key >> idx_shift : (uint32_t) (e0 + (uint64_t) k));
-                if (leftmost && plist) plist[(size_t) blockIdx.x * PB_THREADS + atomicAdd(&sPiles, 1u)] = pile_who((uint32_t) k, k == 0 ? key >> idx_shift : (uint32_t) (e0 + (uint64_t) k), cc.n_buckets, n_entries);
+                if (leftmost && plist) plist[(size_t) tile * PB_THREADS + atomicAdd(&sPiles, 1u)] = pile_who((uint32_t) k, k == 0 ? key >> idx_shift : (uint32_t) (e0 + (uint64_t) k), cc.n_buckets, n_entries);
                 if (!first_group && own_mask) atomicOr(&own_mask[j >> 5], 1u << (j & 31u));
             }
-            if (!SAMPLE && L == t && k >= 1 && k < PILE_MAXSUB) {
+            if (WRITES && L == t && k >= 1 && k < PILE_MAXSUB) {
                 const unsigned long long rm = sRm[t];
                 const uint64_t slot = e0 + (uint64_t) k;
                 rec[slot * 4 + 0] = make_uint4(S[0], S[1], S[2], S[3]);
@@ -265,7 +267,7 @@
                 }
                 const bool irregular = sBad[s] != 0u || nsub > PILE_MAXSUB;
                 const uint32_t ns1 = (uint32_t) (nsub < PILE_MAXSUB ? nsub : PILE_MAXSUB) - 1u;
-                if (!SAMPLE) {
+                if (WRITES) {
                     const unsigned long long rm = sRm[t];
                     line[0] = make_uint4(S[0], S[1], S[2], S[3]);
                     line[1] = make_uint4(S[4], S[5], S[6], S[7]);
@@ -275,21 +277,39 @@
                 atomicAdd(&sCount[0], 1u);
                 if (irregular) atomicAdd(&sCount[1], 1u);
             }
-            if (!SAMPLE && L == s && t == (int) (sMax[s] & 0xFFFFu)) {
+            if (WRITES && L == s && t == (int) (sMax[s] & 0xFFFFu)) {
                 if (KEYS) { const unsigned long long co = class_offsets(); drec.z = (uint32_t) co; drec.w = (uint32_t) (co >> 32); }
                 line[4] = make_uint4(cnt, drec.x, drec.z, drec.w);
                 line[5] = make_uint4(sSlot[s], sMin[s] >> 16, 0u, 0u);
             }
         }
     }
-    if (!SAMPLE && have && t < PB_TILE && !regular) {
+    if (WRITES && have && t < PB_TILE && !regular) {
         side[j] = make_uint4(node_id, 0xFFFFFFFFu, 0u, 0u);
         if (own_mask) atomicOr(&own_mask[j >> 5], 1u << (j & 31u));
     }
     if (SAMPLE && owned) atomicAdd(&sCount[2], 1u);
     __syncthreads();
-    if (!SAMPLE && plist && t == 0) pcount[blockIdx.x] = sPiles;
+    if (WRITES && plist && t == 0) pcount[tile] = sPiles;
     if (SAMPLE && t < 3 && sCount[t]) atomicAdd(&pile_cnt[t], (unsigned long long) sCount[t]);
+}
+
+template <bool SAMPLE, bool KEYS>
+__global__ void __launch_bounds__(PB_THREADS, 6) k_pile_build(NodesDev nd, const uint32_t *__restrict__ skeys, const uint32_t *__restrict__ sids, uint64_t n_entries, const uint4 *__restrict__ dir, ClusterCfg cc, int U,
+                                                           uint4 *__restrict__ rec, uint4 *__restrict__ tab, uint32_t epoch,
+                                                           uint4 *__restrict__ side, unsigned long long *__restrict__ pile_cnt, uint32_t *__restrict__ own_mask,
+                                                           uint32_t *__restrict__ plist, uint32_t *__restrict__ pcount, unsigned long long *__restrict__ bad,
+                                                           uint32_t full_record, uint32_t tile0) {
+    pile_build_tile<SAMPLE, KEYS, false>(nd, skeys, sids, n_entries, dir, cc, U, rec, tab, epoch, side, pile_cnt, own_mask, plist, pcount, bad, full_record, blockIdx.x + tile0);
+}
+
+template <bool KEYS>
+__global__ void __launch_bounds__(PB_THREADS, 6) k_pile_sample_keep(NodesDev nd, const uint32_t *__restrict__ skeys, const uint32_t *__restrict__ sids, uint64_t n_entries, const uint4 *__restrict__ dir, ClusterCfg cc, int U,
+                                                                 uint4 *__restrict__ rec, uint4 *__restrict__ tab, uint32_t epoch,
+                                                                 uint4 *__restrict__ side, unsigned long long *__restrict__ pile_cnt, uint32_t *__restrict__ own_mask,
+                                                                 uint32_t *__restrict__ plist, uint32_t *__restrict__ pcount, unsigned long long *__restrict__ bad,
+                                                                 uint32_t full_record) {
+    pile_build_tile<true, KEYS, true>(nd, skeys, sids, n_entries, dir, cc, U, rec, tab, epoch, side, pile_cnt, own_mask, plist, pcount, bad, full_record, blockIdx.x);
 }
 
 constexpr int PILE_RUNS = 8;
@@ -1074,30 +1094,38 @@
 
 __global__ void k_pile_sample_force(unsigned long long *__restrict__ pile_cnt, unsigned long long buckets, unsigned long long irregular) { pile_cnt[0] = buckets; pile_cnt[1] = irregular; }
 
-void launch_pile_sample(const NodesDev &nd, const ClusterCfg &cc, int uniform_len, const uint32_t *skeys, const uint32_t *sids, const void *dir, unsigned long long *pile_cnt,
-                        int no_sample, hipStream_t s, bool from_keys) {
+uint32_t launch_pile_sample(const NodesDev &nd, const ClusterCfg &cc, int uniform_len, const uint32_t *skeys, const uint32_t *sids, const void *dir, unsigned long long *pile_cnt,
+                            int no_sample, hipStream_t s, bool from_keys, const PileKeep *keep) {
     (void) hipMemsetAsync(pile_cnt, 0, PILE_CNT_WORDS * sizeof(unsigned long long), s);
     const uint64_t n_entries = nd.n > 0 ? (uint64_t) nd.n : 0;
     if (no_sample == 2) hipLaunchKernelGGL(k_pile_sample_force, dim3(1), dim3(1), 0, s, pile_cnt, 100ull, 1ull);
-    if (n_entries == 0 || no_sample) return;
+    if (n_entries == 0 || no_sample) return 0u;
     const uint64_t tiles = (n_entries + PB_TILE - 1) / PB_TILE;
     const dim3 sample((unsigned) std::max<uint64_t>(1, std::min<uint64_t>(tiles, std::max<uint64_t>(64, tiles / 32)))), block(PB_THREADS);
-    hipLaunchKernelGGL((from_keys ? k_pile_build<true, true> : k_pile_build<true, false>), sample, block, 0, s, nd, skeys, sids, n_entries, (const uint4 *) dir, cc, uniform_len, (uint4 *) nullptr,
-                       (uint4 *) nullptr, 0u, (uint4 *) nullptr, pile_cnt, (uint32_t *) nullptr, (uint32_t *) nullptr, (uint32_t *) nullptr, (unsigned long long *) nullptr, 0u);
+    if (keep) {
+        uint32_t *own_mask = keep->own_mask, *pl = own_mask ? (uint32_t *) keep->plist : nullptr, *pc = pl ? pl + tiles * PB_THREADS : nullptr;
+        if (own_mask) (void) hipMemsetAsync(own_mask, 0, pile_own_mask_bytes(n_entries), s);
+        hipLaunchKernelGGL((from_keys ? k_pile_sample_keep<true> : k_pile_sample_keep<false>), sample, block, 0, s, nd, skeys, sids, n_entries, (const uint4 *) dir, cc, uniform_len, (uint4 *) keep->rec,
+                           (uint4 *) keep->tab, keep->epoch, (uint4 *) keep->side, pile_cnt, own_mask, pl, pc, keep->bad_flag, keep->full_record ? 1u : 0u);
+    } else
+        hipLaunchKernelGGL((from_keys ? k_pile_build<true, true> : k_pile_build<true, false>), sample, block, 0, s, nd, skeys, sids, n_entries, (const uint4 *) dir, cc, uniform_len, (uint4 *) nullptr,
+                           (uint4 *) nullptr, 0u, (uint4 *) nullptr, pile_cnt, (uint32_t *) nullptr, (uint32_t *) nullptr, (uint32_t *) nullptr, (unsigned long long *) nullptr, 0u, 0u);
     hipLaunchKernelGGL(k_pile_sample_close, dim3(1), dim3(1), 0, s, pile_cnt);
+    return keep ? sample.x : 0u;
 }
 
 void launch_pile_build(const NodesDev &nd, const PrefSufCfg &cfg, const ClusterCfg &cc, int uniform_len, const uint32_t *skeys, const uint32_t *sids, const void *dir, void *rec, void *rec2,
                        void *tab, uint32_t epoch, void *side, const void *runs, int nwin, const unsigned long long *pile_cnt, uint32_t *own_mask, void *plist, hipStream_t s,
-                       bool from_keys, unsigned long long *bad_flag, bool full_record, bool runs_ahead) {
+                       bool from_keys, unsigned long long *bad_flag, bool full_record, bool runs_ahead, uint32_t tile0) {
     const uint64_t n_entries = nd.n > 0 ? (uint64_t) nd.n : 0;
     if (n_entries == 0) return;
     const uint64_t tiles = (n_entries + PB_TILE - 1) / PB_TILE;
     if (!own_mask) plist = nullptr;
     uint32_t *pl = (uint32_t *) plist, *pc = pl ? pl + tiles * PB_THREADS : nullptr;
-    if (own_mask) (void) hipMemsetAsync(own_mask, 0, pile_own_mask_bytes(n_entries), s);
-    hipLaunchKernelGGL((from_keys ? k_pile_build<false, true> : k_pile_build<false, false>), dim3((unsigned) tiles), dim3(PB_THREADS), 0, s, nd, skeys, sids, n_entries, (const uint4 *) dir, cc, uniform_len,
-                       (uint4 *) rec, (uint4 *) tab, epoch, (uint4 *) side, const_cast<unsigned long long *>(pile_cnt), own_mask, pl, pc, bad_flag, full_record ? 1u : 0u);
+    if (own_mask && tile0 == 0) (void) hipMemsetAsync(own_mask, 0, pile_own_mask_bytes(n_entries), s);
+    if (tile0 < tiles)
+        hipLaunchKernelGGL((from_keys ? k_pile_build<false, true> : k_pile_build<false, false>), dim3((unsigned) (tiles - tile0)), dim3(PB_THREADS), 0, s, nd, skeys, sids, n_entries, (const uint4 *) dir, cc, uniform_len,
+                           (uint4 *) rec, (uint4 *) tab, epoch, (uint4 *) side, const_cast<unsigned long long *>(pile_cnt), own_mask, pl, pc, bad_flag, full_record ? 1u : 0u, tile0);
     if (pl)
         hipLaunchKernelGGL(k_pile_runs_consensus_list, dim3((unsigned) ((tiles + PR_SEGS - 1) / PR_SEGS)), dim3(TK_ROWS), 0, s, (const uint32_t *) pl, (const uint32_t *) pc, (uint32_t) tiles,
                            (const uint4 *) side, n_entries, (uint4 *) tab, (const uint4 *) rec, (uint4 *) rec2, cc, uniform_len, cfg.Lmin, pile_cnt, own_mask, runs_ahead ? 1 : 0);
diff --git a/alga_amd/csrc/prefsuf_shard.h b/alga_amd/csrc/prefsuf_shard.h
--- a/alga_amd/csrc/prefsuf_shard.h
+++ b/alga_amd/csrc/prefsuf_shard.h
@@ -11,7 +11,7 @@
 void launch_shard_select(const uint32_t *keys, uint32_t n, int shift, uint32_t b_lo, uint32_t b_hi, uint32_t *okeys, uint32_t *ovals, unsigned long long *cursor, hipStream_t s);
 hipError_t launch_cluster_store_slice(const NodesDev &nd, const ClusterCfg &cc, int eq, uint64_t m, uint32_t bucket_base, uint32_t n_buckets_local, uint32_t *keys,
                                       uint32_t *vals, uint32_t *keys2, uint32_t *vals2, const uint32_t *meta, int uniform_len, void *sort_temp, size_t sort_temp_bytes,
-                                      void *store, void *dir, unsigned long long *bad_flag, hipStream_t s, bool own_sort = true);
+                                      void *store, void *dir, unsigned long long *bad_flag, hipStream_t s, bool own_sort = true, uint32_t dir_blocks = 0);
 void launch_shard_export(bool count, const void *runs, int32_t node_begin, int32_t node_end, int shift, uint32_t bpr, uint32_t n_ranks, unsigned long long *counts,
                          int32_t *flagged_list, unsigned long long *flagged_count, uint32_t flagged_cap, const unsigned long long *seg_off, unsigned long long *cursor,
                          uint32_t *out, hipStream_t s);
```

New measurement: 5.559 billion edges/s, median of 6. 1.01x the previous value.
